# mcveanlab/mccortex

Hardware: AMD Instinct MI355X
Metric: k-mers/s inserted (build), k=31, 50M x 150bp synthetic reads (higher is better)
Workload: dtype u64

## Files before the change

### include/mcx_gpu.h

```cpp
#ifndef MCX_GPU_H_
#define MCX_GPU_H_

#include <stddef.h>
#include <stdint.h>

#ifdef __cplusplus
extern "C" {
#endif

typedef enum {
  MCX_OK = 0,
  MCX_ERR_ARG = -1,
  MCX_ERR_NODEVICE = -2,
  MCX_ERR_NOMEM = -3,
  MCX_ERR_FULL = -4,
  MCX_ERR_HIP = -5,
  MCX_ERR_SINK = -6
} mcx_status;

typedef struct {
  uint64_t num_se_reads;
  uint64_t num_good_reads;
  uint64_t num_bad_reads;
  uint64_t total_bases_read;
  uint64_t total_bases_loaded;
  uint64_t contigs_parsed;
  uint64_t num_kmers_loaded;
  uint64_t num_kmers_novel;
  uint64_t num_pe_reads;
  uint64_t num_dup_se_reads;
  uint64_t num_dup_pe_pairs;
} mcx_load_stats;

typedef struct mcx_graph mcx_graph;

const char *mcx_last_error(void);
const char *mcx_version(void);
int mcx_device_count(void);
int mcx_device_memory(int device, uint64_t *free_bytes, uint64_t *total_bytes);

int mcx_graph_create(mcx_graph **g, int kmer_size, int ncols,
                     uint64_t capacity_kmers, int device);
int mcx_graph_create_shard(mcx_graph **g, int kmer_size, int ncols, uint64_t capacity_kmers,
                           int device, int nparts, int part);
void mcx_graph_destroy(mcx_graph *g);

int mcx_graph_reset(mcx_graph *g);

int mcx_graph_configure(mcx_graph *g, const char *key, uint64_t value);
int mcx_graph_profile(mcx_graph *g, char *buf, size_t buflen);

int mcx_graph_create_multi(mcx_graph **out, int kmer_size, int ncols, uint64_t capacity_kmers,
                           const int *devices, int ndevices);
int mcx_multi_exchange_bytes(int kmer_size, int ndevices, uint64_t capacity_kmers, uint64_t *bytes_per_device);
int mcx_graph_ndevices(const mcx_graph *g);

int mcx_graph_capacity(const mcx_graph *g, uint64_t *slots, uint64_t *bytes);

int mcx_graph_add_reads(mcx_graph *g, int colour,
                        const uint8_t *bases, const uint8_t *quals,
                        const uint64_t *read_offsets, uint64_t nreads,
                        uint8_t fq_cutoff_abs, uint8_t hp_cutoff,
                        mcx_load_stats *stats_accum);

int mcx_graph_add_reads_pcr(mcx_graph *g, int colour,
                            const uint8_t *bases, const uint8_t *quals,
                            const uint64_t *read_offsets, uint64_t nreads,
                            uint8_t fq_cutoff_abs1, uint8_t fq_cutoff_abs2, uint8_t hp_cutoff,
                            int paired, int matedir, mcx_load_stats *stats_accum);
int mcx_graph_pcr_reset(mcx_graph *g);

int mcx_graph_add_stream_dev(mcx_graph *g, int colour,
                             const void *d_stream, uint64_t nbytes);

int mcx_pack_stream_dev(const void *d_stream, uint64_t nbytes, void *d_code, void *d_inv, void *hip_stream);
int mcx_graph_add_packed_dev(mcx_graph *g, int colour, const void *d_code, const void *d_inv, uint64_t npos);

int mcx_graph_partition_stream_dev(mcx_graph *g, const void *d_stream, uint64_t nbytes,
                                   int nparts, uint64_t bin_capacity,
                                   void *d_keys, void *d_edges, void *d_counts);
int mcx_graph_insert_tuples_dev(mcx_graph *g, int colour, const void *d_keys,
                                const void *d_edges, uint64_t n);
uint32_t mcx_key_owner(const uint64_t *key_words, int kmer_size, int nparts);

int mcx_graph_hashtest(mcx_graph *g, uint64_t first, uint64_t n);
int mcx_hashtest_func(int device, int kmer_size, uint64_t n, uint32_t nparts, uint64_t *hash_out);

int mcx_debug_probe(void *d_buf, uint64_t cap_words, uint32_t nregions, uint32_t spb, uint32_t iters, uint32_t jit_mask, float *ms_out);

int mcx_graph_insert_tuple_segments_dev(mcx_graph *g, int colour, const void *d_keys, const void *d_edges,
                                        const void *d_counts, uint32_t nseg, uint64_t seg_cap);

int mcx_graph_shard_layout(mcx_graph *g, uint64_t tuples_per_call, uint32_t *segs_per_owner,
                           uint64_t *seg_cap, uint64_t *ov_cap);
int mcx_graph_shard_bins_dev(mcx_graph *g, const void *d_stream, uint64_t nbytes, void *d_keys,
                             void *d_counts, uint64_t seg_cap, void *d_ov_keys, void *d_ov_edges,
                             void *d_ov_counts, uint64_t ov_cap);
int mcx_graph_add_segments_dev(mcx_graph *g, int colour, const void *d_keys, const void *d_counts,
                               uint32_t nseg, uint64_t seg_cap, uint64_t ntuples);
uint32_t mcx_graph_key_owner(const mcx_graph *g, const uint64_t *key_words);

enum { MCX_RECORDS_MUST_EXIST = 1, MCX_RECORDS_MASK_EDGES = 2 };
typedef struct {
  uint64_t nkmers_read, nkmers_loaded, nkmers_novel;
  int64_t first_oversized, first_zero_covg, first_edges_no_covg;
} mcx_records_stats;
int mcx_graph_add_records(mcx_graph *g, const void *recs, uint64_t nrecs, int file_ncols,
                          const int32_t *from_col, const int32_t *into_col, int nmap, uint32_t flags,
                          mcx_records_stats *stats_accum);

int mcx_graph_intersect_finish(mcx_graph *g, uint64_t *removed);

#define MCX_CLEAN_NBINS 1000
#define MCX_CLEAN_BYTES_PER_KMER 64
#define MCX_CLEAN_BYTES_PER_SLOT 4
typedef struct {
  uint64_t num_tips, num_tip_kmers;
  uint64_t num_low_covg_unitigs, num_low_covg_unitig_kmers;
  uint64_t num_tip_and_low_unitigs, num_tip_and_low_unitig_kmers;
  uint64_t nkmers_before, nkmers_removed;
} mcx_clean_stats;
int mcx_graph_unitig_stats(mcx_graph *g, uint64_t *before);
int mcx_graph_clean(mcx_graph *g, uint32_t covg_threshold, uint32_t min_keep_tip, mcx_clean_stats *stats, uint64_t *after);

enum { MCX_INFER_POP = 1, MCX_INFER_PRESENCE_COVG = 2 };
int mcx_graph_infer_edges(mcx_graph *g, void *recs, uint64_t nrecs, int ncols, uint32_t flags, uint64_t *nmodified);
int mcx_graph_infer_edges_dev(mcx_graph *g, void *d_recs, uint64_t nrecs, int ncols, uint32_t flags, uint64_t *nmodified);

int mcx_graph_kmer_covg(mcx_graph *g, uint64_t *nkmers, uint64_t *sumcov);
int mcx_graph_covg_histogram(mcx_graph *g, uint64_t *hist, uint32_t nbins);

int mcx_graph_checksum(mcx_graph *g, uint64_t *checksum, uint64_t *nkmers);
// ... 52 lines not shown
```

### mccortex_amd/csrc/mcx_api.hip

```cpp
#include <hip/hip_runtime.h>

#include <stdarg.h>
#include <stdio.h>
#include <stdlib.h>
#include <string.h>
#include <cstring>

#include <rocprim/device/device_radix_sort.hpp>
#include <rocprim/device/device_scan.hpp>

#include <algorithm>
#include <array>
#include <cmath>
#include <memory>
#include <vector>
#include <thread>
#include <atomic>
#include <chrono>
#include <mutex>
#include <condition_variable>
#include <functional>

#include "../../include/mcx_gpu.h"
#include "mcx_kernels.h"
// ... 81 lines not shown
  {
    if (owner_.load() == std::this_thread::get_id()) {
      fprintf(stderr, "mcx: internal error: the staging pool was re-entered between begin() and finish()\n");
      abort();
    }
  }
  std::atomic<std::thread::id> owner_{std::thread::id()};
  void worker()
  {
    std::unique_lock<std::mutex> lk(mu_);
    for (;;) {
      cv_work_.wait(lk, [&] { return next_ < T_; });
      const int ti = next_++;
      const std::function<void(int)> *f = fn_;
      lk.unlock();
      (*f)(ti);
      lk.lock();
      if (--pending_ == 0) cv_done_.notify_one();
    }
  }
  std::mutex mu_, call_mu_;
  std::condition_variable cv_work_, cv_done_;
  std::vector<std::thread> th_;
  const std::function<void(int)> *fn_ = nullptr;
  int T_ = 0, next_ = 0, pending_ = 0;
};

constexpr uint64_t kCarry = 128;
constexpr uint32_t kL1Sets = 32;
static uint64_t stage_bytes()
{
  static uint64_t v = 0;
  if (!v) {
    const char *e = getenv("MCX_STAGE_BYTES");
    v = e ? strtoull(e, nullptr, 10) : (128ull << 20);
    if (v < 1024) v = 1024;
    v = (v + 63) / 64 * 64;
  }
  return v;
}
#define kStageBytes stage_bytes()

struct mcx_group;
struct mcx_graph {
  int k = 0, W = 0, ncols = 0, device = 0;
  hipStream_t stream = nullptr;
  TableView t{};
  uint64_t table_bytes = 0;
  uint64_t touch_bytes = 0;
  Counters *d_ctr = nullptr;
  Counters *h_ctr = nullptr;
  uint32_t *h_full = nullptr;
  static constexpr int kStageBufs = 3;
  uint8_t *h_stage[kStageBufs] = {nullptr, nullptr, nullptr};
  uint8_t *d_stage[kStageBufs] = {nullptr, nullptr, nullptr};
  hipEvent_t ev[kStageBufs] = {nullptr, nullptr, nullptr};
  hipStream_t cstream = nullptr;
  hipEvent_t ev_copy[kStageBufs] = {nullptr, nullptr, nullptr}, ev_wait0[kStageBufs] = {nullptr, nullptr, nullptr}, ev_wait1[kStageBufs] = {nullptr, nullptr, nullptr};
  bool ev_wait_used[kStageBufs] = {false, false, false};
  uint64_t stage_alloc = 0;
  int cur = 0;
  int grid = 0;
  int grid_stream = 0, grid_split = 0, grid_insert = 0;
  bool defer = true;
  uint64_t defer_tuples = 0;
  uint32_t nsub = 0;
  uint32_t b1 = 0, subs_per_bin = 0;
  uint64_t cap1 = 0, cap2 = 0;
  uint32_t rep1 = 8;
  bool rep1_forced = false;
  uint64_t *l1_keys = nullptr, *l2_keys = nullptr;
  uint64_t *l2_hi = nullptr;
  uint64_t l2_hi_off = 0;
  uint64_t *l2_base = nullptr;
  int place_tries = 1;
  uint64_t l2_off = 0;
  hipStream_t stream2 = nullptr;
  hipEvent_t ev_split[2] = {nullptr, nullptr}, ev_ins[2] = {nullptr, nullptr};
  unsigned long long *l1_cnt = nullptr, *l2_cnt = nullptr;
  uint32_t nsets = 1;
  uint64_t set_cap = 0;
  std::vector<int> set_colour;
  std::vector<uint64_t> set_pending;
  uint64_t pending = 0;
  uint64_t pending_l2 = 0;
  uint32_t l2_regions = 0;
  uint32_t flush_regions = 0;
  uint32_t idle_next = 0;
  uint64_t idle_base = 0;
  std::vector<uint64_t> idle_mark;
  static constexpr uint32_t kSnap = 32;
  struct Snap { uint64_t ub; int set; int which; bool is_base; hipEvent_t ev; };
  Counters *h_snap = nullptr;
  Snap snap[kSnap] = {};
  uint32_t snap_head = 0, snap_tail = 0;
  uint64_t snap_last[2] = {0, 0};
  bool snap_base_known = true;
  uint64_t n_flushes = 0;
  int hidden = -1;
  int ncols_vis = 0;
  uint32_t *d_readstrt = nullptr;
  bool must_exist = false;
  int pending_colour = 0;
  bool profile = false;
  int overlap = -1;
  struct Span { const char *name; hipEvent_t a, b; };
  std::vector<Span> spans;
  mcx_group *group = nullptr;
  int gidx = 0;
  mcx_group *as_group = nullptr;
  uint32_t own_lbo = 0;
  unsigned long long *d_infer = nullptr;
  struct CleanCache *clean = nullptr;
};

static uint8_t *touch_base(const mcx_graph *g) { return reinterpret_cast<uint8_t *>(g->t.touch) - kTouchHdr; }

static OwnerSpec owner_spec(const mcx_graph *g)
{
  if (g->own_lbo) return OwnerSpec{2u, g->own_lbo, (uint32_t)g->gidx, g->k};
  return OwnerSpec{g->t.lbo ? 1u : 0u, 0u, 0u, g->k};
}

static int flush_deferred(mcx_graph *g);
static void free_defer(mcx_graph *g);
static void snap_push(mcx_graph *g, bool is_base);
static void snap_push(mcx_graph *g, bool is_base, uint64_t ub, int set, int which);
static void sets_release(mcx_graph *g)
{
  std::fill(g->set_colour.begin(), g->set_colour.end(), -1);
  std::fill(g->set_pending.begin(), g->set_pending.end(), 0);
}
struct StreamLaunch;
static int group_submit_stream(mcx_group *G, int idx, const StreamLaunch &L, int colour);
static void group_destroy(mcx_group *G);
static int grp_drain(mcx_group *G);
static int grp_sync(mcx_group *G);
static int grp_device_stats(mcx_group *G, mcx_load_stats *out);
static int grp_add_reads(mcx_group *G, int colour, const uint8_t *bases, const uint8_t *quals, const uint64_t *off,
                         uint64_t nreads, uint8_t fq, uint8_t hp, mcx_load_stats *stats_accum);
static int grp_add_reads_pcr(mcx_group *G, int colour, const uint8_t *bases, const uint8_t *quals, const uint64_t *off,
                             uint64_t nreads, uint8_t fq1, uint8_t fq2, uint8_t hp, int paired, int matedir,
                             mcx_load_stats *stats_accum);
static int grp_add_reads_must_exist(mcx_group *G, int colour, const uint8_t *bases, const uint8_t *quals, const uint64_t *off,
                                    uint64_t nreads, uint8_t fq, uint8_t hp, mcx_load_stats *stats_accum);
static int grp_intersect_finish(mcx_group *G, uint64_t *removed);
static int grp_add_records(mcx_group *G, const void *recs, uint64_t nrecs, int file_ncols, const int32_t *from_col,
                           const int32_t *into_col, int nmap, uint32_t flags, mcx_records_stats *stats_accum);
static int grp_export(mcx_group *G, mcx_graph *f, int sorted, mcx_sink_fn sink, void *ctx);
static int grp_part_of_pointer(mcx_group *G, const void *d_ptr, mcx_graph **part);
static mcx_graph *grp_part(mcx_group *G, int i);
static int grp_n(mcx_group *G);
static uint64_t grp_spilled(mcx_group *G);
#define NO_GROUP(g, what) do { if ((g) && (g)->as_group) return fail(MCX_ERR_ARG, what " takes a shard, not the multi-GPU handle"); } while (0)

extern "C" const char *mcx_last_error(void) { return g_err; }
extern "C" const char *mcx_version(void) { return "mccortex_amd 0.1 (gfx950)"; }

extern "C" int mcx_device_count(void)
{
  int n = 0;
  if (hipGetDeviceCount(&n) != hipSuccess) return 0;
  return n;
}

extern "C" int mcx_device_memory(int device, uint64_t *free_bytes, uint64_t *total_bytes)
{
  int ndev = 0;
  if (hipGetDeviceCount(&ndev) != hipSuccess || device < 0 || device >= ndev)
    return fail(MCX_ERR_NODEVICE, "no HIP device %d", device);
  HIP_TRY(hipSetDevice(device));
  size_t f = 0, t = 0;
  HIP_TRY(hipMemGetInfo(&f, &t));
  if (free_bytes) *free_bytes = f;
  if (total_bytes) *total_bytes = t;
  return MCX_OK;
}

static int check_k(int k)
{
  if (k < 3 || k > 127 || !(k & 1)) return fail(MCX_ERR_ARG, "kmer size must be odd and 3..127 (got %d)", k);
  return MCX_OK;
}

extern "C" int mcx_graph_create(mcx_graph **out, int kmer_size, int ncols, uint64_t capacity_kmers, int device)
{
  return mcx_graph_create_shard(out, kmer_size, ncols, capacity_kmers, device, 1, 0);
}

static uint32_t region_bits(uint64_t nsub, uint32_t lbo)
{
  uint32_t lb1 = 0;
  const uint32_t lb1_max = lbo ? std::min<uint32_t>(9, 11 - lbo) : 9;
  while (lb1 < lb1_max && (2ull << lb1) <= nsub) lb1++;
  while (lb1 < 11 && ((nsub + (1ull << lb1) - 1) >> lb1) > (uint64_t)kMaxBins) lb1++;
  return lb1;
}

extern "C" int mcx_graph_create_shard(mcx_graph **out, int kmer_size, int ncols, uint64_t capacity_kmers, int device,
                                      int nparts, int part)
{
  if (!out) return fail(MCX_ERR_ARG, "null handle pointer");
  *out = nullptr;
  if (check_k(kmer_size) != MCX_OK) return MCX_ERR_ARG;
  if (nparts < 1 || nparts > 32 || (nparts & (nparts - 1)) || part < 0 || part >= nparts)
    return fail(MCX_ERR_ARG, "shards must be a power of two <= 32 and 0 <= part < shards (got %d of %d)", part, nparts);
  if (ncols < 1 || ncols > 4096) return fail(MCX_ERR_ARG, "ncols out of range: %d", ncols);
  if (kmer_size > 63 && nparts != 1)
    return fail(MCX_ERR_ARG, "k > 63 (three- and four-word keys) builds on one device: the exchange formats carry at most two key words");
  int ndev = 0;
  if (hipGetDeviceCount(&ndev) != hipSuccess || ndev <= 0)
    return fail(MCX_ERR_NODEVICE, "no HIP device available (this library has no CPU path)");
  if (device < 0 || device >= ndev) return fail(MCX_ERR_NODEVICE, "device %d out of range (%d devices)", device, ndev);
  HIP_TRY(hipSetDevice(device));

  mcx_graph *g = new mcx_graph();
  g->k = kmer_size;
  g->W = words_for_k(kmer_size);
  g->ncols = ncols;
  g->ncols_vis = ncols;
  g->device = device;
  const uint64_t sub_slots = 1ull << sub_shift_for_words(g->W);
  uint64_t nsub = (std::max<uint64_t>(capacity_kmers, 1024) + sub_slots - 1) / sub_slots;
  uint32_t lbo = 0;
  while ((1 << lbo) < nparts) lbo++;
  uint32_t lb1 = region_bits(nsub, lbo);
  if (const char *e = getenv("MCX_LB1")) { const uint32_t v = (uint32_t)atoi(e); if (!lbo && v >= 6 && v <= 11 && ((nsub + (1ull << v) - 1) >> v) <= (uint64_t)kMaxBins && ((nsub + (1ull << v) - 1) >> v) >= 1) lb1 = v; }
  if (lbo && lb1 + lbo > 11) {
    const uint64_t max_slots = ((uint64_t)kMaxBins << (11 - lbo)) * sub_slots;
    delete g;
    return fail(MCX_ERR_ARG, "capacity per device too large for a table split over %d devices: %llu slots requested, at most %llu "
                "(use more devices or a smaller -n / -m)", nparts, (unsigned long long)(nsub * sub_slots), (unsigned long long)max_slots);
  }
  const uint64_t spb = (nsub + (1ull << lb1) - 1) >> lb1;
  nsub = spb << lb1;
  if (nsub >= (1ull << 31)) { delete g; return fail(MCX_ERR_ARG, "capacity too large"); }
  uint64_t novf = std::max<uint64_t>(sub_slots, (nsub * sub_slots / 32 + sub_slots - 1) / sub_slots * sub_slots);
  if (const char *e = getenv("MCX_OVERFLOW_SLOTS")) novf = strtoull(e, nullptr, 10) / kBucket * kBucket;
  if (novf / kBucket >= (1ull << 32)) novf = ((1ull << 32) - 1) * kBucket;
  const uint64_t slots = nsub * sub_slots + novf;
  g->t.nmain = nsub * sub_slots;
  g->t.nslots = slots;
  g->t.lb1 = lb1;
  g->t.lbo = lbo;
  g->t.part = (uint32_t)part;
  g->t.spb = (uint32_t)spb;
  g->t.S = (uint32_t)(g->W + ncols);
  g->t.max_probe = (uint32_t)sub_slots;
  { const char *e = getenv("MCX_DEFER"); if (e) g->defer = atoi(e) != 0; }
  if (g->W > 2) g->defer = false;
  { const char *e = getenv("MCX_GRID_STREAM"); if (e) g->grid_stream = atoi(e); }
  { const char *e = getenv("MCX_REP1"); if (e && atoi(e) >= 1 && atoi(e) <= 4096) { g->rep1 = (uint32_t)atoi(e); g->rep1_forced = true; } }
  { const char *e = getenv("MCX_GRID_SPLIT"); if (e) g->grid_split = atoi(e); }
  { const char *e = getenv("MCX_GRID_INSERT"); if (e) g->grid_insert = atoi(e); }
  g->table_bytes = slots * g->t.S * 8;

  hipDeviceProp_t prop;
  HIP_TRY(hipGetDeviceProperties(&prop, device));
  g->grid = prop.multiProcessorCount * 8;

#define CREATE_TRY(expr)                                                            \
  do {                                                                              \
    hipError_t _e = (expr);                                                         \
    if (_e != hipSuccess) {                                                         \
      int rc = fail(_e == hipErrorOutOfMemory ? MCX_ERR_NOMEM : MCX_ERR_HIP, "%s: %s", #expr, hipGetErrorString(_e)); \
      mcx_graph_destroy(g);                                                         \
      return rc;                                                                    \
    }                                                                               \
  } while (0)
  CREATE_TRY(hipStreamCreateWithFlags(&g->stream, hipStreamNonBlocking));
  CREATE_TRY(hipMalloc((void **)&g->t.rec, g->table_bytes));
  if (ncols == 1) {
    g->t.KS = g->t.VS = (uint32_t)(g->W + 1);
    g->t.val = g->t.rec + g->W;
    g->t.VC = 0;
  } else {
    g->t.KS = (uint32_t)g->W;
    g->t.VS = 1;
    g->t.val = g->t.rec + g->t.nslots * (uint64_t)g->W;
    g->t.VC = g->t.nslots;
  }
  CREATE_TRY(hipMalloc((void **)&g->d_ctr, sizeof(Counters)));
  CREATE_TRY(hipHostMalloc((void **)&g->h_ctr, sizeof(Counters), hipHostMallocDefault));
  CREATE_TRY(hipHostMalloc((void **)&g->h_full, sizeof(uint32_t), hipHostMallocDefault));
  *g->h_full = 0;
  g->touch_bytes = (1 + ((g->t.nmain >> sub_shift_for_words(g->W)) + 31) / 32) * 4;
  {
    uint8_t *tb = nullptr;
    CREATE_TRY(hipMalloc((void **)&tb, kTouchHdr + g->touch_bytes));
    g->t.touch = reinterpret_cast<uint32_t *>(tb + kTouchHdr);
  }
  CREATE_TRY(hipMemsetAsync(g->t.rec, 0, g->table_bytes, g->stream));
  CREATE_TRY(hipMemsetAsync(touch_base(g), 0, kTouchHdr + g->touch_bytes, g->stream));
  CREATE_TRY(hipMemsetAsync(g->d_ctr, 0, sizeof(Counters), g->stream));
  CREATE_TRY(hipStreamSynchronize(g->stream));
#undef CREATE_TRY
  *out = g;
  return MCX_OK;
}

static void clean_drop(mcx_graph *g);

extern "C" void mcx_graph_destroy(mcx_graph *g)
{
  if (g && g->as_group) { group_destroy(g->as_group); delete g; return; }
  if (!g) return;
  (void)hipSetDevice(g->device);
  if (g->stream) (void)hipStreamSynchronize(g->stream);
  if (g->cstream) { (void)hipStreamSynchronize(g->cstream); (void)hipStreamDestroy(g->cstream); }
  for (int i = 0; i < mcx_graph::kStageBufs; i++) {
    if (g->h_stage[i]) (void)hipHostFree(g->h_stage[i]);
    if (g->d_stage[i]) (void)hipFree(g->d_stage[i]);
    if (g->ev[i]) (void)hipEventDestroy(g->ev[i]);
    if (g->ev_copy[i]) (void)hipEventDestroy(g->ev_copy[i]);
    if (g->ev_wait0[i]) (void)hipEventDestroy(g->ev_wait0[i]);
    if (g->ev_wait1[i]) (void)hipEventDestroy(g->ev_wait1[i]);
  }
  free_defer(g);
  for (auto &sp : g->spans) { (void)hipEventDestroy(sp.a); (void)hipEventDestroy(sp.b); }
  if (g->t.rec) (void)hipFree(g->t.rec);
  if (g->t.touch) (void)hipFree(touch_base(g));
  if (g->stream2) {
    (void)hipStreamDestroy(g->stream2);
    for (int i = 0; i < 2; i++) { (void)hipEventDestroy(g->ev_split[i]); (void)hipEventDestroy(g->ev_ins[i]); }
  }
  if (g->d_ctr) (void)hipFree(g->d_ctr);
  if (g->d_readstrt) (void)hipFree(g->d_readstrt);
  if (g->d_infer) (void)hipFree(g->d_infer);
  clean_drop(g);
  if (g->h_ctr) (void)hipHostFree(g->h_ctr);
  if (g->h_full) (void)hipHostFree(g->h_full);
  if (g->h_snap) {
    (void)hipHostFree(g->h_snap);
    for (uint32_t i = 0; i < mcx_graph::kSnap; i++) (void)hipEventDestroy(g->snap[i].ev);
  }
  if (g->stream) (void)hipStreamDestroy(g->stream);
  delete g;
}

extern "C" int mcx_graph_reset(mcx_graph *g)
{
  if (g && g->as_group) {
    int rc = grp_drain(g->as_group);
    for (int i = 0; rc == MCX_OK && i < grp_n(g->as_group); i++) rc = mcx_graph_reset(grp_part(g->as_group, i));
    return rc;
  }
  if (!g) return fail(MCX_ERR_ARG, "null graph");
  HIP_TRY(hipSetDevice(g->device));
  clean_drop(g);
  HIP_TRY(hipMemsetAsync(g->t.rec, 0, g->table_bytes, g->stream));
  HIP_TRY(hipMemsetAsync(touch_base(g), 0, kTouchHdr + g->touch_bytes, g->stream));
  HIP_TRY(hipMemsetAsync(g->d_ctr, 0, sizeof(Counters), g->stream));
  g->n_flushes = 0;
  if (g->h_full) { HIP_TRY(hipStreamSynchronize(g->stream)); *g->h_full = 0; }
  if (g->l1_cnt) HIP_TRY(hipMemsetAsync(g->l1_cnt, 0, (size_t)g->nsets * g->b1 * g->rep1 * 8, g->stream));
  if (g->l2_cnt) HIP_TRY(hipMemsetAsync(g->l2_cnt, 0, (size_t)g->l2_regions * g->subs_per_bin * 8, g->stream));
  if (g->d_readstrt) HIP_TRY(hipMemsetAsync(g->d_readstrt, 0xff, g->t.nslots * 8, g->stream));
  g->pending = g->pending_l2 = 0;
  g->idle_next = 0; g->idle_base = 0; g->idle_mark.clear();
  sets_release(g);
  snap_push(g, true);
  return MCX_OK;
}

extern "C" int mcx_graph_capacity(const mcx_graph *g, uint64_t *slots, uint64_t *bytes)
{
  if (g && g->as_group) {
    uint64_t s_ = 0, b_ = 0;
    for (int i = 0; i < grp_n(g->as_group); i++) { uint64_t s1 = 0, b1 = 0; mcx_graph_capacity(grp_part(g->as_group, i), &s1, &b1); s_ += s1; b_ += b1; }
    if (slots) *slots = s_;
    if (bytes) *bytes = b_;
    return MCX_OK;
  }
  if (!g) return fail(MCX_ERR_ARG, "null graph");
  if (slots) *slots = g->t.nslots;
  if (bytes) *bytes = g->table_bytes;
  return MCX_OK;
}

extern "C" void *mcx_graph_stream(mcx_graph *g) { return !g ? nullptr : g->as_group ? (void *)grp_part(g->as_group, 0)->stream : (void *)g->stream; }

struct StreamLaunch {
  const uint8_t *stream;
  uint64_t nbytes, pos_lo, pos_hi;
  unsigned char *flag;
  const uint32_t *code = nullptr;
  const uint16_t *inv = nullptr;
};

#define DISPATCH_WC(g, F, ...)                                                        \
  do {                                                                                \
    if ((g)->W == 1) { if ((g)->ncols == 1) F<1, true>(__VA_ARGS__); else F<1, false>(__VA_ARGS__); } \
    else { if ((g)->ncols == 1) F<2, true>(__VA_ARGS__); else F<2, false>(__VA_ARGS__); }            \
  } while (0)

#define DISPATCH_WC4(g, F, ...)                                                       \
  do {                                                                                \
    const bool one_ = (g)->ncols == 1;                                                \
    switch ((g)->W) {                                                                 \
      case 1: if (one_) F<1, true>(__VA_ARGS__); else F<1, false>(__VA_ARGS__); break; \
      case 2: if (one_) F<2, true>(__VA_ARGS__); else F<2, false>(__VA_ARGS__); break; \
      case 3: if (one_) F<3, true>(__VA_ARGS__); else F<3, false>(__VA_ARGS__); break; \
      default: if (one_) F<4, true>(__VA_ARGS__); else F<4, false>(__VA_ARGS__); break; \
    }                                                                                 \
  } while (0)
#define LAUNCH_W4(W_, KERNEL, ...)                                       \
  do {                                                                   \
    switch (W_) {                                                        \
      case 1: hipLaunchKernelGGL((KERNEL<1>), __VA_ARGS__); break;       \
      case 2: hipLaunchKernelGGL((KERNEL<2>), __VA_ARGS__); break;       \
      case 3: hipLaunchKernelGGL((KERNEL<3>), __VA_ARGS__); break;       \
      default: hipLaunchKernelGGL((KERNEL<4>), __VA_ARGS__); break;      \
    }                                                                    \
  } while (0)
#define NO_WIDE(g, what) do { if ((g) && (g)->W > 2) return fail(MCX_ERR_ARG, what " is not available for k > 63"); } while (0)

struct SpanGuard {
  mcx_graph *g; size_t idx; bool on;
  SpanGuard(mcx_graph *g_, const char *name) : g(g_), idx(0), on(g_->profile) {
    if (!on) return;
    mcx_graph::Span sp{name, nullptr, nullptr};
    (void)hipEventCreate(&sp.a); (void)hipEventCreate(&sp.b);
    (void)hipEventRecord(sp.a, g->stream);
    idx = g->spans.size();
    g->spans.push_back(sp);
  }
  ~SpanGuard() { if (on) (void)hipEventRecord(g->spans[idx].b, g->stream); }
};

template <class K> static void allow_lds(K kernel, size_t bytes)
{
  (void)hipFuncSetAttribute(reinterpret_cast<const void *>(kernel), hipFuncAttributeMaxDynamicSharedMemorySize, (int)bytes);
}

static StreamArgs make_args(mcx_graph *g, const StreamLaunch &L)
{
  StreamArgs a;
  a.stream = L.stream; a.code = L.code; a.inv = L.inv; a.nbytes = L.nbytes; a.pos_lo = L.pos_lo; a.pos_hi = L.pos_hi;
  a.tile0 = L.pos_lo / kTile;
  a.ntiles = (L.pos_hi + kTile - 1) / kTile;
  a.k = g->k; a.ctr = g->d_ctr; a.flag = L.flag;
  return a;
}

template <int W, bool ONECOL> static void launch_direct_t(mcx_graph *g, const StreamLaunch &L, int colour)
{
  const StreamArgs a = make_args(g, L);
  const uint64_t nt = a.ntiles > a.tile0 ? a.ntiles - a.tile0 : 0;
  if (!nt) return;
  InsertSink<W, ONECOL> is{g->t, (uint32_t)colour};
  SpanGuard sp(g, "k_stream");
  const dim3 grid((unsigned)std::min<uint64_t>(nt, (uint64_t)g->grid));
  if (a.code) hipLaunchKernelGGL((k_stream<W, ONECOL, true>), grid, dim3(kThreads), 0, g->stream, a, is);
  else hipLaunchKernelGGL((k_stream<W, ONECOL, false>), grid, dim3(kThreads), 0, g->stream, a, is);
}

template <int W, bool ONECOL, bool FULL, int SH, bool PK>
static void launch_bin_stream_pk(mcx_graph *g, const StreamArgs &a, uint64_t nt, int colour, BinSpec bs, BinOut out)
{
  InsertSink<W, ONECOL> is{g->t, (uint32_t)colour};
  static bool once_dev[64] = {false};
  bool &once = once_dev[g->device & 63];
  if (!once) {
    allow_lds(k_stream_bin<W, ONECOL, 512, FULL, SH, PK>, sizeof(BinLds<W, 512, FULL>));
    allow_lds(k_stream_bin<W, ONECOL, 1024, FULL, SH, PK>, sizeof(BinLds<W, 1024, FULL>));
    allow_lds(k_stream_bin<W, ONECOL, kMaxBins, FULL, SH, PK>, sizeof(BinLds<W, kMaxBins, FULL>));
    once = true;
  }
  SpanGuard sp(g, "k_stream_bin");
  if constexpr (W == 1 && !FULL && SH == 0) {
    static const int fc_cap = [] { const char *e = getenv("MCX_STREAM_FC"); return e ? atoi(e) : 0; }();
    if (fc_cap && bs.nlocal <= 512) {
      const dim3 gridf((unsigned)std::min<uint64_t>(nt, (uint64_t)(g->grid_stream ? g->grid_stream : g->grid)));
#define MCX_FC_LAUNCH(CAPV, PRIVV) { \
        static bool once_f[64] = {false}; \
        if (!once_f[g->device & 63]) { allow_lds(k_stream_fc<ONECOL, PK, CAPV, PRIVV>, sizeof(FcLds<CAPV>)); once_f[g->device & 63] = true; } \
        hipLaunchKernelGGL((k_stream_fc<ONECOL, PK, CAPV, PRIVV>), gridf, dim3(kThreads), sizeof(FcLds<CAPV>), g->stream, a, bs, out, is); }
      if (bs.rep >= gridf.x && bs.rep > 8) MCX_FC_LAUNCH(10, true)
      else MCX_FC_LAUNCH(10, false)
#undef MCX_FC_LAUNCH
      return;
    }
    static const bool wide = [] { const char *e = getenv("MCX_STREAM_T"); return !e || atoi(e) == 512; }();
    if (wide && bs.nlocal <= 512) {
      using GeoW = Geo<512, 512 * kPosPerLane>;
      static bool once_w[64] = {false};
      if (!once_w[g->device & 63]) { allow_lds(k_stream_bin<W, ONECOL, 512, FULL, SH, PK, 512>, sizeof(BinLds<W, 512, FULL, GeoW>)); once_w[g->device & 63] = true; }
      const dim3 gridw((unsigned)std::min<uint64_t>((nt + 1) / 2, (uint64_t)(g->grid_stream ? g->grid_stream : g->grid)));
      hipLaunchKernelGGL((k_stream_bin<W, ONECOL, 512, FULL, SH, PK, 512>), gridw, dim3(512), sizeof(BinLds<W, 512, FULL, GeoW>), g->stream, a, bs, out, is);
      return;
    }
  }
  const dim3 grid((unsigned)std::min<uint64_t>(nt, (uint64_t)(g->grid_stream ? g->grid_stream : g->grid)));
  if (bs.nlocal <= 512)
    hipLaunchKernelGGL((k_stream_bin<W, ONECOL, 512, FULL, SH, PK>), grid, dim3(kThreads), sizeof(BinLds<W, 512, FULL>), g->stream, a, bs, out, is);
  else if (bs.nlocal <= 1024)
    hipLaunchKernelGGL((k_stream_bin<W, ONECOL, 1024, FULL, SH, PK>), grid, dim3(kThreads), sizeof(BinLds<W, 1024, FULL>), g->stream, a, bs, out, is);
  else
    hipLaunchKernelGGL((k_stream_bin<W, ONECOL, kMaxBins, FULL, SH, PK>), grid, dim3(kThreads), sizeof(BinLds<W, kMaxBins, FULL>), g->stream, a, bs, out, is);
}

template <int W, bool ONECOL, bool FULL, int SH>
static void launch_bin_stream_t(mcx_graph *g, const StreamLaunch &L, int colour, BinSpec bs, BinOut out)
{
  const StreamArgs a = make_args(g, L);
  const uint64_t nt = a.ntiles > a.tile0 ? a.ntiles - a.tile0 : 0;
  if (!nt) return;
  if (!FULL && a.code) launch_bin_stream_pk<W, ONECOL, FULL, SH, !FULL>(g, a, nt, colour, bs, out);
  else launch_bin_stream_pk<W, ONECOL, FULL, SH, false>(g, a, nt, colour, bs, out);
}

template <int W, bool ONECOL, bool IN_FULL, bool SHARD>
static void launch_bin_tuples_t(mcx_graph *g, TupleIn in, int colour, BinSpec bs, BinOut out)
{
  constexpr bool kWide = W == 1 && !IN_FULL;
  static const bool wide = kWide && [] { const char *e = getenv("MCX_SPLIT_T"); return !e || atoi(e) == 512; }();
  const bool use_wide = wide && bs.nlocal <= 1024;
  const bool use_huge = wide && !use_wide && bs.nlocal <= (uint32_t)kMaxBins;
  const uint64_t tile = use_huge ? 1024 * 16 : use_wide ? 512 * 16 : kTile;
  const uint64_t nchunks = (in.seg_cap + tile - 1) / tile * in.nseg;
  if (!nchunks) return;
  InsertSink<W, ONECOL> is{g->t, (uint32_t)colour};
  using GeoW = Geo<512, 512 * 16>;
  static bool once_dev[64] = {false};
  bool &once = once_dev[g->device & 63];
  if (!once) {
    allow_lds(k_tuples_bin<W, ONECOL, 512, IN_FULL, SHARD>, sizeof(BinLds<W, 512, false>));
    allow_lds(k_tuples_bin<W, ONECOL, 1024, IN_FULL, SHARD>, sizeof(BinLds<W, 1024, false>));
    allow_lds(k_tuples_bin<W, ONECOL, kMaxBins, IN_FULL, SHARD>, sizeof(BinLds<W, kMaxBins, false>));
    if constexpr (kWide) allow_lds(k_tuples_bin<W, ONECOL, 512, IN_FULL, SHARD, 512>, sizeof(BinLds<W, 512, false, GeoW>));
    if constexpr (kWide) allow_lds(k_tuples_bin<W, ONECOL, 1024, IN_FULL, SHARD, 512>, sizeof(BinLds<W, 1024, false, GeoW>));
    if constexpr (kWide) allow_lds(k_tuples_bin<W, ONECOL, kMaxBins, IN_FULL, SHARD, 1024>, sizeof(BinLds<W, kMaxBins, false, Geo<1024, 1024 * 16>>));
    once = true;
  }
  SpanGuard sp(g, "k_tuples_bin");
  const uint64_t gmax = (uint64_t)(g->grid_split ? g->grid_split : g->grid * 4);
  if constexpr (kWide) {
    if (use_huge) {
      using GeoH = Geo<1024, 1024 * 16>;
      const dim3 gridh((unsigned)std::min<uint64_t>(nchunks, g->grid_split ? gmax : gmax / 4));
      hipLaunchKernelGGL((k_tuples_bin<W, ONECOL, kMaxBins, IN_FULL, SHARD, 1024>), gridh, dim3(1024), sizeof(BinLds<W, kMaxBins, false, GeoH>), g->stream, in, bs, out, is, g->d_ctr);
      return;
    }
    if (use_wide) {
      const dim3 gridw((unsigned)std::min<uint64_t>(nchunks, g->grid_split ? gmax : gmax / 2));
      if (bs.nlocal <= 512)
        hipLaunchKernelGGL((k_tuples_bin<W, ONECOL, 512, IN_FULL, SHARD, 512>), gridw, dim3(512), sizeof(BinLds<W, 512, false, GeoW>), g->stream, in, bs, out, is, g->d_ctr);
      else
        hipLaunchKernelGGL((k_tuples_bin<W, ONECOL, 1024, IN_FULL, SHARD, 512>), gridw, dim3(512), sizeof(BinLds<W, 1024, false, GeoW>), g->stream, in, bs, out, is, g->d_ctr);
      return;
    }
  }
  const dim3 grid((unsigned)std::min<uint64_t>(nchunks, gmax));
  if (bs.nlocal <= 512)
    hipLaunchKernelGGL((k_tuples_bin<W, ONECOL, 512, IN_FULL, SHARD>), grid, dim3(kThreads), sizeof(BinLds<W, 512, false>), g->stream, in, bs, out, is, g->d_ctr);
  else if (bs.nlocal <= 1024)
    hipLaunchKernelGGL((k_tuples_bin<W, ONECOL, 1024, IN_FULL, SHARD>), grid, dim3(kThreads), sizeof(BinLds<W, 1024, false>), g->stream, in, bs, out, is, g->d_ctr);
  else
    hipLaunchKernelGGL((k_tuples_bin<W, ONECOL, kMaxBins, IN_FULL, SHARD>), grid, dim3(kThreads), sizeof(BinLds<W, kMaxBins, false>), g->stream, in, bs, out, is, g->d_ctr);
}
template <int W, bool ONECOL> static void launch_bin_region_stream(mcx_graph *g, const StreamLaunch &L, int colour, BinSpec bs, BinOut out)
{
  if (g->t.lbo) launch_bin_stream_t<W, ONECOL, false, 1>(g, L, colour, bs, out);
  else launch_bin_stream_t<W, ONECOL, false, 0>(g, L, colour, bs, out);
}
template <int W, bool ONECOL> static void launch_split_regions(mcx_graph *g, TupleIn in, int colour, BinSpec bs, BinOut out)
{ launch_bin_tuples_t<W, ONECOL, false, false>(g, in, colour, bs, out); }
template <int W, bool ONECOL> static void launch_bin_received(mcx_graph *g, TupleIn in, int colour, BinSpec bs, BinOut out)
{
  if (g->t.lbo) launch_bin_tuples_t<W, ONECOL, true, true>(g, in, colour, bs, out);
  else launch_bin_tuples_t<W, ONECOL, true, false>(g, in, colour, bs, out);
}

static uint64_t *l2_ptr(const mcx_graph *g, uint64_t off)
{
  if (g->l2_hi && off >= g->l2_hi_off) return g->l2_hi + (off - g->l2_hi_off) * g->cap2 * g->W;
  return g->l2_keys + off * g->cap2 * g->W;
}

template <int W, bool ONECOL> static void launch_lds_insert_t(mcx_graph *g, int colour, uint32_t sub0, uint32_t nsub)
{
  const size_t lds = Sub<W>::kSlots * (W + 1) * 8 + LdsQueue<W>::kTuples * 8 * W;
  static bool once_dev[64] = {false};
  bool &once = once_dev[g->device & 63];
  if (!once) { allow_lds(k_lds_insert<W, ONECOL>, lds); once = true; }
  BinOut bins{l2_ptr(g, g->l2_off), nullptr, g->l2_cnt + g->l2_off, g->cap2, nullptr, nullptr, nullptr, 0};
  SpanGuard sp(g, "k_lds_insert");
  hipLaunchKernelGGL((k_lds_insert<W, ONECOL>), dim3((unsigned)std::min<uint64_t>(nsub, (uint64_t)(g->grid_insert ? g->grid_insert : g->grid * 4))),
                     dim3(LdsCfg<W>::kThreads), lds, g->stream, g->t, (uint32_t)colour, bins, sub0, nsub, g->d_ctr);
}

template <int W, bool ONECOL>
static void launch_insert_tuples_t(mcx_graph *g, int colour, const uint64_t *keys, const uint8_t *edges, uint64_t n, uint32_t only_own = 0)
{
  const int grid = (int)std::min<uint64_t>((n + kThreads * kBatch - 1) / (kThreads * kBatch), (uint64_t)g->grid);
  InsertSink<W, ONECOL> s{g->t, (uint32_t)colour};
  SpanGuard sp(g, "k_insert_tuples");
  hipLaunchKernelGGL((k_insert_tuples<W, ONECOL>), dim3(grid), dim3(kThreads), 0, g->stream, s, keys, edges, n, g->d_ctr, only_own);
}

static void free_defer(mcx_graph *g)
{
  (void)hipFree(g->l1_keys); (void)hipFree(g->l1_cnt);
  (void)hipFree(g->l2_base); (void)hipFree(g->l2_hi); (void)hipFree(g->l2_cnt);
  g->l1_keys = g->l2_keys = g->l2_base = g->l2_hi = nullptr; g->l1_cnt = g->l2_cnt = nullptr;
  g->cap1 = g->cap2 = 0;
  g->l2_regions = 0;
  g->set_colour.clear(); g->set_pending.clear();
}

__global__ __launch_bounds__(512) void k_l2_probe(uint64_t *keys, uint64_t cap, uint32_t nregions, uint32_t spb, uint32_t iters,
                                                  uint32_t jit_mask = 0 )
{
  const uint32_t region = blockIdx.x % nregions, blk = blockIdx.x / nregions, nblk = gridDim.x / nregions;
  const uint32_t w = threadIdx.x >> 6, l = threadIdx.x & 63u;
  for (uint32_t it = 0; it < iters; it++)
    for (uint32_t k = 0; k < spb / 32u; k++) {
      const uint32_t front = w * 4u + (l >> 4) + 32u * k;
      const uint32_t seg = region * spb + front;
      const uint64_t jit = ((seg * 0x9E3779B1u) >> 8) & jit_mask & ~15u;
      const uint64_t at = (uint64_t)seg * cap + jit + ((uint64_t)it * nblk + blk) * 16u + (l & 15u);
      if (jit + ((uint64_t)it * nblk + blk) * 16u + 16u <= cap) keys[at] = at;
    }
}

static uint64_t *l2_place(mcx_graph *g, size_t bytes, uint32_t nreg, int tries, float *ms_out)
{
  std::vector<uint64_t *> cand;
  std::vector<float> ms;
  hipEvent_t e0 = nullptr, e1 = nullptr;
  if (tries > 1 && (hipEventCreate(&e0) != hipSuccess || hipEventCreate(&e1) != hipSuccess)) { (void)hipGetLastError(); tries = 1; }
  const uint32_t iters = (uint32_t)std::max<uint64_t>(8, g->cap2 * g->W / 1024);
  for (int i = 0; i < std::max(tries, 1); i++) {
    if (i > 0) {
      size_t fr = 0, tot = 0;
      if (hipMemGetInfo(&fr, &tot) != hipSuccess || fr < bytes + (size_t)(tot / 16)) { (void)hipGetLastError(); break; }
    }
    uint64_t *p = nullptr;
    if (hipMalloc((void **)&p, bytes) != hipSuccess) { (void)hipGetLastError(); break; }
    cand.push_back(p);
    float t = 0.f;
    if (tries > 1)
      for (int rep = 0; rep < 2; rep++) {
        (void)hipEventRecord(e0, g->stream);
        hipLaunchKernelGGL(k_l2_probe, dim3(nreg * 64), dim3(512), 0, g->stream, p, g->cap2 * g->W, nreg, g->subs_per_bin, iters);
        (void)hipEventRecord(e1, g->stream);
        if (hipEventSynchronize(e1) != hipSuccess || hipEventElapsedTime(&t, e0, e1) != hipSuccess) { (void)hipGetLastError(); t = 0.f; }
      }
    ms.push_back(t);
    float worst = 0.f, best_t = 0.f;
    for (float x : ms) { worst = std::max(worst, x); if (x > 0.f && (best_t == 0.f || x < best_t)) best_t = x; }
    if (tries > 1 && best_t > 0.f && best_t < 0.70f * worst) break;
  }
  if (e0) (void)hipEventDestroy(e0);
  if (e1) (void)hipEventDestroy(e1);
  if (cand.empty()) return nullptr;
  size_t best = 0;
  for (size_t i = 1; i < cand.size(); i++) if (ms[i] > 0.f && (ms[best] <= 0.f || ms[i] < ms[best])) best = i;
  for (size_t i = 0; i < cand.size(); i++) if (i != best) (void)hipFree(cand[i]);
  if (getenv("MCX_TIMING") && cand.size() > 1) {
    fprintf(stderr, "[timing] sub-table bins (%u regions): %zu placements probed:", nreg, cand.size());
    for (size_t i = 0; i < cand.size(); i++) fprintf(stderr, " %.3f%s", ms[i], i == best ? "*" : "");
    fprintf(stderr, " ms\n");
  }
  if (ms_out) *ms_out = ms[best];
  return cand[best];
}

static uint32_t flush_group(const mcx_graph *g);
static int ensure_l2(mcx_graph *g, uint32_t regions, bool whole = false)
{
  if (g->l2_keys && g->l2_regions >= regions && !(g->l2_hi && (whole || (regions > g->l2_regions / 2 && regions != g->l2_regions)))) return MCX_OK;
  if (g->pending_l2) return fail(MCX_ERR_ARG, "internal: sub-table bins resized while in use");
  HIP_TRY(hipStreamSynchronize(g->stream));
  (void)hipFree(g->l2_base); (void)hipFree(g->l2_hi); (void)hipFree(g->l2_cnt);
  g->l2_keys = g->l2_base = g->l2_hi = nullptr; g->l2_cnt = nullptr; g->l2_regions = 0; g->l2_hi_off = 0;
  const uint64_t nb = (uint64_t)regions * g->subs_per_bin;
  int tries = g->place_tries;
  { const char *e = getenv("MCX_PLACE_BINS"); if (e) tries = atoi(e); }
  if (g->subs_per_bin % 32 || regions < 8) tries = 1;
  const uint32_t G = flush_group(g);
  const bool halves = !whole && tries > 1 && regions == 2 * G && !g->t.lbo && !g->group;
  if (halves) {
    const size_t hbytes = (nb / 2) * g->cap2 * 8 * g->W;
    g->l2_base = l2_place(g, hbytes, G, tries, nullptr);
    if (g->l2_base) g->l2_hi = l2_place(g, hbytes, G, tries, nullptr);
    if (g->l2_base && !g->l2_hi) { (void)hipFree(g->l2_base); g->l2_base = nullptr; }
    g->l2_hi_off = nb / 2;
  } else {
    g->l2_base = l2_place(g, nb * g->cap2 * 8 * g->W, std::min<uint32_t>(regions, 32), tries, nullptr);
  }
  if (!g->l2_base || hipMalloc((void **)&g->l2_cnt, nb * 8) != hipSuccess) {
    (void)hipGetLastError();
    (void)hipFree(g->l2_base); (void)hipFree(g->l2_hi); g->l2_base = g->l2_hi = nullptr;
    return fail(MCX_ERR_NOMEM, "out of device memory for the sub-table bins (%llu regions)", (unsigned long long)regions);
  }
  HIP_TRY(hipMemsetAsync(g->l2_cnt, 0, nb * 8, g->stream));
  g->l2_keys = g->l2_base;
  g->l2_regions = regions;
  return MCX_OK;
}

static bool flush_overlap(const mcx_graph *g)
{
  static const bool on = [] { const char *e = getenv("MCX_FLUSH_OVERLAP"); return !e || atoi(e) != 0; }();
  return g->overlap < 0 ? on : g->overlap != 0;
}

static uint32_t flush_group(const mcx_graph *g)
{
  uint32_t G = g->flush_regions;
  if (!G) {
    const char *e = getenv("MCX_FLUSH_REGIONS");
    G = e ? (uint32_t)strtoul(e, nullptr, 10) : 0;
  }
  if (!G) G = std::max<uint32_t>(32u, 16384u / std::max<uint32_t>(1u, g->subs_per_bin));
  return std::min<uint32_t>(G, g->b1);
}

static int ensure_defer(mcx_graph *g)
{
  if (g->l1_keys) return MCX_OK;
  g->nsub = (uint32_t)(g->t.nmain >> sub_shift_for_words(g->W));
  g->b1 = 1u << g->t.lb1;
  g->subs_per_bin = g->t.spb;
  if (g->t.lb1 < 6 || g->b1 > (uint32_t)kMaxBins || g->subs_per_bin > (uint32_t)kMaxBins) { g->defer = false; return MCX_OK; }
  uint64_t tcap = g->defer_tuples;
  if (!tcap) {
    const char *e = getenv("MCX_DEFER_TUPLES");
    if (e) {
      tcap = strtoull(e, nullptr, 10);
    } else {
      size_t fr = 0, tot = 0;
      (void)hipMemGetInfo(&fr, &tot);
      const uint64_t per_tuple = 8ull * g->W * (g->t.lbo ? 240 : 118) / 100 + 1;
      const uint64_t by_mem = (uint64_t)((double)fr * 0.40) / per_tuple;
      tcap = std::max<uint64_t>(std::min<uint64_t>(std::min<uint64_t>(64 * g->t.nslots, by_mem), 1ull << 33), 1ull << 20);
    }
  }
  for (;; tcap /= 2) {
    if (tcap < (1ull << 20)) { g->defer = false; g->defer_tuples = 0; (void)hipGetLastError(); return MCX_OK; }
    g->defer_tuples = tcap;
    g->nsets = g->ncols > 1 ? kL1Sets : 1;
    if (const char *e = getenv("MCX_L1_SETS")) { const int v = atoi(e); if (v >= 1 && v <= 32) g->nsets = (uint32_t)v; }
    g->set_cap = tcap / g->nsets;
    if (!g->rep1_forced) g->rep1 = g->nsets != 1 ? 8 : g->set_cap / g->b1 / 64 >= (1u << 16) ? 64 : g->set_cap / g->b1 / 32 >= (1u << 16) ? 32 : 8;
    g->cap1 = (uint64_t)((double)g->set_cap / g->b1 / g->rep1 * (g->b1 == 1 ? 1.02 : 1.06)) + (g->nsets > 1 ? 2048 : 8192);
    static const double cap2_slack = [] { const char *e = getenv("MCX_CAP2_SLACK"); const double v = e ? atof(e) : 0; return v >= 1.0 && v <= 4.0 ? v : 1.25; }();
    g->cap2 = g->nsub == 1 ? tcap + 8192 : (uint64_t)((double)tcap / g->nsub * cap2_slack) + 1024;
    g->cap1 = (g->cap1 + 1) & ~1ull;
    g->cap2 = (g->cap2 + 1) & ~1ull;
    if (g->cap1 >= 0xFFFFFFFFull || g->cap2 >= 0xFFFFFFFFull) continue;
    const uint64_t n1 = (uint64_t)g->nsets * g->b1 * g->rep1 * g->cap1;
    const bool ok = hipMalloc((void **)&g->l1_keys, n1 * 8 * g->W) == hipSuccess &&
                    hipMalloc((void **)&g->l1_cnt, (size_t)g->nsets * g->b1 * g->rep1 * 8) == hipSuccess &&
                    ensure_l2(g, flush_overlap(g) ? std::min<uint32_t>(2 * flush_group(g), g->b1) : flush_group(g)) == MCX_OK;
    if (ok) break;
    free_defer(g);
    (void)hipGetLastError();
  }
  HIP_TRY(hipMemsetAsync(g->l1_cnt, 0, (size_t)g->nsets * g->b1 * g->rep1 * 8, g->stream));
  g->set_colour.assign(g->nsets, -1);
  g->set_pending.assign(g->nsets, 0);
  return MCX_OK;
}

static BinOut l1_out(const mcx_graph *g, int set)
{
  const uint64_t segs = (uint64_t)g->b1 * g->rep1;
  return BinOut{g->l1_keys + (uint64_t)set * segs * g->cap1 * g->W, nullptr, g->l1_cnt + (uint64_t)set * segs, g->cap1, nullptr, nullptr, nullptr, 0};
}

static int ensure_flush_stream(mcx_graph *g)
{
  if (g->stream2) return MCX_OK;
  HIP_TRY(hipStreamCreateWithFlags(&g->stream2, hipStreamNonBlocking));
  for (int i = 0; i < 2; i++) {
    if (!g->ev_split[i]) HIP_TRY(hipEventCreateWithFlags(&g->ev_split[i], hipEventDisableTiming));
    if (!g->ev_ins[i]) HIP_TRY(hipEventCreateWithFlags(&g->ev_ins[i], hipEventDisableTiming));
  }
  return MCX_OK;
}

static int flush_deferred(mcx_graph *g)
{
  if (!g->pending && !g->pending_l2) {
    sets_release(g);
    if (!g->idle_mark.empty()) {
      g->idle_next = 0; g->idle_base = 0; g->idle_mark.clear();
      snap_push(g, true);
    }
    return MCX_OK;
  }
  HIP_TRY(hipSetDevice(g->device));
  const uint32_t G = g->pending_l2 ? g->b1 : std::min(flush_group(g), g->l2_regions);
  if (g->pending_l2 && g->l2_regions < g->b1) return fail(MCX_ERR_ARG, "internal: split tuples without bins");
  const bool overlap = flush_overlap(g) && g->pending && !g->pending_l2 && g->l2_regions >= 2 * G && G < g->b1;
  hipStream_t s1 = g->stream;
  if (overlap) {
    int rc2 = ensure_flush_stream(g);
    if (rc2 != MCX_OK) return rc2;
    HIP_TRY(hipEventRecord(g->ev_split[0], s1));
    HIP_TRY(hipStreamWaitEvent(g->stream2, g->ev_split[0], 0));
  }
  std::vector<int> colours;
  if (g->pending_l2) colours.push_back(g->pending_colour);
  for (uint32_t s = 0; s < g->nsets && g->pending; s++) {
    const int c = g->set_colour[s];
    if (c >= 0 && g->set_pending[s] && std::find(colours.begin(), colours.end(), c) == colours.end()) colours.push_back(c);
  }
  uint32_t gi = 0;
  for (size_t ci = 0; ci < colours.size(); ci++) {
    const int colour = colours[ci];
    TupleIn in{};
    uint32_t nmine = 0;
    for (uint32_t s = 0; s < g->nsets && g->pending; s++)
      if (g->set_colour[s] == colour && g->set_pending[s]) in.set_map[nmine++] = (uint8_t)s;
    for (uint32_t r0 = 0; r0 < g->b1; r0 += G, gi++) {
      const uint32_t ng = std::min(G, g->b1 - r0);
      const int hb = overlap ? (int)(gi & 1u) : 0;
      g->l2_off = (uint64_t)hb * G * g->subs_per_bin;
      if (overlap && gi >= 2) HIP_TRY(hipStreamWaitEvent(s1, g->ev_ins[hb], 0));
      if (nmine) {
        in.keys = g->l1_keys + (uint64_t)r0 * g->cap1 * g->W;
        in.edges = nullptr;
        in.counts = g->l1_cnt + r0;
        in.seg_cap = g->cap1;
        in.nseg = ng * g->rep1 * nmine;
        in.seg_group = ng;
        in.seg_stride = g->b1;
        in.set_rep = g->nsets > 1 ? g->rep1 : 0;
        BinSpec bs{BIN_SUBLOCAL, 0, g->subs_per_bin, 1, ng * g->subs_per_bin, ng, 0, r0};
        BinOut out{l2_ptr(g, g->l2_off), nullptr, g->l2_cnt + g->l2_off, g->cap2, nullptr, nullptr, nullptr, 0};
        DISPATCH_WC(g, launch_split_regions, g, in, colour, bs, out);
        HIP_TRY(hipGetLastError());
      }
      if (overlap) {
        HIP_TRY(hipEventRecord(g->ev_split[hb], s1));
        HIP_TRY(hipStreamWaitEvent(g->stream2, g->ev_split[hb], 0));
        g->stream = g->stream2;
      }
      DISPATCH_WC(g, launch_lds_insert_t, g, colour, r0 * g->subs_per_bin, ng * g->subs_per_bin);
      g->stream = s1;
      HIP_TRY(hipGetLastError());
      if (overlap) HIP_TRY(hipEventRecord(g->ev_ins[hb], g->stream2));
    }
  }
  g->l2_off = 0;
  if (overlap)
    for (int i = 0; i < 2; i++) HIP_TRY(hipStreamWaitEvent(s1, g->ev_ins[i], 0));
  if (g->pending) HIP_TRY(hipMemsetAsync(g->l1_cnt, 0, (size_t)g->nsets * g->b1 * g->rep1 * 8, g->stream));
  g->pending = 0;
  g->pending_l2 = 0;
  g->n_flushes++;
  g->idle_next = 0; g->idle_base = 0; g->idle_mark.clear();
  sets_release(g);
  snap_push(g, true);
  return MCX_OK;
}

static void snap_push(mcx_graph *g, bool is_base, uint64_t ub, int set, int which)
{
  if (!g->h_snap) {
    if (hipHostMalloc((void **)&g->h_snap, sizeof(Counters) * mcx_graph::kSnap, hipHostMallocDefault) != hipSuccess) { (void)hipGetLastError(); g->h_snap = nullptr; return; }
    for (uint32_t i = 0; i < mcx_graph::kSnap; i++)
      if (hipEventCreateWithFlags(&g->snap[i].ev, hipEventDisableTiming) != hipSuccess) {
        (void)hipGetLastError();
        for (uint32_t j = 0; j < i; j++) { (void)hipEventDestroy(g->snap[j].ev); g->snap[j].ev = nullptr; }
        (void)hipHostFree(g->h_snap);
        g->h_snap = nullptr;
        return;
      }
  }
  if (is_base) {
    g->snap_tail = g->snap_head;
    g->snap_base_known = false;
  }
  if (g->snap_head - g->snap_tail >= mcx_graph::kSnap) return;
  const uint32_t i = g->snap_head % mcx_graph::kSnap;
  if (hipMemcpyAsync(&g->h_snap[i], g->d_ctr, sizeof(Counters), hipMemcpyDeviceToHost, g->stream) != hipSuccess ||
      hipEventRecord(g->snap[i].ev, g->stream) != hipSuccess) { (void)hipGetLastError(); return; }
  g->snap[i].ub = ub;
  g->snap[i].set = set;
  g->snap[i].which = which;
  g->snap[i].is_base = is_base;
  g->snap_head++;
}
static void snap_push(mcx_graph *g, bool is_base) { snap_push(g, is_base, 0, 0, 0); }

static void snap_poll(mcx_graph *g)
{
  if (!g->h_snap) return;
  while (g->snap_tail != g->snap_head) {
    const uint32_t i = g->snap_tail % mcx_graph::kSnap;
    if (hipEventQuery(g->snap[i].ev) != hipSuccess) { (void)hipGetLastError(); break; }
    const uint64_t v[2] = {g->h_snap[i].kmers, g->h_snap[i].binned};
    const mcx_graph::Snap &e = g->snap[i];
    if (e.is_base) {
      g->snap_base_known = true;
    } else if (g->snap_base_known && g->idle_mark.empty() && (size_t)e.set < g->set_pending.size()) {
      const uint64_t yielded = std::min<uint64_t>(e.ub, v[e.which] - g->snap_last[e.which]);
      const uint64_t d = e.ub - yielded;
      g->pending -= std::min(g->pending, d);
      g->set_pending[e.set] -= std::min(g->set_pending[e.set], d);
    }
    g->snap_last[0] = v[0];
    g->snap_last[1] = v[1];
    g->snap_tail++;
  }
}

static bool defer_has_room(const mcx_graph *g, int colour, uint64_t need)
{
  for (uint32_t s = 0; s < g->nsets; s++)
    if (g->set_colour[s] < 0 || (g->set_colour[s] == colour && g->set_pending[s] + need <= g->set_cap)) return true;
  return false;
}
static void settle_for_room(mcx_graph *g, int colour, uint64_t need)
{
  if (!g->h_snap) return;
  while (!defer_has_room(g, colour, need) && g->snap_tail != g->snap_head) {
    if (hipEventSynchronize(g->snap[g->snap_tail % mcx_graph::kSnap].ev) != hipSuccess) { (void)hipGetLastError(); return; }
    const uint32_t before = g->snap_tail;
    snap_poll(g);
    if (g->snap_tail == before) return;
// ... 7 lines not shown
  if (rc != MCX_OK || !g->defer) return rc;
  snap_poll(g);
  settle_for_room(g, colour, ub);
  for (int pass = 0; pass < 2; pass++) {
    int free_set = -1;
    for (uint32_t s = 0; s < g->nsets; s++) {
      if (g->set_colour[s] == colour && g->set_pending[s] + ub <= g->set_cap) {
        g->set_pending[s] += ub; g->pending += ub;
        if (set_out) *set_out = (int)s;
        return MCX_OK;
      }
      if (g->set_colour[s] < 0 && free_set < 0) free_set = (int)s;
    }
    if (free_set >= 0) {
      g->set_colour[free_set] = colour;
      g->set_pending[free_set] = ub; g->pending += ub;
      if (set_out) *set_out = free_set;
      return MCX_OK;
    }
    rc = flush_deferred(g);
    if (rc != MCX_OK) return rc;
  }
  return fail(MCX_ERR_ARG, "internal: no L1 bin set after a flush");
}

static int l2_reserve(mcx_graph *g, int colour, uint64_t ub)
{
  int rc = ensure_defer(g);
  if (rc != MCX_OK || !g->defer) return rc;
  if ((g->pending_l2 && colour != g->pending_colour) ||
      ((g->pending_l2 || g->pending) && g->pending_l2 + g->pending + ub > g->defer_tuples)) {
    rc = flush_deferred(g);
    if (rc != MCX_OK) return rc;
  }
  g->pending_colour = colour;
  return MCX_OK;
}

static int full_poll(mcx_graph *g)
{
  if (!g->h_full || !g->t.touch) return MCX_OK;
  if (*g->h_full) return fail(MCX_ERR_FULL, "Hash table is full");
  HIP_TRY(hipMemcpyAsync(g->h_full, g->t.touch - 2, sizeof(uint32_t), hipMemcpyDeviceToHost, g->stream));
  return MCX_OK;
}

static int submit_stream(mcx_graph *g, const StreamLaunch &L, int colour)
{
  if (g->group) return group_submit_stream(g->group, g->gidx, L, colour);
  { int rc = full_poll(g); if (rc != MCX_OK) return rc; }
  if (g->defer) { int rc = ensure_defer(g); if (rc != MCX_OK) return rc; }
  if (!g->defer) {
    DISPATCH_WC4(g, launch_direct_t, g, L, colour);
    HIP_TRY(hipGetLastError());
    return MCX_OK;
  }
  snap_poll(g);
  for (uint64_t lo = L.pos_lo; lo < L.pos_hi;) {
    settle_for_room(g, colour, std::min<uint64_t>(L.pos_hi - lo, g->set_cap));
    uint64_t room = g->set_cap;
    for (uint32_t s = 0; s < g->nsets; s++)
      if (g->set_colour[s] == colour && g->set_pending[s] < g->set_cap) { room = g->set_cap - g->set_pending[s]; break; }
    if (room < (uint64_t)kTile * 16 && room < L.pos_hi - lo) room = g->set_cap;
    const uint64_t hi = std::min(L.pos_hi, lo + room);
    int set = 0;
    int rc = defer_reserve(g, colour, hi - lo, &set);
    if (rc != MCX_OK) return rc;
    StreamLaunch P = L;
    P.pos_lo = lo; P.pos_hi = hi;
    BinSpec bs{BIN_GROUP, 0, g->b1, g->rep1, g->b1, 1, 0, 0};
    BinOut out = l1_out(g, set);
    DISPATCH_WC(g, launch_bin_region_stream, g, P, colour, bs, out);
    HIP_TRY(hipGetLastError());
    snap_push(g, false, hi - lo, set, 0);
    lo = hi;
  }
  return MCX_OK;
}

static int ensure_stage(mcx_graph *g);



extern "C" int mcx_graph_configure(mcx_graph *g, const char *key, uint64_t value)
{
  if (g && key && g->as_group) {
    const bool isec = !strcmp(key, "intersect");
    if (isec && g->ncols < 2) return fail(MCX_ERR_ARG, "intersect mode needs one colour more than the output has");
    if (!strcmp(key, "defer") && !value) return fail(MCX_ERR_ARG, "a multi-GPU table always uses the partitioned insert");
    int rc = grp_drain(g->as_group);
    for (int i = 0; rc == MCX_OK && i < grp_n(g->as_group); i++) rc = mcx_graph_configure(grp_part(g->as_group, i), key, value);
    if (isec && rc == MCX_OK) {
      g->hidden = g->ncols - 1;
      g->ncols_vis = g->ncols - 1;
    }
    return rc;
  }
  if (!g || !key) return fail(MCX_ERR_ARG, "null argument");
  HIP_TRY(hipSetDevice(g->device));
  if (!strcmp(key, "defer")) {
    int rc = flush_deferred(g);
    if (rc != MCX_OK) return rc;
    g->defer = value != 0 && g->W <= 2;
    return MCX_OK;
  }
  if (!strcmp(key, "debug_realloc_l2")) {
    int rc = flush_deferred(g);
    if (rc != MCX_OK) return rc;
    if (!g->l2_keys || g->l2_hi) return MCX_OK;
    HIP_TRY(hipStreamSynchronize(g->stream));
    if (g->stream2) HIP_TRY(hipStreamSynchronize(g->stream2));
    static std::vector<void *> holes;
    void *hole = nullptr;
    if (value && hipMalloc(&hole, value) == hipSuccess) holes.push_back(hole);
    uint64_t *nk = nullptr;
    HIP_TRY(hipMalloc((void **)&nk, (uint64_t)g->l2_regions * g->subs_per_bin * g->cap2 * 8 * g->W));
    (void)hipFree(g->l2_base);
    g->l2_base = g->l2_keys = nk;
    return MCX_OK;
  }
  if (!strcmp(key, "place_bins")) {
    if (value < 1 || value > 32) return fail(MCX_ERR_ARG, "place_bins: 1..32");
    g->place_tries = (int)value;
    return MCX_OK;
  }
  if (!strcmp(key, "defer_tuples")) {
    int rc = flush_deferred(g);
    if (rc != MCX_OK) return rc;
    HIP_TRY(hipStreamSynchronize(g->stream));
    free_defer(g);
    g->defer_tuples = value;
    return MCX_OK;
  }
  if (!strcmp(key, "flush_overlap")) {
    int rc = flush_deferred(g);
    if (rc != MCX_OK) return rc;
    HIP_TRY(hipStreamSynchronize(g->stream));
    g->overlap = value != 0;
    if (g->l1_keys && g->overlap) return ensure_l2(g, std::min<uint32_t>(2 * flush_group(g), g->b1));
    return MCX_OK;
  }
  if (!strcmp(key, "flush_regions")) {
    int rc = flush_deferred(g);
    if (rc != MCX_OK) return rc;
    g->flush_regions = (uint32_t)value;
    if (g->l1_keys) return ensure_l2(g, flush_group(g));
    return MCX_OK;
  }
  if (!strcmp(key, "intersect")) {
    if (!value) return fail(MCX_ERR_ARG, "intersect mode cannot be switched off");
    if (g->ncols < 2) return fail(MCX_ERR_ARG, "intersect mode needs one colour more than the output has");
    HIP_TRY(hipStreamSynchronize(g->stream));
    g->hidden = g->ncols - 1;
    g->ncols_vis = g->ncols - 1;
    g->defer = false;
    return MCX_OK;
  }
  if (!strcmp(key, "must_exist")) {
    int rc = flush_deferred(g);
    if (rc != MCX_OK) return rc;
    g->must_exist = value != 0;
    if (g->must_exist) g->defer = false;
    return MCX_OK;
  }
  if (!strcmp(key, "prepare")) {
    const double t0 = now_s();
    int rc = ensure_stage(g);
    const double t1 = now_s();
    if (rc == MCX_OK && g->defer && !g->must_exist) rc = ensure_defer(g);
    const double t2 = now_s();
    if (rc == MCX_OK && g->defer && !g->must_exist && flush_overlap(g)) rc = ensure_flush_stream(g);
    if (getenv("MCX_TIMING"))
      fprintf(stderr, "[timing] prepare: pinned staging + copy stream %.1f ms, partition workspace (%.1f GB) %.1f ms, flush stream %.1f ms\n", (t1 - t0) * 1e3,
              g->l1_keys ? (double)g->nsets * g->b1 * g->rep1 * g->cap1 * 8 * g->W / 1e9 : 0.0, (t2 - t1) * 1e3, (now_s() - t2) * 1e3);
    return rc;
  }
  if (!strcmp(key, "grid")) {
    if (value > (1u << 20)) return fail(MCX_ERR_ARG, "grid: 0 .. 2^20 blocks");
    int cus = 0;
    HIP_TRY(hipDeviceGetAttribute(&cus, hipDeviceAttributeMultiprocessorCount, g->device));
    g->grid = value ? (int)value : cus * 8;
    return MCX_OK;
  }
  if (!strcmp(key, "grid_stream")) { g->grid_stream = (int)value; return MCX_OK; }
  if (!strcmp(key, "grid_split")) { g->grid_split = (int)value; return MCX_OK; }
  if (!strcmp(key, "grid_insert")) { g->grid_insert = (int)value; return MCX_OK; }
  if (!strcmp(key, "profile")) {
    HIP_TRY(hipStreamSynchronize(g->stream));
    for (auto &sp : g->spans) { (void)hipEventDestroy(sp.a); (void)hipEventDestroy(sp.b); }
    g->spans.clear();
    g->profile = value != 0;
    return MCX_OK;
  }
  return fail(MCX_ERR_ARG, "unknown configuration key '%s'", key);
}

extern "C" int mcx_graph_profile(mcx_graph *g, char *buf, size_t buflen)
{
  if (g && buf && buflen && g->as_group) {
    size_t o = 0;
    buf[0] = '\0';
    std::vector<char> tmp(buflen);
    for (int i = 0; i < grp_n(g->as_group); i++) {
// ... 34 lines not shown
  if (g && g->as_group) {
    mcx_graph *part = nullptr;
    int rc = grp_part_of_pointer(g->as_group, d_stream, &part);
    if (rc != MCX_OK) return rc;
    return mcx_graph_add_stream_dev(part, colour, d_stream, nbytes);
  }
  if (!g) return fail(MCX_ERR_ARG, "null graph");
  if (colour < 0 || colour >= g->ncols) return fail(MCX_ERR_ARG, "colour %d out of range", colour);
  if (((uintptr_t)d_stream & 15) != 0) return fail(MCX_ERR_ARG, "stream must be 16-byte aligned");
  if (!nbytes) return MCX_OK;
  HIP_TRY(hipSetDevice(g->device));
  StreamLaunch L{(const uint8_t *)d_stream, nbytes, 0, nbytes, nullptr};
  return submit_stream(g, L, colour);
}

extern "C" int mcx_pack_stream_dev(const void *d_stream, uint64_t nbytes, void *d_code, void *d_inv, void *hip_stream)
{
  if (!d_stream || !d_code || !d_inv) return fail(MCX_ERR_ARG, "null argument");
  if (((uintptr_t)d_stream & 15) != 0) return fail(MCX_ERR_ARG, "stream must be 16-byte aligned");
  if (!nbytes) return MCX_OK;
  const uint64_t nch = (nbytes + 15) / 16;
  hipLaunchKernelGGL(k_pack_stream, dim3((unsigned)((nch + 255) / 256)), dim3(256), 0, (hipStream_t)hip_stream,
                     (const uint8_t *)d_stream, nbytes, (uint32_t *)d_code, (uint16_t *)d_inv);
  HIP_TRY(hipGetLastError());
  return MCX_OK;
}

extern "C" int mcx_graph_add_packed_dev(mcx_graph *g, int colour, const void *d_code, const void *d_inv, uint64_t npos)
{
  if (!g) return fail(MCX_ERR_ARG, "null graph");
  if (g->as_group) {
    mcx_graph *part = nullptr;
    int rc = grp_part_of_pointer(g->as_group, d_code, &part);
    if (rc != MCX_OK) return rc;
    return mcx_graph_add_packed_dev(part, colour, d_code, d_inv, npos);
  }
  if (colour < 0 || colour >= g->ncols) return fail(MCX_ERR_ARG, "colour %d out of range", colour);
  if (!d_code || !d_inv) return fail(MCX_ERR_ARG, "null argument");
  if (!npos) return MCX_OK;
  if (g->must_exist) return fail(MCX_ERR_ARG, "device streams cannot be loaded in must-exist mode");
  HIP_TRY(hipSetDevice(g->device));
  StreamLaunch L{nullptr, npos, 0, npos, nullptr, (const uint32_t *)d_code, (const uint16_t *)d_inv};
  return submit_stream(g, L, colour);
}

extern "C" int mcx_graph_partition_stream_dev(mcx_graph *g, const void *d_stream, uint64_t nbytes, int nparts,
                                              uint64_t bin_capacity, void *d_keys, void *d_edges, void *d_counts)
{
  NO_GROUP(g, "mcx_graph_partition_stream_dev");
  if (!g) return fail(MCX_ERR_ARG, "null graph");
  NO_WIDE(g, "mcx_graph_partition_stream_dev");
  if (nparts < 1 || nparts > kMaxBins) return fail(MCX_ERR_ARG, "nparts must be 1..%d", kMaxBins);
  if (bin_capacity >= 0xFFFFFFFFull) return fail(MCX_ERR_ARG, "bin capacity must be below 2^32 tuples");
  if (((uintptr_t)d_stream & 15) != 0) return fail(MCX_ERR_ARG, "stream must be 16-byte aligned");
  if (!nbytes) return MCX_OK;
  HIP_TRY(hipSetDevice(g->device));
  StreamLaunch L{(const uint8_t *)d_stream, nbytes, 0, nbytes, nullptr};
  BinSpec bs{BIN_OWNER, (uint32_t)nparts, (uint32_t)nparts, 1, (uint32_t)nparts, 1, 0, 0};
  BinOut out{(uint64_t *)d_keys, (uint8_t *)d_edges, (unsigned long long *)d_counts, bin_capacity, nullptr, nullptr, nullptr, 0};
  if (g->W == 1) launch_bin_stream_t<1, true, true, 0>(g, L, 0, bs, out);
  else launch_bin_stream_t<2, true, true, 0>(g, L, 0, bs, out);
  HIP_TRY(hipGetLastError());
  return MCX_OK;
}

extern "C" int mcx_graph_insert_tuples_dev(mcx_graph *g, int colour, const void *d_keys, const void *d_edges, uint64_t n)
{
  NO_GROUP(g, "mcx_graph_insert_tuples_dev");
  if (!g) return fail(MCX_ERR_ARG, "null graph");
  if (colour < 0 || colour >= g->ncols) return fail(MCX_ERR_ARG, "colour %d out of range", colour);
  if (!n) return MCX_OK;
  HIP_TRY(hipSetDevice(g->device));
  if (g->defer) { int rc = ensure_defer(g); if (rc != MCX_OK) return rc; }
  if (!g->defer) {
    DISPATCH_WC4(g, launch_insert_tuples_t, g, colour, (const uint64_t *)d_keys, (const uint8_t *)d_edges, n);
    HIP_TRY(hipGetLastError());
    return MCX_OK;
  }
  for (uint64_t lo = 0; lo < n;) {
    const uint64_t cnt = std::min(n - lo, g->set_cap);
    int set = 0;
    int rc = defer_reserve(g, colour, cnt, &set);
    if (rc != MCX_OK) return rc;
    TupleIn in{(const uint64_t *)d_keys + lo * g->W, (const uint8_t *)d_edges + lo, nullptr, cnt, 1, 1, 1};
    BinSpec bs{BIN_GROUP, 0, g->b1, g->rep1, g->b1, 1, 0, 0};
    BinOut out = l1_out(g, set);
    DISPATCH_WC(g, launch_bin_received, g, in, colour, bs, out);
    HIP_TRY(hipGetLastError());
    lo += cnt;
  }
  return MCX_OK;
}

extern "C" int mcx_debug_probe(void *d_buf, uint64_t cap_words, uint32_t nregions, uint32_t spb, uint32_t iters, uint32_t jit_mask, float *ms_out)
{
  hipEvent_t e0, e1;
  HIP_TRY(hipEventCreate(&e0)); HIP_TRY(hipEventCreate(&e1));
  float t = 0.f;
  for (int rep = 0; rep < 2; rep++) {
    (void)hipEventRecord(e0, 0);
    hipLaunchKernelGGL(k_l2_probe, dim3(nregions * 64), dim3(512), 0, 0, (uint64_t *)d_buf, cap_words, nregions, spb, iters, jit_mask);
    (void)hipEventRecord(e1, 0);
    HIP_TRY(hipEventSynchronize(e1));
    HIP_TRY(hipEventElapsedTime(&t, e0, e1));
  }
  (void)hipEventDestroy(e0); (void)hipEventDestroy(e1);
  if (ms_out) *ms_out = t;
  return MCX_OK;
}

template <int W> __global__ void k_hashtest_keys(uint64_t *keys, uint64_t first, uint64_t n)
{
  for (uint64_t i = (uint64_t)blockIdx.x * blockDim.x + threadIdx.x; i < n; i += (uint64_t)gridDim.x * blockDim.x) {
    keys[i * W] = first + i;
    for (int w = 1; w < W; w++) keys[i * W + w] = 0;
  }
}
template <int W> __global__ void k_hashtest_func(uint64_t lo, uint64_t hi, unsigned int *out)
{
  uint32_t h = 0;
  for (uint64_t i = lo + (uint64_t)blockIdx.x * blockDim.x + threadIdx.x; i < hi; i += (uint64_t)gridDim.x * blockDim.x) {
    Kmer<W> key;
    key.w[0] = i;
    for (int w = 1; w < W; w++) key.w[w] = 0;
    h ^= kmer_hash<W>(key, 0, nullptr);
  }
  for (int d = 32; d; d >>= 1) h ^= __shfl_xor(h, d, 64);
  if ((threadIdx.x & 63) == 0 && h) atomicXor(out, h);
}

extern "C" int mcx_graph_hashtest(mcx_graph *g, uint64_t first, uint64_t n)
{
  NO_GROUP(g, "mcx_graph_hashtest");
  if (!g) return fail(MCX_ERR_ARG, "null graph");
  if (first + n < first) return fail(MCX_ERR_ARG, "key range wraps");
  HIP_TRY(hipSetDevice(g->device));
  const uint64_t chunk = std::min<uint64_t>(n, 1ull << 26);
  if (!chunk) return mcx_graph_sync(g);
  uint64_t *d_keys = nullptr;
  uint8_t *d_edges = nullptr;
  if (hipMalloc((void **)&d_keys, chunk * 8 * g->W) != hipSuccess || hipMalloc((void **)&d_edges, chunk) != hipSuccess) {
    (void)hipGetLastError(); (void)hipFree(d_keys); (void)hipFree(d_edges);
    return fail(MCX_ERR_NOMEM, "out of device memory for the hashtest key buffer");
  }
  int rc = MCX_OK;
  if (hipMemsetAsync(d_edges, 0, chunk, g->stream) != hipSuccess) rc = fail(MCX_ERR_HIP, "hipMemsetAsync failed");
  for (uint64_t lo = 0; lo < n && rc == MCX_OK; lo += chunk) {
    const uint64_t cnt = std::min(chunk, n - lo);
    LAUNCH_W4(g->W, k_hashtest_keys, dim3(4096), dim3(256), 0, g->stream, d_keys, first + lo, cnt);
    rc = mcx_graph_insert_tuples_dev(g, 0, d_keys, d_edges, cnt);
  }
  const int rc2 = mcx_graph_sync(g);
  (void)hipFree(d_keys); (void)hipFree(d_edges);
  return rc != MCX_OK ? rc : rc2;
}

extern "C" int mcx_hashtest_func(int device, int kmer_size, uint64_t n, uint32_t nparts, uint64_t *hash_out)
{
  int ndev = 0;
  if (hipGetDeviceCount(&ndev) != hipSuccess || device < 0 || device >= ndev) return fail(MCX_ERR_NODEVICE, "no HIP device %d", device);
  if (kmer_size < 3 || kmer_size > 127 || !(kmer_size & 1)) return fail(MCX_ERR_ARG, "kmer size %d", kmer_size);
  if (!nparts || !hash_out) return fail(MCX_ERR_ARG, "nparts / hash_out");
  HIP_TRY(hipSetDevice(device));
  unsigned int *d = nullptr;
  HIP_TRY(hipMalloc((void **)&d, (size_t)nparts * 4));
  std::vector<unsigned int> h(nparts, 0);
  bool ok = hipMemset(d, 0, (size_t)nparts * 4) == hipSuccess;
  const int W = words_for_k(kmer_size);
  for (uint32_t p = 0; p < nparts && ok; p++) {
    const uint64_t lo = (uint64_t)p * (n / nparts), hi = p + 1 == nparts ? n : lo + n / nparts;
    if (hi <= lo) continue;
    const unsigned grid = (unsigned)std::min<uint64_t>((hi - lo + 255) / 256, 8192);
    LAUNCH_W4(W, k_hashtest_func, dim3(grid), dim3(256), 0, 0, lo, hi, d + p);
  }
  ok = ok && hipMemcpy(h.data(), d, (size_t)nparts * 4, hipMemcpyDeviceToHost) == hipSuccess;
  (void)hipFree(d);
  if (!ok) { (void)hipGetLastError(); return fail(MCX_ERR_HIP, "hashtest kernels failed"); }
  uint64_t sum = 0;
  for (uint32_t p = 0; p < nparts; p++) sum += h[p];
  *hash_out = sum;
  return MCX_OK;
}

extern "C" int mcx_graph_insert_tuple_segments_dev(mcx_graph *g, int colour, const void *d_keys, const void *d_edges,
                                                   const void *d_counts, uint32_t nseg, uint64_t seg_cap)
{
  NO_GROUP(g, "mcx_graph_insert_tuple_segments_dev");
  if (!g) return fail(MCX_ERR_ARG, "null graph");
  if (colour < 0 || colour >= g->ncols) return fail(MCX_ERR_ARG, "colour %d out of range", colour);
  if (!nseg || !seg_cap) return MCX_OK;
  if (!d_keys || !d_edges || !d_counts) return fail(MCX_ERR_ARG, "null tuple buffers");
  HIP_TRY(hipSetDevice(g->device));
  int rc = ensure_defer(g);
  if (rc != MCX_OK) return rc;
  if (!g->defer) return fail(MCX_ERR_ARG, "tuple segments need the deferred insert path (table too small or defer=0)");
  const uint64_t ub = std::min<uint64_t>((uint64_t)nseg * seg_cap, g->set_cap);
  int set = 0;
  rc = defer_reserve(g, colour, ub, &set);
  if (rc != MCX_OK) return rc;
  TupleIn in{(const uint64_t *)d_keys, (const uint8_t *)d_edges, (const unsigned long long *)d_counts, seg_cap, nseg, nseg, nseg};
  BinSpec bs{BIN_GROUP, 0, g->b1, g->rep1, g->b1, 1, 0, 0};
  BinOut out = l1_out(g, set);
  DISPATCH_WC(g, launch_bin_received, g, in, colour, bs, out);
  HIP_TRY(hipGetLastError());
  return MCX_OK;
}

static const uint32_t kShardRep = 8;

extern "C" int mcx_graph_shard_layout(mcx_graph *g, uint64_t tuples_per_call, uint32_t *segs_per_owner,
                                      uint64_t *seg_cap, uint64_t *ov_cap)
{
  NO_GROUP(g, "mcx_graph_shard_layout");
  if (!g) return fail(MCX_ERR_ARG, "null graph");
  NO_WIDE(g, "mcx_graph_shard_layout");
  const uint32_t nparts = 1u << g->t.lbo, b1 = 1u << g->t.lb1;
  const uint64_t nseg = (uint64_t)nparts * kShardRep * b1;
  if (segs_per_owner) *segs_per_owner = kShardRep * b1;
  if (seg_cap) *seg_cap = (uint64_t)((double)tuples_per_call / (double)nseg * 1.06) + 2048;
  if (ov_cap) *ov_cap = std::max<uint64_t>(1u << 16, tuples_per_call / nparts / 64);
  return MCX_OK;
}

static int shard_bins_launch(mcx_graph *g, const StreamLaunch &L, void *d_keys, void *d_counts, uint64_t seg_cap,
                             void *d_ov_keys, void *d_ov_edges, void *d_ov_counts, uint64_t ov_cap, bool spill = false);

extern "C" int mcx_graph_shard_bins_dev(mcx_graph *g, const void *d_stream, uint64_t nbytes, void *d_keys,
                                        void *d_counts, uint64_t seg_cap, void *d_ov_keys, void *d_ov_edges,
                                        void *d_ov_counts, uint64_t ov_cap)
{
  if (!g) return fail(MCX_ERR_ARG, "null graph");
  NO_WIDE(g, "mcx_graph_shard_bins_dev");
  if (g->as_group) return fail(MCX_ERR_ARG, "device-pointer exchange calls take a shard, not the multi-GPU handle");
  if (!nbytes) return MCX_OK;
  StreamLaunch L{(const uint8_t *)d_stream, nbytes, 0, nbytes, nullptr};
  return shard_bins_launch(g, L, d_keys, d_counts, seg_cap, d_ov_keys, d_ov_edges, d_ov_counts, ov_cap);
}

static int shard_bins_launch(mcx_graph *g, const StreamLaunch &L, void *d_keys, void *d_counts, uint64_t seg_cap,
                             void *d_ov_keys, void *d_ov_edges, void *d_ov_counts, uint64_t ov_cap, bool spill)
{
  if (!L.code && ((uintptr_t)L.stream & 15) != 0) return fail(MCX_ERR_ARG, "stream must be 16-byte aligned");
  if (g->t.lb1 + g->t.lbo > 11) return fail(MCX_ERR_ARG, "too many (owner, region) bins");
  if (seg_cap >= 0xFFFFFFFFull) return fail(MCX_ERR_ARG, "segment capacity must be below 2^32 tuples");
  HIP_TRY(hipSetDevice(g->device));
  const uint32_t nparts = 1u << g->t.lbo, b1 = 1u << g->t.lb1;
  BinSpec bs{BIN_GLOBAL, nparts, nparts * b1, kShardRep, b1, 1, g->t.lb1, spill ? 1u : 0u};
  BinOut out{(uint64_t *)d_keys, nullptr, (unsigned long long *)d_counts, seg_cap,
             (uint64_t *)d_ov_keys, (uint8_t *)d_ov_edges, (unsigned long long *)d_ov_counts, ov_cap};
  if (g->W == 1) launch_bin_stream_t<1, true, false, 2>(g, L, 0, bs, out);
  else launch_bin_stream_t<2, true, false, 2>(g, L, 0, bs, out);
  HIP_TRY(hipGetLastError());
  return MCX_OK;
}

extern "C" int mcx_graph_add_segments_dev(mcx_graph *g, int colour, const void *d_keys, const void *d_counts,
                                          uint32_t nseg, uint64_t seg_cap, uint64_t ntuples)
{
  NO_GROUP(g, "mcx_graph_add_segments_dev");
  if (!g) return fail(MCX_ERR_ARG, "null graph");
  NO_WIDE(g, "mcx_graph_add_segments_dev");
  if (colour < 0 || colour >= g->ncols) return fail(MCX_ERR_ARG, "colour %d out of range", colour);
  if (!nseg) return MCX_OK;
  HIP_TRY(hipSetDevice(g->device));
  int rc = ensure_defer(g);
  if (rc != MCX_OK) return rc;
  if (!g->defer) return fail(MCX_ERR_ARG, "packed segments need the deferred insert path (table too small or defer=0)");
  if (nseg % g->b1) return fail(MCX_ERR_ARG, "segments must cover whole sets of %u regions", g->b1);
  rc = l2_reserve(g, colour, ntuples);
  if (rc != MCX_OK) return rc;
  rc = ensure_l2(g, g->b1, true);
  if (rc != MCX_OK) return rc;
  TupleIn in{(const uint64_t *)d_keys, nullptr, (const unsigned long long *)d_counts, seg_cap, nseg, nseg, nseg};
  BinSpec bs{BIN_SUBLOCAL, 0, g->subs_per_bin, 1, g->nsub, g->b1, 0, 0};
  BinOut out{g->l2_keys, nullptr, g->l2_cnt, g->cap2, nullptr, nullptr, nullptr, 0};
  DISPATCH_WC(g, launch_split_regions, g, in, colour, bs, out);
  HIP_TRY(hipGetLastError());
  g->pending_l2 += ntuples;
  return MCX_OK;
}

static const uint32_t kSuperkRep = 8;

extern "C" int mcx_superk_supported(int kmer_size) { return kmer_size >= kSuperkMinK && kmer_size <= 63 && (kmer_size & 1); }
extern "C" int mcx_superk_record_bytes(int kmer_size) { return mcx_superk_supported(kmer_size) ? 16 * words_for_k(kmer_size) : 0; }

extern "C" uint32_t mcx_superk_owner(const uint64_t *key_words, int kmer_size, int nparts)
{
  uint32_t lbo = 0;
  while ((1 << lbo) < nparts) lbo++;
  return words_for_k(kmer_size) == 1 ? superk_owner(0, key_words[0], kmer_size, lbo) : superk_owner(key_words[0], key_words[1], kmer_size, lbo);
}

extern "C" int mcx_graph_superk_layout(mcx_graph *g, int nparts, uint64_t positions_per_call, uint32_t *segs_per_owner,
                                       uint64_t *seg_cap)
{
  NO_GROUP(g, "mcx_graph_superk_layout");
  if (!g) return fail(MCX_ERR_ARG, "null graph");
  NO_WIDE(g, "mcx_graph_superk_layout");
  if (nparts < 1 || nparts > 32 || (nparts & (nparts - 1))) return fail(MCX_ERR_ARG, "shards must be a power of two <= 32");
  if (segs_per_owner) *segs_per_owner = kSuperkRep;
  if (seg_cap) *seg_cap = positions_per_call / 4 / ((uint64_t)nparts * kSuperkRep) + 4096;
  return MCX_OK;
}

extern "C" int mcx_graph_superk_bins_dev(mcx_graph *g, const void *d_stream, uint64_t nbytes, int nparts, void *d_recs,
                                         void *d_counts, uint64_t seg_cap)
{
  NO_GROUP(g, "mcx_graph_superk_bins_dev");
  if (!g) return fail(MCX_ERR_ARG, "null graph");
  NO_WIDE(g, "mcx_graph_superk_bins_dev");
  if (!mcx_superk_supported(g->k)) return fail(MCX_ERR_ARG, "super-k-mer records need an odd k in %d..63 (got %d)", kSuperkMinK, g->k);
  if (nparts < 1 || nparts > 32 || (nparts & (nparts - 1))) return fail(MCX_ERR_ARG, "shards must be a power of two <= 32");
  if (((uintptr_t)d_stream & 15) != 0) return fail(MCX_ERR_ARG, "stream must be 16-byte aligned");
  if (!nbytes) return MCX_OK;
  HIP_TRY(hipSetDevice(g->device));
  uint32_t lbo = 0;
  while ((1 << lbo) < nparts) lbo++;
  StreamLaunch L{(const uint8_t *)d_stream, nbytes, 0, nbytes, nullptr};
  const StreamArgs a = make_args(g, L);
  const uint64_t nt = a.ntiles > a.tile0 ? a.ntiles - a.tile0 : 0;
  if (!nt) return MCX_OK;
  SuperkOut out{d_recs, (unsigned long long *)d_counts, seg_cap, lbo, kSuperkRep, nullptr, nullptr, nullptr, 0};
  SpanGuard sp(g, "k_stream_superk");
  const dim3 grid((unsigned)std::min<uint64_t>(nt, (uint64_t)g->grid));
  if (g->W == 1) hipLaunchKernelGGL((k_stream_superk<1, false>), grid, dim3(kThreads), 0, g->stream, a, out);
  else hipLaunchKernelGGL((k_stream_superk<2, false>), grid, dim3(kThreads), 0, g->stream, a, out);
  HIP_TRY(hipGetLastError());
  return MCX_OK;
}

static int superk_bins_launch(mcx_graph *g, const StreamLaunch &L, const SuperkOut &out)
{
  if (!L.code && ((uintptr_t)L.stream & 15) != 0) return fail(MCX_ERR_ARG, "stream must be 16-byte aligned");
  HIP_TRY(hipSetDevice(g->device));
  const StreamArgs a = make_args(g, L);
  const uint64_t nt = a.ntiles > a.tile0 ? a.ntiles - a.tile0 : 0;
  if (!nt) return MCX_OK;
  SpanGuard sp(g, "k_stream_superk");
  const dim3 grid((unsigned)std::min<uint64_t>(nt, (uint64_t)g->grid));
  if (g->W == 1) {
    if (a.code) hipLaunchKernelGGL((k_stream_superk<1, true>), grid, dim3(kThreads), 0, g->stream, a, out);
    else hipLaunchKernelGGL((k_stream_superk<1, false>), grid, dim3(kThreads), 0, g->stream, a, out);
  } else {
    if (a.code) hipLaunchKernelGGL((k_stream_superk<2, true>), grid, dim3(kThreads), 0, g->stream, a, out);
    else hipLaunchKernelGGL((k_stream_superk<2, false>), grid, dim3(kThreads), 0, g->stream, a, out);
  }
  HIP_TRY(hipGetLastError());
  return MCX_OK;
}

template <int W, bool ONECOL> static void launch_superk_bin(mcx_graph *g, SuperkIn in, int colour, BinSpec bs, BinOut out)
{
  const uint64_t nunits = (in.seg_cap + kSkChunk - 1) / kSkChunk * in.nseg;
  InsertSink<W, ONECOL> is{g->t, (uint32_t)colour};
  const size_t lds512 = ((sizeof(BinLds<W, 512, false>) + 15) & ~(size_t)15) + kSkMapBytes;
  const size_t ldsmax = ((sizeof(BinLds<W, kMaxBins, false>) + 15) & ~(size_t)15) + kSkMapBytes;
  static bool once_dev[64] = {false};
  bool &once = once_dev[g->device & 63];
// ... 220 lines not shown
{
#if defined(__x86_64__)
  static const int level = getenv("MCX_NO_AVX2") ? 0 : (__builtin_cpu_supports("avx512bw") && __builtin_cpu_supports("avx512vl") && !getenv("MCX_NO_AVX512")) ? 2
                           : __builtin_cpu_supports("avx2") ? 1 : 0;
  if (level == 2) { pack_block_avx512(src, n, code, inv); return; }
  if (level == 1) { pack_block_avx2(src, n, code, inv); return; }
#endif
  for (size_t i = 0; i < n; i += 16) pack16_swar(src + i, code + i / 16, inv + i / 16);
}

extern "C" uint64_t mcx_pack_reads_host(const uint8_t *bases, const uint64_t *off, uint64_t nreads, uint32_t *code, uint16_t *inv, uint64_t cap_pos, int fused)
{
  const uint64_t L = nreads ? off[nreads] - off[0] + nreads : 0, total = kCarry + ((L + 63) & ~63ull);
  if (total > cap_pos) return 0;
  if (fused) {
    if (!pack_reads_available()) return 0;
#if defined(__x86_64__)
    uint8_t sep[kCarry];
    memset(sep, '\n', sizeof(sep));
    pack_block(sep, (size_t)kCarry, code, inv);
    const PackReads PR{bases, off, 0, nreads, kCarry, false, 0, 0};
    uint64_t p = kCarry;
    for (uint64_t step = 64; p < total; step = total > (1u << 24) ? (1u << 18) : step * 3 % 8191 / 64 * 64 + 64) {
      const uint64_t q = std::min(total, p + step);
      pack_reads_avx512(PR, p, q, code, inv);
      p = q;
    }
#endif
    return total;
  }
  std::vector<uint8_t> txt(total, (uint8_t)'\n');
  for (uint64_t i = 0, p = kCarry; i < nreads; i++) {
    const uint64_t len = off[i + 1] - off[i];
    memcpy(txt.data() + p, bases + off[i], len);
    p += len + 1;
  }
  pack_block(txt.data(), (size_t)total, code, inv);
  return total;
}

extern "C" void mcx_pack_bases(const uint8_t *src, uint64_t n, uint32_t *code, uint16_t *inv)
{
  pack_block(src, (size_t)n, code, inv);
}

static int stage_threads()
{
  static const int n = [] {
    const char *e = getenv("MCX_STAGE_THREADS");
    const int hw = (int)std::thread::hardware_concurrency();
    const int v = e ? atoi(e) : std::max(1, std::min(24, hw / 2));
    return v < 1 ? 1 : v > 64 ? 64 : v;
  }();
  return n;
}

struct StageTiming {
  double wait = 0, prep = 0, pack = 0, submit = 0; uint64_t chunks = 0, flushes = 0;
  ~StageTiming() { if (chunks && getenv("MCX_STAGE_TIMING")) fprintf(stderr, "[stage] %llu chunks: wait for buffer %.1f ms, prepare %.1f ms, pack %.1f ms, copy + launches %.1f ms (%llu background flushes)\n",
                                          (unsigned long long)chunks, wait * 1e3, prep * 1e3, pack * 1e3, submit * 1e3, (unsigned long long)flushes); }
};
static StageTiming g_stage_timing;

static int flush_if_device_idle(mcx_graph *g, int starved = -1 )
{
  static const int mode_env = [] { const char *e = getenv("MCX_IDLE_FLUSH"); return e ? atoi(e) : 1; }();
  if (mode_env == 3 && !(g->idle_base || g->pending >= g->defer_tuples / 4 * 3)) return MCX_OK;
  const int mode = mode_env == 3 ? 2 : mode_env;
  const bool on = mode != 0;
  if (!on || !g->defer || g->group || g->nsets != 1 || !g->pending || g->pending_l2 || g->set_colour.empty() || g->set_colour[0] < 0) return MCX_OK;
  const uint32_t G = std::min(flush_group(g), g->l2_regions);
  if (G >= g->b1) return MCX_OK;
  const uint32_t ngroups = (g->b1 + G - 1) / G;
  if (mode != 2 && g->pending / ngroups < std::max<uint64_t>(g->defer_tuples / 8 / ngroups, 1ull << 24)) return MCX_OK;
  if (mode != 2 && starved == 0) return MCX_OK;
  if (mode != 2 && starved < 0 && hipStreamQuery(g->stream) != hipSuccess) { (void)hipGetLastError(); return MCX_OK; }
  const uint32_t r0 = g->idle_next * G < g->b1 ? g->idle_next * G : 0;
  g->idle_next = (r0 / G + 1) % ngroups;
  g_stage_timing.flushes++;
  const uint32_t ng = std::min(G, g->b1 - r0);
  const int colour = g->set_colour[0];
  g->l2_off = 0;
  TupleIn in{g->l1_keys + (uint64_t)r0 * g->cap1 * g->W, nullptr, g->l1_cnt + r0, g->cap1, ng * g->rep1, ng, g->b1};
  BinSpec bs{BIN_SUBLOCAL, 0, g->subs_per_bin, 1, ng * g->subs_per_bin, ng, 0, r0};
  BinOut out{g->l2_keys, nullptr, g->l2_cnt, g->cap2, nullptr, nullptr, nullptr, 0};
  DISPATCH_WC(g, launch_split_regions, g, in, colour, bs, out);
  HIP_TRY(hipGetLastError());
  DISPATCH_WC(g, launch_lds_insert_t, g, colour, r0 * g->subs_per_bin, ng * g->subs_per_bin);
  HIP_TRY(hipGetLastError());
  HIP_TRY(hipMemset2DAsync(g->l1_cnt + r0, (size_t)g->b1 * 8, 0, (size_t)ng * 8, g->rep1, g->stream));
  if (g->idle_mark.size() != ngroups) g->idle_mark.assign(ngroups, g->idle_base);
  g->idle_mark[r0 / G] = g->idle_base + g->pending;
  const uint64_t base = *std::min_element(g->idle_mark.begin(), g->idle_mark.end());
  const uint64_t freed = base - g->idle_base;
  g->idle_base = base;
  g->pending -= std::min(g->pending, freed);
  g->set_pending[0] -= std::min(g->set_pending[0], freed);
  return MCX_OK;
}

static bool stage_packed()
{
  static const bool packed = [] { const char *e = getenv("MCX_PACKED"); return !e || atoi(e) != 0; }();
  return packed;
}
static uint64_t stage_inv_at() { return (((kCarry + kStageBytes + 64) / 16 * 4) + 63) & ~63ull; }
static uint64_t stage_off_region()
{
  if (!stage_packed()) return kCarry + kStageBytes + 256;
  return (stage_inv_at() + (kCarry + kStageBytes + 64) / 16 * 2 + 255) & ~255ull;
}

static int ensure_stage(mcx_graph *g)
{
  if (g->stage_alloc) return MCX_OK;
  const uint64_t bytes = stage_off_region() + (kStageBytes / 16 + 2) * sizeof(uint64_t);
  for (int i = 0; i < mcx_graph::kStageBufs; i++) {
    if (!g->h_stage[i]) HIP_TRY(hipHostMalloc((void **)&g->h_stage[i], bytes, hipHostMallocDefault));
    if (!g->d_stage[i]) HIP_TRY(hipMalloc((void **)&g->d_stage[i], bytes));
    if (!g->ev[i]) HIP_TRY(hipEventCreateWithFlags(&g->ev[i], hipEventDisableTiming));
    if (!g->ev_copy[i]) HIP_TRY(hipEventCreateWithFlags(&g->ev_copy[i], hipEventDisableTiming));
    if (!g->ev_wait0[i]) HIP_TRY(hipEventCreate(&g->ev_wait0[i]));
    if (!g->ev_wait1[i]) HIP_TRY(hipEventCreate(&g->ev_wait1[i]));
  }
  if (!g->cstream) HIP_TRY(hipStreamCreateWithFlags(&g->cstream, hipStreamNonBlocking));
  g->stage_alloc = bytes;
  return MCX_OK;
}

static int add_reads_qh(mcx_graph *g, int colour, const uint8_t *bases, const uint8_t *quals,
                        const uint64_t *off, uint64_t nreads, uint8_t fq, uint8_t hp);
static int add_reads_must_exist(mcx_graph *g, int colour, const uint8_t *bases, const uint8_t *quals,
                                const uint64_t *off, uint64_t nreads, uint8_t fq, uint8_t hp);

static int add_reads_packed(mcx_graph *g, int colour, const uint8_t *bases, const uint64_t *off, uint64_t nreads,
                            unsigned char *d_flags)
{
  const uint64_t off_region = stage_off_region();
  const uint64_t max_offs = kStageBytes / 16;
  const uint64_t cap_pos = kCarry + kStageBytes + 64;
  const uint64_t inv_at = stage_inv_at();
  uint32_t carry_code[kCarry / 16];
  uint16_t carry_inv[kCarry / 16];
  for (uint64_t i = 0; i < kCarry / 16; i++) { carry_code[i] = 0; carry_inv[i] = 0xFFFF; }
  uint64_t r = 0, r_pos = 0;
  const int T = stage_threads();
  const bool fused = pack_reads_available();

  struct Job {
    int b = 0;
    uint8_t *hs = nullptr;
    uint32_t *hcode = nullptr;
    uint16_t *hinv = nullptr;
    uint64_t *hoff = nullptr;
    uint64_t r0 = 0, nwhole = 0, L = 0, Lp = 0, total = 0;
    long long piece_of = -1;
    uint64_t piece_from = 0, piece_data = 0;
    std::atomic<uint64_t> next_run{0};
    std::function<void(int)> fn;
    bool async = false;
  } jobs[2];

  auto plan = [&](Job &J) -> int {
    J.b = g->cur;
    g->cur = (g->cur + 1) % mcx_graph::kStageBufs;
    const double tq0 = now_s();
    HIP_TRY(hipEventSynchronize(g->ev[J.b]));
    g_stage_timing.wait += now_s() - tq0;
    J.hs = g->h_stage[J.b];
    J.hcode = reinterpret_cast<uint32_t *>(J.hs);
    J.hinv = reinterpret_cast<uint16_t *>(J.hs + inv_at);
// ... 1559 lines not shown
```

### mccortex_amd/csrc/mcx_defer.h

```cpp
#pragma once
#include "mcx_kernels.h"

namespace mcx {

enum : int { BIN_OWNER = 0, BIN_GROUP = 1, BIN_SUBLOCAL = 2, BIN_GLOBAL = 3 };

struct BinSpec {
  int mode;
  uint32_t nparts;
  uint32_t nlocal;
  uint32_t rep;
  uint32_t nout;
  uint32_t seg_mod;
  uint32_t lb1;
  uint32_t region0;
};

__device__ __forceinline__ uint32_t out_seg(const BinSpec &bs, uint32_t ob0, uint32_t b)
{
  if (bs.mode == BIN_GLOBAL)
    return ((((b >> bs.lb1) * bs.rep + blockIdx.x % bs.rep) << bs.lb1) | (b & ((1u << bs.lb1) - 1u)));
  return ob0 + b;
}

struct BinOut {
  uint64_t *keys;
  uint8_t *edges;
  unsigned long long *counts;
  uint64_t cap;
  uint64_t *ov_keys;
  uint8_t *ov_edges;
  unsigned long long *ov_counts;
  uint64_t ov_cap;
};

#define MCX_LDS_AS __attribute__((address_space(3)))

#ifdef MCX_PHASES
__device__ unsigned long long g_phase[3][8];
#define MCX_PH_DECL unsigned long long ph_t = wall_clock64(), ph_acc[8] = {0, 0, 0, 0, 0, 0, 0, 0};
#define MCX_PH(i) { const unsigned long long n_ = wall_clock64(); ph_acc[i] += n_ - ph_t; ph_t = n_; }
#define MCX_PH_COUNT ph_acc[7]++;
#define MCX_PH_DUMP(kid) { if (threadIdx.x == 0) for (int i_ = 0; i_ < 8; i_++) atomicAdd(&g_phase[kid][i_], ph_acc[i_]); }
#else
#define MCX_PH_DECL
#define MCX_PH(i)
#define MCX_PH_COUNT
#define MCX_PH_DUMP(kid)
#endif
constexpr int kMaxBins = 2048;
constexpr uint64_t kQMask = (1ull << 56) - 1;

template <int W> __device__ __forceinline__ Kmer<W> tuple_pack(const Kmer<W> &q, uint32_t e)
{
  Kmer<W> t = q;
  t.w[0] |= (uint64_t)e << 56;
  return t;
}
template <int W> __device__ __forceinline__ Kmer<W> tuple_q(const Kmer<W> &t)
{
  Kmer<W> q = t;
  q.w[0] &= kQMask;
  return q;
}

constexpr int kRounds = 2;
constexpr int kStage = kTile / kRounds;

template <int T_, int TILE_, int R_ = kRounds> struct Geo {
  static constexpr int kT = T_, kTileG = TILE_, kRoundsG = R_, kStageG = TILE_ / R_;
};
using Geo256 = Geo<kThreads, kTile>;

template <int W, int NB, bool FULL, class G = Geo256> struct BinLds {
  using geo = G;
  uint64_t skey[G::kStageG * W];
  unsigned long long gbase[NB];
  uint32_t cnt[NB + 64];
  uint32_t rnk[NB + 64];
  uint32_t off[NB + 64];
  uint32_t wsum[G::kT / 64];
  uint16_t sbin[G::kStageG];
  uint8_t se[FULL ? G::kStageG : 16];
};

__device__ __forceinline__ uint32_t tid_now()
{
  uint32_t t = threadIdx.x;
  asm volatile("" : "+v"(t));
  return t;
}

template <int NB, int T = kThreads> struct BinRes { unsigned long long g0[(NB + T - 1) / T]; };

template <class LDS, int NB>
__device__ __forceinline__ void bin_reserve(LDS &L, const BinSpec &bs, const BinOut &out, uint32_t ob0, BinRes<NB, LDS::geo::kT> &res,
                                            bool trash_beyond = false)
{
  constexpr int kT = LDS::geo::kT;
  const int tid = threadIdx.x;
  __syncthreads();
  {
    constexpr int PERB = NB / kT;
    static_assert(NB % kT == 0, "bins per thread");
    uint32_t c[PERB], x = 0;
#pragma unroll
    for (int i = 0; i < PERB; i++) {
      const uint32_t b = (uint32_t)tid * PERB + i;
      c[i] = b < bs.nlocal ? L.cnt[b] : 0;
      x += c[i];
    }
    const uint32_t mine = x;
#pragma unroll
    for (int d = 1; d < 64; d <<= 1) {
      const uint32_t y = __shfl_up(x, d, 64);
      if ((tid & 63) >= d) x += y;
    }
    if ((tid & 63) == 63) L.wsum[tid >> 6] = x;
    __syncthreads();
    uint32_t before = 0, total = 0;
#pragma unroll
    for (int w = 0; w < kT / 64; w++) {
      const uint32_t ws = L.wsum[w];
      if (w < (tid >> 6)) before += ws;
      total += ws;
    }
    uint32_t o = before + x - mine;
#pragma unroll
    for (int i = 0; i < PERB; i++) {
      const uint32_t b = (uint32_t)tid * PERB + i;
      if (b < bs.nlocal) L.off[b] = o;
      o += c[i];
    }
    if (tid < 64) L.off[bs.nlocal + tid] = tid && trash_beyond ? (uint32_t)LDS::geo::kTileG : total;
  }
  __syncthreads();
#pragma unroll
  for (int q = 0; q < (NB + kT - 1) / kT; q++) {
    const uint32_t b = (uint32_t)q * kT + tid;
    res.g0[q] = 0;
    if (b < bs.nlocal) {
      const uint32_t c = L.cnt[b];
      if (c) res.g0[q] = atomicAdd(&out.counts[out_seg(bs, ob0, b)], (unsigned long long)c);
    }
  }
}

constexpr unsigned long long kDstMask = (1ULL << 48) - 1;

template <class LDS, int NB>
__device__ __forceinline__ void bin_commit(LDS &L, const BinSpec &bs, const BinOut &out, uint32_t ob0, const BinRes<NB, LDS::geo::kT> &res)
{
  constexpr int kT = LDS::geo::kT;
#pragma unroll
  for (int q = 0; q < (NB + kT - 1) / kT; q++) {
    const uint32_t b = (uint32_t)q * kT + threadIdx.x;
    if (b < bs.nlocal) {
      const uint32_t o0 = L.off[b], o1 = L.off[b + 1];
      const unsigned long long g0 = res.g0[q];
      const unsigned long long room = out.cap > g0 ? out.cap - g0 : 0;
      const uint32_t lim = o0 + (uint32_t)min((unsigned long long)(o1 - o0), room);
      const unsigned long long dst = ((unsigned long long)out_seg(bs, ob0, b) * out.cap + g0 - o0) & kDstMask;
      L.gbase[b] = dst | ((unsigned long long)lim << 48);
    }
  }
}

template <class LDS> __device__ __forceinline__ uint32_t bin_rank(LDS &L, uint32_t local)
{
  return L.off[local] + atomicAdd(&L.rnk[local], 1u);
}

template <int W, bool FULL, class LDS>
__device__ __forceinline__ void bin_place(LDS &L, int round, uint32_t p, uint32_t local, const Kmer<W> &t, uint32_t e)
{
  constexpr uint32_t kSt = LDS::geo::kStageG;
  if ((int)(p / kSt) != round) return;
  const uint32_t q = p % kSt;
  L.skey[q * W] = t.w[0];
  if (W == 2) L.skey[q * W + 1] = t.w[W - 1];
  L.sbin[q] = (uint16_t)local;
  if (FULL) L.se[q] = (uint8_t)e;
}

template <int W, bool ONECOL, bool FULL, int SH, class LDS>
__device__ __forceinline__ void bin_writeout(LDS &L, int round, const BinSpec &bs, const BinOut &out, uint32_t ob0,
                                             uint32_t region_of_seg, const InsertSink<W, ONECOL> &isink,
                                             uint32_t &novel, uint32_t &full)
{
  __syncthreads();
  const uint32_t n = L.off[bs.nlocal];
  constexpr uint32_t kSt = LDS::geo::kStageG;
  const uint32_t lo = (uint32_t)round * kSt;
  const uint32_t hi = min(n, lo + kSt);
  auto emit = [&](uint32_t p, uint32_t b, unsigned long long gb, uint64_t t0, uint64_t t1) {
    if (p < (uint32_t)(gb >> 48)) {
      const uint64_t at = (gb + p) & kDstMask;
      uint64_t *kd = out.keys + at * W;
      kd[0] = t0;
      if (W == 2) kd[1] = t1;
      if (FULL) out.edges[at] = L.se[p - lo];
    } else if (FULL || bs.mode == BIN_OWNER) {
      full = 2;
    } else {
      Kmer<W> tq;
      tq.w[0] = t0;
      if (W == 2) tq.w[W - 1] = t1;
      const uint32_t e = (uint32_t)(tq.w[0] >> 56);
      const Kmer<W> qq = tuple_q<W>(tq);
      const uint32_t lbq = lbq_of(isink.t);
      if (SH == 2) {
        const Kmer<W> key = key_unquot<W>(qq, lbq, b ^ mix_g(region_mix<W>(qq), lbq));
        const uint32_t owner = b >> bs.lb1;
        const unsigned long long pos = atomicAdd(&out.ov_counts[owner], 1ULL);
        if (pos < out.ov_cap) {
          uint64_t *kd = out.ov_keys + ((uint64_t)owner * out.ov_cap + pos) * W;
          kd[0] = key.w[0];
          if (W == 2) kd[1] = key.w[W - 1];
          out.ov_edges[(uint64_t)owner * out.ov_cap + pos] = (uint8_t)e;
        } else {
          const unsigned long long sp_cap = bs.region0 ? out.ov_counts[bs.nparts + 1] : 0;
          const unsigned long long sp = sp_cap ? atomicAdd(&out.ov_counts[bs.nparts], 1ULL) : 0;
          if (sp < sp_cap) {
            const uint64_t at = (uint64_t)bs.nparts * out.ov_cap + sp;
            uint64_t *kd = out.ov_keys + at * W;
            kd[0] = key.w[0];
            if (W == 2) kd[1] = key.w[W - 1];
            out.ov_edges[at] = (uint8_t)e;
          } else {
            full = 2;
          }
        }
      } else {
        table_mark_written(isink.t);
        table_count_fallback(isink.t);
        const uint32_t region = bs.mode == BIN_GROUP ? b : region_of_seg;
        const Kmer<W> key = key_unquot<W>(qq, lbq, r_of<W>(isink.t, region, qq));
        const uint64_t slot = key_slot<W>(isink.t, key);
        const uint64_t cur = *key_ptr_t<W, ONECOL>(isink.t, slot);
        probe_insert<W, ONECOL>(isink.t, key, slot, cur, 0, e, isink.col, novel, full);
      }
    }
  };
  for (uint32_t p = lo + threadIdx.x; p < hi; p += LDS::geo::kT) {
    const uint32_t q = p - lo;
    const uint32_t b = L.sbin[q];
    emit(p, b, L.gbase[b], L.skey[q * W], W == 2 ? L.skey[q * W + W - 1] : 0);
  }
  if (round + 1 < LDS::geo::kRoundsG) __syncthreads();
}

struct LaneWin { uint32_t a2, a1, a0, r2, r1, r0; };
__device__ __forceinline__ uint32_t pairrev32(uint32_t x)
{
  const uint32_t r = __builtin_bitreverse32(x);
  return ((r >> 1) & 0x55555555u) | ((r & 0x55555555u) << 1);
}
__device__ __forceinline__ LaneWin lane_win(const uint32_t *s_code, uint32_t pl, int k)
{
  LaneWin w;
  w.a2 = s_code[pl >> 4];
  w.a1 = s_code[(pl >> 4) + 1];
  w.a0 = s_code[(pl >> 4) + 2];
  const uint32_t c2 = pairrev32(~w.a0), c1 = pairrev32(~w.a1), c0 = pairrev32(~w.a2);
  const int t = 66 - 2 * k;
  if (t < 32) {
    w.r2 = (c2 << t) | (c1 >> (32 - t));
    w.r1 = (c1 << t) | (c0 >> (32 - t));
    w.r0 = c0 << t;
  } else {
    const uint64_t x = (((uint64_t)c1 << 32) | c0) << (t - 32);
    w.r2 = (uint32_t)(x >> 32);
    w.r1 = (uint32_t)x;
    w.r0 = 0;
  }
  return w;
}

template <int W, bool ONECOL>
__device__ __noinline__ void foreign_insert(const InsertSink<W, ONECOL> &isink, Kmer<W> key, uint32_t e,
                                            uint32_t &novel, uint32_t &full)
{
  table_mark_written(isink.t);
  table_count_foreign(isink.t);
  const uint64_t slot = key_slot<W>(isink.t, key);
// ... 145 lines not shown
          local = (local & valid) | (trash & ~valid);
          tle[j] = local | (e << 24);
        } else {
          uint32_t G;
          Kmer<W> q;
          if (W == 1) {
            const uint64_t kk = sel >> key_sh;
            q.w[0] = kk >> lbq;
            G = ((uint32_t)kk ^ (region_mix<W>(q) >> mix_sh)) & qmask;
          } else {
            uint32_t r;
            q = key_quot<W>(key, lbq, r);
            G = r ^ mix_g(region_mix<W>(q), lbq);
          }
          local = SH == 1 ? (G & lmask) : G;
          tk[j] = tuple_pack<W>(q, e);
          if (SH == 1 && valid && (G >> t_lb1) != t_part) {
            foreign_insert<W, ONECOL>(isink, key, e, n_novel, full);
            local = trash;
          }
          local = (local & valid) | (trash & ~valid);
          tle[j] = local;
        }
        const uint32_t arr_now = atomicAdd(&L.cnt[local], 1u);
        if (j > 0) { tle[j - 1] |= arr_prev << 12; asm volatile("" : "+v"(tle[j - 1])); }
        arr_prev = arr_now;
        if (j == kPosPerLane - 1) tle[j] |= arr_now << 12;
        if (W == 1) asm volatile("" : "+v"(tle[j]), "+v"(tk[j].w[0]));
        else asm volatile("" : "+v"(tle[j]), "+v"(tk[j].w[0]), "+v"(tk[j].w[W - 1]));
        if (W == 2) {
          fw.w[0] = ((fw.w[0] << 2) | (fw.w[W - 1] >> 62)) & top_mask;
          fw.w[W - 1] = (fw.w[W - 1] << 2) | nuc_next;
          rc.w[W - 1] = (rc.w[W - 1] >> 2) | (rc.w[0] << 62);
          rc.w[0] = (rc.w[0] >> 2) | ((uint64_t)(3u - nuc_next) << first_shift);
        }
      }
    }
    MCX_PH(1)
    BinRes<NB, T> res;
    bin_reserve<LDS, NB>(L, bs, out, ob0, res, !FULL);
    MCX_PH(2)
#pragma unroll
    for (int j = 0; j < kPosPerLane; j++) {
      tle[j] += L.off[tle[j] & 0xfffu] << 12;
      if ((j & 3) == 3) asm volatile("" : "+v"(tle[j - 3]), "+v"(tle[j - 2]), "+v"(tle[j - 1]), "+v"(tle[j]));
    }
    bin_commit<LDS, NB>(L, bs, out, ob0, res);
    MCX_PH(3)
    for (int round = 0; round < kRounds; round++) {
#pragma unroll
      for (int j = 0; j < kPosPerLane; j++)
        bin_place<W, FULL, LDS>(L, round, FULL ? (tle[j] >> 12) & 0xfffu : tle[j] >> 12, tle[j] & 0xfffu, tk[j], tle[j] >> 24);
      bin_writeout<W, ONECOL, FULL, SH, LDS>(L, round, bs, out, ob0, 0, isink, n_novel, full);
      if (round == 0) { MCX_PH(4) } else { MCX_PH(5) }
    }
  }
  MCX_PH_DUMP(0)

  block_add(&a.ctr->kmers, n_kmers);
  block_add(&a.ctr->contigs, n_contigs);
  block_add(&a.ctr->novel, n_novel);
  if (full == 1) a.ctr->full = 1;
  if (full == 2) a.ctr->bin_over = 1;
  if (a.flag && n_contigs) *a.flag = 1;
}

struct TupleIn {
  const uint64_t *keys;
  const uint8_t *edges;
  const unsigned long long *counts;
  uint64_t seg_cap;
  uint32_t nseg;
  uint32_t seg_group, seg_stride;
  uint32_t set_rep;
  uint8_t set_map[32];
};
__device__ __forceinline__ uint64_t tuple_seg_phys(const TupleIn &in, uint32_t seg)
{
  uint32_t q = seg / in.seg_group;
  if (in.set_rep) q = (uint32_t)in.set_map[q / in.set_rep] * in.set_rep + q % in.set_rep;
  return (uint64_t)q * in.seg_stride + seg % in.seg_group;
}

template <int W, bool ONECOL, int NB, bool IN_FULL, bool SHARD, int T = kThreads, int R = kRounds, int P = 16>
__global__ __launch_bounds__(T, (W == 1 || T > kThreads ? 4 : 3)) void k_tuples_bin(TupleIn in, BinSpec bs, BinOut out,
                                                                         InsertSink<W, ONECOL> isink_arg, Counters *ctr)
{
  extern __shared__ __attribute__((aligned(16))) unsigned char dyn_lds[];
  using LDS = BinLds<W, NB, false, Geo<T, T * P, R>>;
  constexpr int kThreads = T, kTile = T * P;
  LDS &L = *reinterpret_cast<LDS *>(dyn_lds);
  __shared__ InsertSink<W, ONECOL> isink;
  if (threadIdx.x == 0) isink = isink_arg;
  __syncthreads();
  const uint32_t t_spb = isink_arg.t.spb, t_lb1 = isink_arg.t.lb1, t_lbq = isink_arg.t.lb1 + isink_arg.t.lbo, t_part = isink_arg.t.part;
  const int tid = threadIdx.x;
  uint32_t n_novel = 0, full = 0;
  const uint64_t chunks_per_seg = (in.seg_cap + kTile - 1) / kTile;
  const bool xcd = bs.mode == BIN_SUBLOCAL && gridDim.x % 8 == 0 && bs.seg_mod % 8 == 0 && in.nseg % bs.seg_mod == 0;
  const uint32_t group = xcd ? blockIdx.x % 8 : 0;
  const uint32_t nseg_g = xcd ? in.nseg / 8 : in.nseg;
  constexpr uint32_t kWin = 2;
  const uint32_t bins_g = xcd ? bs.seg_mod / 8 : 1;
  const uint32_t reps = xcd ? in.nseg / bs.seg_mod : 1;
  const uint32_t win_segs = kWin * reps;
  const uint32_t nwin = (bins_g + kWin - 1) / kWin;
  const uint64_t nchunks = xcd ? (uint64_t)nwin * chunks_per_seg * win_segs : chunks_per_seg * nseg_g;
  const uint64_t v0 = xcd ? blockIdx.x / 8 : blockIdx.x, vstep = xcd ? gridDim.x / 8 : gridDim.x;
  const uint32_t lmask = (1u << t_lb1) - 1u;
  MCX_PH_DECL
  for (uint64_t v = v0; v < nchunks; v += vstep) {
    uint32_t seg;
    uint64_t start;
    if (xcd) {
      const uint64_t per_win = chunks_per_seg * win_segs;
      const uint32_t win = (uint32_t)(v / per_win);
      const uint64_t rem = v % per_win;
      const uint32_t s = (uint32_t)(rem % win_segs);
      const uint32_t rgi = win * kWin + s % kWin;
      if (rgi >= bins_g) continue;
      seg = (s / kWin) * bs.seg_mod + group + 8 * rgi;
      start = (rem / win_segs) * kTile;
    } else {
      seg = (uint32_t)(v % nseg_g);
      start = (v / nseg_g) * kTile;
    }
    const uint64_t pseg = tuple_seg_phys(in, seg);
    uint64_t cnt = in.counts ? (uint64_t)in.counts[pseg] : in.seg_cap;
    if (cnt > in.seg_cap) cnt = in.seg_cap;
    if (start >= cnt) continue;
    const uint32_t n = (uint32_t)min((uint64_t)kTile, cnt - start);
    const uint32_t lregion = bs.mode == BIN_SUBLOCAL ? seg % bs.seg_mod : 0;
    const uint32_t region = bs.region0 + lregion;
    const uint32_t ob0 = (bs.mode == BIN_SUBLOCAL ? lregion * t_spb : 0) + (blockIdx.x % bs.rep) * bs.nout;
    MCX_PH(6) MCX_PH_COUNT
    __syncthreads();
    for (uint32_t b = tid; b < bs.nlocal + 64; b += kThreads) { L.cnt[b] = 0; L.rnk[b] = 0; }
    __syncthreads();
    MCX_PH(0)
    const uint32_t trash = bs.nlocal + 1u + ((uint32_t)tid & 31u);
    const uint64_t *kin = in.keys + (pseg * in.seg_cap + start) * W;
    const uint8_t *ein = IN_FULL ? in.edges + pseg * in.seg_cap + start : nullptr;
    constexpr int PER = kTile / kThreads;
    Kmer<W> tk[PER];
    uint32_t ev[IN_FULL ? PER : 1], loc[PER];
    uint32_t okm = 0;
    const bool vec16 = !IN_FULL && (((uintptr_t)in.keys & 15u) == 0) && (W == 2 || (in.seg_cap & 1u) == 0);
    if (vec16) {
      const ulonglong2 *kin2 = reinterpret_cast<const ulonglong2 *>(kin);
#pragma unroll
      for (int q = 0; q < PER; q += (W == 1 ? 2 : 1)) {
        const uint32_t p = (uint32_t)(q / (W == 1 ? 2 : 1)) * kThreads + tid;
        const uint32_t i = W == 1 ? 2 * p : p;
        tk[q].w[0] = 0; tk[q + (W == 1 ? 1 : 0)].w[W - 1] = 0;
        if (i < n) {
          const ulonglong2 x = kin2[p];
          okm |= 1u << q;
          if (W == 1) {
            tk[q].w[0] = x.x;
            tk[q + (W == 1 ? 1 : 0)].w[0] = x.y;
            if (i + 1 < n) okm |= 2u << q;
          } else {
            tk[q].w[0] = x.x;
            tk[q].w[W - 1] = x.y;
          }
        }
      }
    } else {
#pragma unroll
    for (int q = 0; q < PER; q++) {
      const uint32_t i = (uint32_t)q * kThreads + tid;
      if (i < n) okm |= 1u << q;
      tk[q].w[0] = 0; if (W == 2) tk[q].w[W - 1] = 0;
      if (IN_FULL) ev[q] = 0;
      if (i < n) {
        tk[q].w[0] = kin[(uint64_t)i * W];
        if (W == 2) tk[q].w[W - 1] = kin[(uint64_t)i * W + 1];
        if (IN_FULL) ev[q] = ein[i];
      }
    }
    }
#pragma unroll
    for (int q = 0; q < PER; q++) {
      const uint32_t i = (uint32_t)q * kThreads + tid;
      uint32_t hb;
      if (IN_FULL) {
        uint32_t r;
        const uint32_t lbq = t_lbq;
        const Kmer<W> key = tk[q];
        const Kmer<W> qq = key_quot<W>(key, lbq, r);
        const uint32_t G = r ^ mix_g(region_mix<W>(qq), lbq);
        hb = 0;
        loc[q] = G & lmask;
        tk[q] = tuple_pack<W>(qq, ev[q]);
        if (SHARD && (okm >> q & 1u) && (G >> t_lb1) != t_part) {
          foreign_insert<W, ONECOL>(isink, key, ev[q], n_novel, full);
          okm &= ~(1u << q);
        }
      } else {
        hb = sub_hash<W>(tuple_q<W>(tk[q]));
        loc[q] = __umulhi(hb, t_spb);
      }
      if (loc[q] >= bs.nlocal) loc[q] = bs.nlocal - 1;
      loc[q] = (okm >> q & 1u) ? loc[q] : trash;
      atomicAdd(&L.cnt[loc[q]], 1u);
      (void)i;
    }
    MCX_PH(1)
    BinRes<NB, T> res;
    bin_reserve<LDS, NB>(L, bs, out, ob0, res, true);
    MCX_PH(2)
#pragma unroll
    for (int q = 0; q < PER; q++)
      loc[q] |= bin_rank<LDS>(L, loc[q]) << 16;
    bin_commit<LDS, NB>(L, bs, out, ob0, res);
    MCX_PH(3)
    for (int round = 0; round < R; round++) {
#pragma unroll
      for (int q = 0; q < PER; q++)
        bin_place<W, false, LDS>(L, round, loc[q] >> 16, loc[q] & 0xffffu, tk[q], 0);
      bin_writeout<W, ONECOL, false, 0, LDS>(L, round, bs, out, ob0, region, isink, n_novel, full);
      if (round == 0) { MCX_PH(4) } else { MCX_PH(5) }
    }
  }
  MCX_PH_DUMP(1)
  block_add(&ctr->novel, n_novel);
  if (full == 1) ctr->full = 1;
  if (full == 2) ctr->bin_over = 1;
}

template <int W> struct LdsCfg {
  static constexpr int kThreads = 512;
  static constexpr int kMinWaves = 4;
  static constexpr bool kPrefetch = true;
  static constexpr int kBatch = 4;
};
template <int W> struct LdsQueue { static constexpr uint32_t kTuples = W == 1 ? 1856 : 288; };

__device__ __forceinline__ uint32_t lds_phys1(uint32_t slot)
{
  return slot ^ ((slot >> 4) & 2u);
}
constexpr uint32_t kLdsVal1 = 4096;

template <int W>
__device__ __forceinline__ bool lds_apply(unsigned long long *lds, const Kmer<W> &key, uint32_t bucket, uint32_t e,
                                          uint32_t &n_novel, uint32_t &full)
{
  const unsigned long long want = key.w[0] | kFlag;
  uint32_t steps = 0;
  if constexpr (W == 1) {
    typedef unsigned long long u64x2 __attribute__((ext_vector_type(2)));
    typedef MCX_LDS_AS const volatile u64x2 lds_cv;
    uint32_t b = bucket;
    for (;;) {
      const uint32_t sw = (b >> 3) & 1u;
      unsigned long long *b0 = lds + b * kBucket;
      unsigned long long *h0 = b0 + 2 * sw, *h1 = b0 + 2 * (sw ^ 1u);
      const u64x2 lo = *(lds_cv *)h0;
      const u64x2 hi = *(lds_cv *)h1;
      unsigned long long *hit = nullptr, *emp = nullptr;
      if (hi.y == 0) emp = h1 + 1;
      if (hi.x == 0) emp = h1;
      if (lo.y == 0) emp = h0 + 1;
      if (lo.x == 0) emp = h0;
      if (hi.y == want) hit = h1 + 1;
      if (hi.x == want) hit = h1;
      if (lo.y == want) hit = h0 + 1;
      if (lo.x == want) hit = h0;
      if (hit) {
        unsigned long long *val = hit + kLdsVal1;
        const unsigned long long old = atomicAdd(val, 256ULL);
        if (e & ~(uint32_t)old) atomicOr(val, (unsigned long long)e);
        return true;
      }
      if (emp) {
        if (atomicCAS(emp, 0ULL, want) == 0) {
          unsigned long long *val = emp + kLdsVal1;
          n_novel++;
          atomicAdd(val, 256ULL);
          if (e) atomicOr(val, (unsigned long long)e);
          return true;
        }
        if (++steps > (1u << 22)) { full = 1; return true; }
        continue;
      }
      b = (b + 1) & (uint32_t)(Sub<W>::kBuckets - 1);
      if (b == bucket) return false;
    }
  } else {
    constexpr uint32_t kK1 = 1, kV = W;
#define MCX_SP(b_, j_) (lds + (size_t)(b_) * (kBucket * (W + 1)) + (j_) * (W + 1))
    uint32_t b = bucket;
    for (;;) {
      unsigned long long k[kBucket];
#pragma unroll
      for (int j = 0; j < kBucket; j++)
        k[j] = __hip_atomic_load((MCX_LDS_AS unsigned long long *)MCX_SP(b, j), __ATOMIC_RELAXED, __HIP_MEMORY_SCOPE_WORKGROUP);
      int hit = -1, empty = -1;
      bool retry = false;
#pragma unroll
      for (int j = kBucket - 1; j >= 0; j--) {
        if (k[j] == 0) empty = j;
        if ((k[j] & ~kPending) == want) {
// ... 118 lines not shown
    MCX_LD(a, K[2 * (0 * T + tid)]) MCX_LD(b, K[2 * (0 * T + tid) + 1]) MCX_LD(c, V[0 * T + tid])
    MCX_LD(d, K[2 * (1 * T + tid)]) MCX_LD(e, K[2 * (1 * T + tid) + 1]) MCX_LD(f, V[1 * T + tid])
#undef MCX_LD
  }
}

template <int W, bool ONECOL, int T>
__device__ __forceinline__ void slice_fetch(const TableView &t, uint32_t sub, uint32_t col, int tid, SliceRegs &v, bool zeros_known)
{
  if (zeros_known && !((t.touch[1 + (sub >> 5)] >> (sub & 31u)) & 1u)) {
#define MCX_Z(m) { v.m.x = 0; v.m.y = 0; }
    MCX_Z(a) MCX_Z(b) MCX_Z(c) MCX_Z(d) MCX_Z(e) MCX_Z(f) MCX_Z(g) MCX_Z(h)
#undef MCX_Z
    return;
  }
  slice_load<W, ONECOL, T>(t, sub, col, tid, v);
}

template <int W, bool ONECOL, int T>
__device__ __forceinline__ void slice_to_lds(unsigned long long *lds, int tid, const SliceRegs &v)
{
  ulonglong2 *dst = reinterpret_cast<ulonglong2 *>(lds);
  if (ONECOL && W == 1) {
#define MCX_ST(m, q) { const uint32_t ph = lds_phys1((uint32_t)(q * T + tid)); lds[ph] = v.m.x; lds[kLdsVal1 + ph] = v.m.y; }
    MCX_ST(a, 0) MCX_ST(b, 1) MCX_ST(c, 2) MCX_ST(d, 3) MCX_ST(e, 4) MCX_ST(f, 5) MCX_ST(g, 6) MCX_ST(h, 7)
#undef MCX_ST
  } else if (ONECOL) {
#define MCX_ST(m, q) dst[q * T + tid] = make_ulonglong2(v.m.x, v.m.y);
    MCX_ST(a, 0) MCX_ST(b, 1) MCX_ST(c, 2) MCX_ST(d, 3) MCX_ST(e, 4) MCX_ST(f, 5)
#undef MCX_ST
  } else if (W == 1) {
#define MCX_PUT1(q, kv, vv) { const uint32_t ph = lds_phys1(2u * (uint32_t)(q * T + tid)) >> 1; dst[ph] = make_ulonglong2(kv.x, kv.y); dst[kLdsVal1 / 2 + ph] = make_ulonglong2(vv.x, vv.y); }
    MCX_PUT1(0, v.a, v.e) MCX_PUT1(1, v.b, v.f) MCX_PUT1(2, v.c, v.g) MCX_PUT1(3, v.d, v.h)
#undef MCX_PUT1
  } else {
#define MCX_PUT2(j, k0, k1, vv) { const int p = j * T + tid; dst[3 * p] = make_ulonglong2(k0.x, k0.y); dst[3 * p + 1] = make_ulonglong2(vv.x, k1.x); dst[3 * p + 2] = make_ulonglong2(k1.y, vv.y); }
    MCX_PUT2(0, v.a, v.b, v.c) MCX_PUT2(1, v.d, v.e, v.f)
#undef MCX_PUT2
  }
}

template <int W, bool ONECOL, int T>
__device__ __forceinline__ void slice_store(const TableView &t, uint32_t sub, uint32_t col, int tid, const unsigned long long *lds)
{
  const ulonglong2 *src = reinterpret_cast<const ulonglong2 *>(lds);
  const uint64_t s0 = (uint64_t)sub * Sub<W>::kSlots;
  if (ONECOL && W == 1) {
    ulonglong2 *dst = reinterpret_cast<ulonglong2 *>(t.rec + s0 * 2);
#pragma unroll
    for (int q = 0; q < 8; q++) {
      const uint32_t sl = (uint32_t)(q * T + tid), ph = lds_phys1(sl);
      dst[sl] = make_ulonglong2(lds[ph], lds[kLdsVal1 + ph]);
    }
  } else if (ONECOL) {
    ulonglong2 *dst = reinterpret_cast<ulonglong2 *>(t.rec + s0 * (W + 1));
    constexpr int PER = (int)(Sub<W>::kSlots * (W + 1) * 8 / 16 / T);
#pragma unroll
    for (int q = 0; q < PER; q++) {
      dst[q * T + tid] = src[q * T + tid];
    }
  } else if (W == 1) {
    ulonglong2 *K = reinterpret_cast<ulonglong2 *>(t.rec + s0);
    ulonglong2 *V = reinterpret_cast<ulonglong2 *>(t.val + (uint64_t)col * t.VC + s0);
#pragma unroll
    for (int q = 0; q < 4; q++) {
      const uint32_t p = (uint32_t)(q * T + tid), ph = lds_phys1(2u * p) >> 1;
      K[p] = src[ph];
      V[p] = src[kLdsVal1 / 2 + ph];
    }
  } else {
    ulonglong2 *K = reinterpret_cast<ulonglong2 *>(t.rec + s0 * 2);
    ulonglong2 *V = reinterpret_cast<ulonglong2 *>(t.val + (uint64_t)col * t.VC + s0);
#pragma unroll
    for (int j = 0; j < 2; j++) {
      const int p = j * T + tid;
      const ulonglong2 x = src[3 * p], y = src[3 * p + 1], z = src[3 * p + 2];
      K[2 * p] = x;
      K[2 * p + 1] = make_ulonglong2(y.y, z.x);
      V[p] = make_ulonglong2(y.x, z.y);
    }
  }
}

template <int W, bool ONECOL>
__global__ __launch_bounds__(LdsCfg<W>::kThreads, LdsCfg<W>::kMinWaves) void k_lds_insert(TableView t, uint32_t col, BinOut bins,
                                                                       uint32_t sub0, uint32_t nsub, Counters *ctr)
{
  constexpr int kLdsThreads = LdsCfg<W>::kThreads;
  constexpr int kLdsBatch = LdsCfg<W>::kBatch;
  extern __shared__ __attribute__((aligned(16))) unsigned char dyn_lds[];
  unsigned long long *lds = reinterpret_cast<unsigned long long *>(dyn_lds);
  const int tid = threadIdx.x;
  uint32_t n_novel = 0, full = 0;
  unsigned long long *queue = lds + Sub<W>::kSlots * (W + 1);
  constexpr uint32_t kQueueCap = LdsQueue<W>::kTuples;
  __shared__ uint32_t s_nq;
  if (tid == 0) s_nq = 0;

  auto next_bin = [&](uint32_t from) {
    while (from < nsub && bins.counts[from] == 0) from += gridDim.x;
    return from;
  };
  uint32_t bi = next_bin(blockIdx.x);
  SliceRegs v{};
  const bool zeros_known = t.touch && t.touch[0] == 0;
  constexpr bool kPrefetch = LdsCfg<W>::kPrefetch;
  if (kPrefetch && bi < nsub) slice_fetch<W, ONECOL, kLdsThreads>(t, sub0 + bi, col, tid, v, zeros_known);
  auto idx = [&](int q) -> uint32_t { return (uint32_t)q * kLdsThreads + tid; };
  auto load_batch_of = [&](uint32_t bin, uint64_t nfill, uint64_t j0, Kmer<W> (&tk)[kLdsBatch]) {
    const uint64_t *kin = bins.keys + (uint64_t)bin * bins.cap * W;
#pragma unroll
    for (int q = 0; q < kLdsBatch; q++) {
      uint64_t i = j0 + idx(q);
      i = i < nfill ? i : 0;
      tk[q].w[0] = kin[i * W];
      if (W == 2) tk[q].w[W - 1] = kin[i * W + 1];
    }
  };
  constexpr uint64_t kStep = (uint64_t)kLdsThreads * kLdsBatch;
  MCX_PH_DECL
  while (bi < nsub) {
    const uint32_t sub = sub0 + bi;
    const uint32_t region = sub / t.spb;
    MCX_PH(6) MCX_PH_COUNT
    uint64_t n = bins.counts[bi];
    if (n > bins.cap) n = bins.cap;
    const uint32_t nb = next_bin(bi + gridDim.x);
    __syncthreads();
    MCX_PH(0)
    if (tid == 0) bins.counts[bi] = 0;
    if (!kPrefetch) slice_fetch<W, ONECOL, kLdsThreads>(t, sub, col, tid, v, zeros_known);
    slice_to_lds<W, ONECOL, kLdsThreads>(lds, tid, v);
    __syncthreads();
    MCX_PH(1)

    auto load_batch = [&](uint64_t j0, Kmer<W> (&tk)[kLdsBatch]) { load_batch_of(bi, n, j0, tk); };
    auto unpack = [&](const Kmer<W> &tp, Kmer<W> &key, uint32_t &bucket, uint32_t &e) {
      e = (uint32_t)(tp.w[0] >> 56);
      const Kmer<W> qq = tuple_q<W>(tp);
      const uint32_t m = region_mix<W>(qq);
      key = key_unquot<W>(qq, lbq_of(t), ((t.part << t.lb1) | region) ^ mix_g(m, lbq_of(t)));
      bucket = mix_bucket(m, lbq_of(t), Sub<W>::kBuckets);
    };
    auto apply_slow = [&](const Kmer<W> &key, uint32_t bucket, uint32_t e) {
      if (!lds_apply<W>(lds, key, bucket, e, n_novel, full))
        probe_insert<W, ONECOL>(t, key, ovf_start<W>(t, key), 0, 0, e, col, n_novel, full, true);
    };
    auto apply_batch = [&](uint64_t j0, const Kmer<W> (&tk)[kLdsBatch]) {
#pragma unroll
      for (int q = 0; q < kLdsBatch; q++)
        if (j0 + idx(q) < n) {
          Kmer<W> key;
          uint32_t bucket, e;
          unpack(tk[q], key, bucket, e);
          if (!lds_try<W>(lds, key, bucket, e, n_novel)) {
            const uint32_t qi = atomicAdd(&s_nq, 1u);
            if (qi < kQueueCap) {
              queue[qi * W] = tk[q].w[0];
              if (W == 2) queue[qi * W + 1] = tk[q].w[W - 1];
            } else {
              apply_slow(key, bucket, e);
            }
          }
        }
    };
    auto run = [&](auto has_next) {
      Kmer<W> ta[kLdsBatch], tb[kLdsBatch];
      load_batch(0, ta);
      load_batch(kStep, tb);
      if (decltype(has_next)::value) slice_fetch<W, ONECOL, kLdsThreads>(t, sub0 + nb, col, tid, v, zeros_known);
      for (uint64_t j0 = 0; j0 < n; j0 += 2 * kStep) {
        apply_batch(j0, ta);
        load_batch(j0 + 2 * kStep, ta);
        apply_batch(j0 + kStep, tb);
        load_batch(j0 + 3 * kStep, tb);
      }
    };
    if (kPrefetch && nb < nsub) run(std::true_type{}); else run(std::false_type{});
    MCX_PH(2)
    __syncthreads();
    MCX_PH(3)
    {
      const uint32_t nq = min(s_nq, kQueueCap);
      for (uint32_t i = tid; i < nq; i += kLdsThreads) {
        Kmer<W> tp, key;
        uint32_t bucket, e;
        tp.w[0] = queue[i * W];
        if (W == 2) tp.w[W - 1] = queue[i * W + 1];
        unpack(tp, key, bucket, e);
        apply_slow(key, bucket, e);
      }
      __syncthreads();
      if (tid == 0) s_nq = 0;
    }
    MCX_PH(4)
    slice_store<W, ONECOL, kLdsThreads>(t, sub, col, tid, lds);
    if (tid == 0 && t.touch) atomicOr(&t.touch[1 + (sub >> 5)], 1u << (sub & 31u));
    bi = nb;
    MCX_PH(5)
  }
  MCX_PH_DUMP(2)
  block_add(&ctr->novel, n_novel);
  if (full) ctr->full = 1;
}

}
```

### mccortex_amd/csrc/mcx_kernels.h

```cpp
#pragma once
#include <hip/hip_runtime.h>
#include <stdint.h>
#include "mcx_kmer.h"

namespace mcx {

constexpr int kBucket = 4;
template <int W> struct Sub {
  static constexpr int kShift = W == 1 ? 12 : 11;
  static constexpr uint64_t kSlots = 1ull << kShift;
  static constexpr uint32_t kBuckets = (uint32_t)(kSlots / kBucket);
};
__host__ __device__ constexpr int sub_shift_for_words(int W) { return W == 1 ? 12 : 11; }

struct TableView {
  uint64_t *rec;
  uint64_t nslots;
  uint64_t nmain;
  uint32_t lb1;
  uint32_t lbo;
  uint32_t part;
  uint32_t spb;
  uint32_t S;
  uint32_t max_probe;
  uint32_t KS;
  uint32_t VS;
  uint64_t *val;
  uint64_t VC;
  uint32_t *touch;
};
constexpr int kTouchHdr = 32;
__device__ __forceinline__ void table_mark_written(const TableView &t)
{
  if (t.touch) t.touch[0] = 1u;
}
__device__ __forceinline__ void table_count_slow(unsigned long long *ctr)
{
  const unsigned long long act = __builtin_amdgcn_ballot_w64(true);
  const uint32_t lane = __builtin_amdgcn_mbcnt_hi((uint32_t)(act >> 32), __builtin_amdgcn_mbcnt_lo((uint32_t)act, 0u));
  if (lane == 0) atomicAdd(ctr, (unsigned long long)__popcll(act));
}
__device__ __forceinline__ void table_count_fallback(const TableView &t)
{
  if (t.touch) table_count_slow(reinterpret_cast<unsigned long long *>(t.touch) - 4);
}
__device__ __forceinline__ void table_count_foreign(const TableView &t)
{
  if (t.touch) table_count_slow(reinterpret_cast<unsigned long long *>(t.touch) - 3);
}
__device__ __forceinline__ bool table_full_flagged(const TableView &t)
{
  return t.touch && __hip_atomic_load(t.touch - 2, __ATOMIC_RELAXED, __HIP_MEMORY_SCOPE_AGENT) != 0u;
}
__device__ __forceinline__ void table_flag_full(const TableView &t)
{
  if (t.touch) __hip_atomic_store(t.touch - 2, 1u, __ATOMIC_RELAXED, __HIP_MEMORY_SCOPE_AGENT);
}
__device__ __forceinline__ uint64_t *key_ptr(const TableView &t, uint64_t slot) { return t.rec + slot * t.KS; }
__device__ __forceinline__ uint64_t *val_ptr(const TableView &t, uint64_t slot, uint32_t col)
{
  return t.val + slot * t.VS + (uint64_t)col * t.VC;
}
template <int W, bool ONECOL> __device__ __forceinline__ uint64_t *key_ptr_t(const TableView &t, uint64_t slot)
{
  return t.rec + slot * (ONECOL ? (uint64_t)(W + 1) : (uint64_t)W);
}
template <int W, bool ONECOL> __device__ __forceinline__ uint64_t *val_ptr_t(const TableView &t, uint64_t slot, uint32_t col)
{
  return ONECOL ? t.rec + slot * (uint64_t)(W + 1) + W : t.val + (uint64_t)col * t.VC + slot;
}

template <int W> __device__ __host__ __forceinline__ uint32_t region_mix(const Kmer<W> &q)
{
  uint32_t x = (uint32_t)q.w[0] ^ (uint32_t)(q.w[0] >> 32);
  if (W == 2) x ^= ((uint32_t)q.w[W - 1] ^ (uint32_t)(q.w[W - 1] >> 32)) * 0x85EBCA6Bu;
  if (W > 2)
    for (int i = 1; i < W; i++) x ^= ((uint32_t)q.w[i] ^ (uint32_t)(q.w[i] >> 32)) * (0x85EBCA6Bu + 0x9E3779B2u * (uint32_t)(i - 1));
  return x * 0x9E3779B1u;
}
template <int W> __device__ __host__ __forceinline__ uint32_t sub_hash(const Kmer<W> &q)
{
  uint32_t x = (uint32_t)q.w[0] + (uint32_t)(q.w[0] >> 32) * 0xC2B2AE35u;
  if (W == 2) x += (uint32_t)q.w[W - 1] * 0x27D4EB2Fu + (uint32_t)(q.w[W - 1] >> 32) * 0x165667B1u;
  if (W > 2)
    for (int i = 1; i < W; i++) x += (uint32_t)q.w[i] * (0x27D4EB2Fu + 0x3C6EF372u * (uint32_t)(i - 1)) + (uint32_t)(q.w[i] >> 32) * (0x165667B1u + 0x7F4A7C16u * (uint32_t)(i - 1));
  x *= 0x85EBCA6Bu;
  x ^= x >> 15;
  return x * 0x2C1B3C6Du;
}
__device__ __host__ __forceinline__ uint32_t mix_g(uint32_t m, uint32_t lbq) { return (uint32_t)(((uint64_t)m << lbq) >> 32); }
__device__ __host__ __forceinline__ uint32_t mix_bucket(uint32_t m, uint32_t lbq, uint32_t nbuckets)
{
  return (m >> (22u - lbq)) & (nbuckets - 1u);
}
template <int W> __device__ __host__ __forceinline__ Kmer<W> key_quot(const Kmer<W> &key, uint32_t lb1 , uint32_t &r)
{
  Kmer<W> q = key;
  if (W == 1) {
    r = (uint32_t)key.w[0] & ((1u << lb1) - 1u);
    q.w[0] = key.w[0] >> lb1;
    return q;
  }
  r = 0;
  if (lb1) {
    r = (uint32_t)key.w[W - 1] & ((1u << lb1) - 1u);
    if (W == 2) q.w[W - 1] = (key.w[W - 1] >> lb1) | (key.w[0] << (64 - lb1));
    if (W > 2)
      for (int i = W - 1; i >= 1; i--) q.w[i] = (key.w[i] >> lb1) | (key.w[i - 1] << (64 - lb1));
    q.w[0] = key.w[0] >> lb1;
  }
  return q;
}
template <int W> __device__ __host__ __forceinline__ Kmer<W> key_unquot(const Kmer<W> &q, uint32_t lb1, uint32_t r)
{
  Kmer<W> key = q;
  if (W == 1) {
    key.w[0] = (q.w[0] << lb1) | r;
    return key;
  }
  if (lb1) {
    key.w[0] = q.w[0] << lb1;
    if (W == 2) { key.w[0] |= q.w[W - 1] >> (64 - lb1); key.w[W - 1] = q.w[W - 1] << lb1; }
    if (W > 2)
      for (int i = 0; i < W; i++) key.w[i] = (q.w[i] << lb1) | (i + 1 < W ? q.w[i + 1] >> (64 - lb1) : 0ull);
    key.w[W - 1] |= r;
  }
  return key;
}
__device__ __host__ __forceinline__ uint32_t lbq_of(const TableView &t) { return t.lb1 + t.lbo; }

struct TableAddr { uint32_t G, region, sub, bucket; };
template <int W> __device__ __forceinline__ TableAddr addr_of(const TableView &t, const Kmer<W> &q, uint32_t r)
{
  const uint32_t b = sub_hash<W>(q);
  const uint32_t lbq = lbq_of(t), m = region_mix<W>(q);
  TableAddr a;
  a.G = r ^ mix_g(m, lbq);
  a.region = a.G & ((1u << t.lb1) - 1u);
  a.sub = a.region * t.spb + __umulhi(b, t.spb);
  a.bucket = mix_bucket(m, lbq, Sub<W>::kBuckets);
  return a;
}
template <int W> __device__ __forceinline__ uint32_t key_owner(const TableView &t, const Kmer<W> &key)
{
  uint32_t r;
  const Kmer<W> q = key_quot<W>(key, lbq_of(t), r);
  return (r ^ mix_g(region_mix<W>(q), lbq_of(t))) >> t.lb1;
}
template <int W> __device__ __forceinline__ uint32_t r_of(const TableView &t, uint32_t region, const Kmer<W> &q)
{
  return ((t.part << t.lb1) | region) ^ mix_g(region_mix<W>(q), lbq_of(t));
}
template <int W> __device__ __forceinline__ uint64_t key_slot(const TableView &t, const Kmer<W> &key)
{
  uint32_t r;
  const Kmer<W> q = key_quot<W>(key, lbq_of(t), r);
  const TableAddr a = addr_of<W>(t, q, r);
  return ((uint64_t)a.sub << Sub<W>::kShift) + (uint64_t)a.bucket * kBucket;
}

constexpr int kMmer = 13;
constexpr uint32_t kMmerMask = (1u << (2 * kMmer)) - 1u;
constexpr int kSuperkMinK = kMmer + 16;

MCX_HD uint32_t mmer_hash(uint32_t c)
{
  const uint32_t x = c * 0x9E3779B1u;
  return x ^ (x >> 15);
}
MCX_HD uint32_t owner_of_minimizer(uint32_t min_hash, uint32_t lbo)
{
  return lbo ? ((min_hash * 0x85EBCA6Bu) ^ (min_hash >> 13)) * 0xC2B2AE35u >> (32u - lbo) : 0u;
}

MCX_HD uint32_t superk_owner(uint64_t w0, uint64_t w1, int k, uint32_t lbo)
{
  uint32_t best = 0xFFFFFFFFu;
  for (int p = 0; p + kMmer <= k; p++) {
    const int sh = 2 * (k - kMmer - p);
    const uint64_t low = sh >= 64 ? (w0 >> (sh - 64)) : (sh ? (w1 >> sh) | (w0 << (64 - sh)) : w1);
    const uint32_t f = (uint32_t)low & kMmerMask;
    uint32_t r = 0;
    for (int i = 0; i < kMmer; i++) r |= (3u - ((f >> (2 * i)) & 3u)) << (2 * (kMmer - 1 - i));
    const uint32_t h = mmer_hash(f < r ? f : r);
    best = h < best ? h : best;
  }
  return owner_of_minimizer(best, lbo);
}


struct OwnerSpec {
  uint32_t mode;
  uint32_t lbo;
  uint32_t part;
  int k;
};
template <int W> __device__ __forceinline__ bool owner_is_me(const TableView &t, const OwnerSpec &os, const Kmer<W> &key)
{
  if (os.mode == 2) return W > 2 ? true : superk_owner(W == 1 ? 0ULL : key.w[0], key.w[W - 1], os.k, os.lbo) == os.part;
  if (os.mode == 1) return key_owner<W>(t, key) == t.part;
  return true;
}

struct Counters {
  unsigned long long novel;
  unsigned long long kmers;
  unsigned long long contigs;
  unsigned long long full;
  unsigned long long bin_over;
  unsigned long long good_reads, bad_reads;
  unsigned long long absent;
  unsigned long long binned;
};

__device__ __forceinline__ void block_add(unsigned long long *counter, unsigned long long v)
{
  __shared__ unsigned long long s_sum;
  if (threadIdx.x == 0) s_sum = 0;
  __syncthreads();
  if (v) atomicAdd(&s_sum, v);
  __syncthreads();
  if (threadIdx.x == 0 && s_sum) atomicAdd(counter, s_sum);
// ... 1084 lines not shown
```

### mccortex_amd/graph.py

```python
import ctypes as C
import os

import numpy as np

from . import _build

MCX_OK, MCX_ERR_ARG, MCX_ERR_NODEVICE, MCX_ERR_NOMEM, MCX_ERR_FULL, MCX_ERR_HIP, MCX_ERR_SINK = 0, -1, -2, -3, -4, -5, -6

_LIB = None

SYMBOLS = [
    "mcx_last_error", "mcx_version", "mcx_device_count", "mcx_device_memory", "mcx_graph_create", "mcx_graph_create_multi", "mcx_graph_ndevices",
    "mcx_graph_create_shard", "mcx_graph_shard_layout", "mcx_graph_shard_bins_dev", "mcx_graph_add_segments_dev",
    "mcx_graph_key_owner", "mcx_graph_insert_tuple_segments_dev", "mcx_graph_add_records", "mcx_graph_kmer_covg", "mcx_graph_covg_histogram", "mcx_sort_records",
    "mcx_records_sorted", "mcx_graph_intersect_finish", "mcx_superk_supported", "mcx_superk_record_bytes", "mcx_superk_owner", "mcx_graph_checksum", "mcx_records_checksum",
    "mcx_graph_superk_layout", "mcx_graph_superk_bins_dev", "mcx_graph_add_superk_dev", "mcx_graph_destroy",
    "mcx_graph_reset", "mcx_graph_configure", "mcx_graph_profile", "mcx_graph_capacity", "mcx_graph_add_reads", "mcx_graph_add_reads_pcr", "mcx_graph_pcr_reset", "mcx_graph_add_stream_dev",
    "mcx_graph_partition_stream_dev", "mcx_graph_insert_tuples_dev", "mcx_key_owner", "mcx_graph_sync",
    "mcx_graph_nkmers", "mcx_graph_device_stats", "mcx_graph_stream", "mcx_graph_export",
    "mcx_kmer_from_str", "mcx_kmer_canonical", "mcx_kmer_hash", "mcx_pack_bases", "mcx_pack_reads_host", "mcx_pack_stream_dev", "mcx_graph_add_packed_dev",
    "mcx_ubench_stream", "mcx_ubench_random_rmw", "mcx_graph_insert_stats", "mcx_multi_exchange_bytes", "mcx_graph_hashtest", "mcx_hashtest_func", "mcx_debug_probe",
    "mcx_graph_infer_edges", "mcx_graph_infer_edges_dev", "mcx_graph_unitig_stats", "mcx_graph_clean",
]


class McxError(RuntimeError):
    def __init__(self, code, msg):
        super().__init__("mcx error %d: %s" % (code, msg))
        self.code = code


class LoadStats(C.Structure):
    _fields_ = [(n, C.c_uint64) for n in (
        "num_se_reads", "num_good_reads", "num_bad_reads", "total_bases_read",
        "total_bases_loaded", "contigs_parsed", "num_kmers_loaded", "num_kmers_novel",
        "num_pe_reads", "num_dup_se_reads", "num_dup_pe_pairs")]

    def as_dict(self):
        return {n: int(getattr(self, n)) for n, _ in self._fields_}


class RecordStats(C.Structure):
    _fields_ = [("nkmers_read", C.c_uint64), ("nkmers_loaded", C.c_uint64), ("nkmers_novel", C.c_uint64),
                ("first_oversized", C.c_int64), ("first_zero_covg", C.c_int64), ("first_edges_no_covg", C.c_int64)]

    def __init__(self):
        super().__init__(0, 0, 0, -1, -1, -1)

    def as_dict(self):
        return {n: int(getattr(self, n)) for n, _ in self._fields_}


class CleanStats(C.Structure):
    _fields_ = [(n, C.c_uint64) for n in ("num_tips", "num_tip_kmers", "num_low_covg_unitigs", "num_low_covg_unitig_kmers",
                                          "num_tip_and_low_unitigs", "num_tip_and_low_unitig_kmers", "nkmers_before",
                                          "nkmers_removed")]

    def as_dict(self):
        return {n: int(getattr(self, n)) for n, _ in self._fields_}


CLEAN_NBINS = 1000
RECORDS_MUST_EXIST = 1
INFER_POP, INFER_PRESENCE_COVG = 1, 2
SINK_FN = C.CFUNCTYPE(C.c_int, C.c_void_p, C.c_void_p, C.c_size_t)


def lib():
    global _LIB
    if _LIB is not None:
        return _LIB
    try:
        import torch
    except ImportError:
        pass
    path = os.environ.get("MCX_LIB") or _build.LIB
    if not os.path.exists(path):
        raise RuntimeError("HIP extension missing: %s (run __graft_entry__.build())" % path)
    L = C.CDLL(path)
    vp, u64p = C.c_void_p, C.POINTER(C.c_uint64)
    L.mcx_last_error.restype = C.c_char_p
    L.mcx_version.restype = C.c_char_p
    L.mcx_device_count.restype = C.c_int
    L.mcx_graph_create.argtypes = [C.POINTER(vp), C.c_int, C.c_int, C.c_uint64, C.c_int]
    L.mcx_graph_create_shard.argtypes = [C.POINTER(vp), C.c_int, C.c_int, C.c_uint64, C.c_int, C.c_int, C.c_int]
    L.mcx_graph_create_multi.argtypes = [C.POINTER(vp), C.c_int, C.c_int, C.c_uint64, C.POINTER(C.c_int), C.c_int]
    L.mcx_graph_ndevices.argtypes = [vp]
    L.mcx_graph_shard_layout.argtypes = [vp, C.c_uint64, C.POINTER(C.c_uint32), u64p, u64p]
    L.mcx_graph_shard_bins_dev.argtypes = [vp, vp, C.c_uint64, vp, vp, C.c_uint64, vp, vp, vp, C.c_uint64]
    L.mcx_graph_add_segments_dev.argtypes = [vp, C.c_int, vp, vp, C.c_uint32, C.c_uint64, C.c_uint64]
    L.mcx_graph_insert_tuple_segments_dev.argtypes = [vp, C.c_int, vp, vp, vp, C.c_uint32, C.c_uint64]
    L.mcx_graph_add_records.argtypes = [vp, vp, C.c_uint64, C.c_int, vp, vp, C.c_int, C.c_uint32, C.POINTER(RecordStats)]
    L.mcx_graph_kmer_covg.argtypes = [vp, u64p, u64p]
    L.mcx_graph_insert_stats.argtypes = [vp, vp]
    L.mcx_graph_covg_histogram.argtypes = [vp, u64p, C.c_uint32]
    L.mcx_sort_records.argtypes = [vp, C.c_uint64, C.c_int, C.c_int, C.c_int]
    L.mcx_records_sorted.argtypes = [vp, C.c_uint64, C.c_int, C.c_int, C.c_int, C.POINTER(C.c_int64)]
    L.mcx_graph_intersect_finish.argtypes = [vp, u64p]
    L.mcx_graph_unitig_stats.argtypes = [vp, vp]
    L.mcx_graph_clean.argtypes = [vp, C.c_uint32, C.c_uint32, C.POINTER(CleanStats), vp]
    L.mcx_graph_infer_edges.argtypes = [vp, vp, C.c_uint64, C.c_int, C.c_uint32, u64p]
    L.mcx_graph_infer_edges_dev.argtypes = [vp, vp, C.c_uint64, C.c_int, C.c_uint32, u64p]
    L.mcx_superk_supported.argtypes = [C.c_int]
    L.mcx_superk_record_bytes.argtypes = [C.c_int]
    L.mcx_superk_owner.restype = C.c_uint32
    L.mcx_superk_owner.argtypes = [u64p, C.c_int, C.c_int]
    L.mcx_graph_superk_layout.argtypes = [vp, C.c_int, C.c_uint64, C.POINTER(C.c_uint32), u64p]
    L.mcx_graph_superk_bins_dev.argtypes = [vp, vp, C.c_uint64, C.c_int, vp, vp, C.c_uint64]
    L.mcx_graph_add_superk_dev.argtypes = [vp, C.c_int, vp, vp, C.c_uint32, C.c_uint64, C.c_uint64]
    L.mcx_graph_checksum.argtypes = [vp, u64p, u64p]
    L.mcx_records_checksum.restype = C.c_uint64
    L.mcx_records_checksum.argtypes = [vp, C.c_uint64, C.c_int, C.c_int]
    L.mcx_ubench_stream.argtypes = [C.c_int, C.c_uint64, C.POINTER(C.c_double), C.POINTER(C.c_double), C.POINTER(C.c_double)]
    L.mcx_ubench_random_rmw.argtypes = [C.c_int, C.c_uint64, C.c_uint64, C.POINTER(C.c_double), C.POINTER(C.c_double), C.POINTER(C.c_double)]
    L.mcx_graph_key_owner.restype = C.c_uint32
    L.mcx_graph_key_owner.argtypes = [vp, u64p]
    L.mcx_graph_destroy.argtypes = [vp]
    L.mcx_graph_destroy.restype = None
    L.mcx_graph_reset.argtypes = [vp]
    L.mcx_graph_capacity.argtypes = [vp, u64p, u64p]
    L.mcx_graph_configure.argtypes = [vp, C.c_char_p, C.c_uint64]
    L.mcx_graph_profile.argtypes = [vp, C.c_char_p, C.c_size_t]
    L.mcx_graph_add_reads.argtypes = [vp, C.c_int, vp, vp, vp, C.c_uint64, C.c_uint8, C.c_uint8,
                                      C.POINTER(LoadStats)]
    L.mcx_graph_add_reads_pcr.argtypes = [vp, C.c_int, vp, vp, vp, C.c_uint64, C.c_uint8, C.c_uint8, C.c_uint8,
                                          C.c_int, C.c_int, C.POINTER(LoadStats)]
    L.mcx_graph_pcr_reset.argtypes = [vp]
    L.mcx_graph_add_stream_dev.argtypes = [vp, C.c_int, vp, C.c_uint64]
    L.mcx_pack_stream_dev.argtypes = [vp, C.c_uint64, vp, vp, vp]
    L.mcx_graph_add_packed_dev.argtypes = [vp, C.c_int, vp, vp, C.c_uint64]
    L.mcx_graph_partition_stream_dev.argtypes = [vp, vp, C.c_uint64, C.c_int, C.c_uint64, vp, vp, vp]
    L.mcx_graph_insert_tuples_dev.argtypes = [vp, C.c_int, vp, vp, C.c_uint64]
    L.mcx_graph_hashtest.argtypes = [vp, C.c_uint64, C.c_uint64]
    L.mcx_hashtest_func.argtypes = [C.c_int, C.c_int, C.c_uint64, C.c_uint32, C.POINTER(C.c_uint64)]
    L.mcx_key_owner.restype = C.c_uint32
    L.mcx_key_owner.argtypes = [u64p, C.c_int, C.c_int]
    L.mcx_graph_sync.argtypes = [vp]
    L.mcx_graph_nkmers.argtypes = [vp, u64p]
    L.mcx_graph_device_stats.argtypes = [vp, C.POINTER(LoadStats)]
    L.mcx_graph_stream.restype = vp
    L.mcx_graph_stream.argtypes = [vp]
    L.mcx_graph_export.argtypes = [vp, C.c_int, SINK_FN, vp]
    L.mcx_kmer_from_str.restype = None
    L.mcx_kmer_from_str.argtypes = [C.c_char_p, C.c_int, u64p]
    L.mcx_kmer_canonical.restype = None
    L.mcx_kmer_canonical.argtypes = [u64p, C.c_int, u64p, C.POINTER(C.c_int)]
    L.mcx_kmer_hash.restype = C.c_uint32
    L.mcx_kmer_hash.argtypes = [u64p, C.c_int, C.c_uint32]
    _LIB = L
    return L


def _check(rc):
    if rc != MCX_OK:
        raise McxError(rc, lib().mcx_last_error().decode())


def device_count():
    return lib().mcx_device_count()


def _words(k):
    return (2 * k + 63) // 64


def kmer_from_str(s, k):
    out = (C.c_uint64 * 4)()
    lib().mcx_kmer_from_str(s.encode() if isinstance(s, str) else s, k, out)
    return [int(out[i]) for i in range(_words(k))]


def kmer_canonical(words, k):
    a = (C.c_uint64 * 4)(*words)
    out = (C.c_uint64 * 4)()
    o = C.c_int()
    lib().mcx_kmer_canonical(a, k, out, C.byref(o))
    return [int(out[i]) for i in range(_words(k))], int(o.value)
# ... 149 lines not shown
        return int(n.value)

    @staticmethod
    def _clean_hists(a):
        return {"kmer_covg": a[:CLEAN_NBINS], "unitig_covg": a[CLEAN_NBINS:2 * CLEAN_NBINS], "unitig_len": a[2 * CLEAN_NBINS:]}

    def unitig_stats(self):
        a = np.zeros(3 * CLEAN_NBINS, dtype=np.uint64)
        _check(self.L.mcx_graph_unitig_stats(self.h, _ptr(a)))
        return self._clean_hists(a)

    def clean(self, threshold, tips):
        a = np.zeros(3 * CLEAN_NBINS, dtype=np.uint64)
        st = CleanStats()
        _check(self.L.mcx_graph_clean(self.h, int(threshold), int(tips), C.byref(st), _ptr(a)))
        return st.as_dict(), self._clean_hists(a)

    def kmer_covg(self):
        nk = np.zeros(self.ncols, dtype=np.uint64)
        sc = np.zeros(self.ncols, dtype=np.uint64)
        _check(self.L.mcx_graph_kmer_covg(self.h, nk.ctypes.data_as(C.POINTER(C.c_uint64)), sc.ctypes.data_as(C.POINTER(C.c_uint64))))
        return nk, sc

    def covg_histogram(self, nbins):
        h = np.zeros(nbins, dtype=np.uint64)
        _check(self.L.mcx_graph_covg_histogram(self.h, h.ctypes.data_as(C.POINTER(C.c_uint64)), nbins))
        return h

    def add_packed_dev(self, colour, d_code, d_inv, npos):
        _check(self.L.mcx_graph_add_packed_dev(self.h, colour, _ptr(d_code), _ptr(d_inv), int(npos)))

    def add_stream_dev(self, colour, d_stream, nbytes):
        _check(self.L.mcx_graph_add_stream_dev(self.h, colour, _ptr(d_stream), nbytes))

    def partition_stream_dev(self, d_stream, nbytes, nparts, bin_capacity, d_keys, d_edges, d_counts):
        _check(self.L.mcx_graph_partition_stream_dev(self.h, _ptr(d_stream), nbytes, nparts, bin_capacity,
                                                     _ptr(d_keys), _ptr(d_edges), _ptr(d_counts)))

    def hashtest(self, first, n):
        _check(self.L.mcx_graph_hashtest(self.h, first, n))

    def insert_tuples_dev(self, colour, d_keys, d_edges, n):
        _check(self.L.mcx_graph_insert_tuples_dev(self.h, colour, _ptr(d_keys), _ptr(d_edges), n))

    def shard_layout(self, tuples_per_call):
        segs, cap, ov = C.c_uint32(), C.c_uint64(), C.c_uint64()
        _check(self.L.mcx_graph_shard_layout(self.h, int(tuples_per_call), C.byref(segs), C.byref(cap), C.byref(ov)))
        return int(segs.value), int(cap.value), int(ov.value)

    def shard_bins_dev(self, d_stream, nbytes, d_keys, d_counts, seg_cap, d_ov_keys, d_ov_edges, d_ov_counts, ov_cap):
        _check(self.L.mcx_graph_shard_bins_dev(self.h, _ptr(d_stream), nbytes, _ptr(d_keys), _ptr(d_counts), seg_cap,
                                               _ptr(d_ov_keys), _ptr(d_ov_edges), _ptr(d_ov_counts), ov_cap))

    def add_segments_dev(self, colour, d_keys, d_counts, nseg, seg_cap, ntuples):
        _check(self.L.mcx_graph_add_segments_dev(self.h, colour, _ptr(d_keys), _ptr(d_counts), nseg, seg_cap, int(ntuples)))

    def insert_tuple_segments_dev(self, colour, d_keys, d_edges, d_counts, nseg, seg_cap):
        _check(self.L.mcx_graph_insert_tuple_segments_dev(self.h, colour, _ptr(d_keys), _ptr(d_edges), _ptr(d_counts),
                                                          nseg, seg_cap))

    def key_owner(self, words):
        a = (C.c_uint64 * 2)(*words)
        return int(self.L.mcx_graph_key_owner(self.h, a))

    def sync(self):
        _check(self.L.mcx_graph_sync(self.h))

    @property
    def nkmers(self):
        n = C.c_uint64()
        _check(self.L.mcx_graph_nkmers(self.h, C.byref(n)))
        return int(n.value)

    def device_stats(self):
        st = LoadStats()
        _check(self.L.mcx_graph_device_stats(self.h, C.byref(st)))
        return st

    def insert_stats(self):
        st = (C.c_uint64 * 4)()
        _check(self.L.mcx_graph_insert_stats(self.h, st))
        return dict(zip(("fallback_inserts", "foreign_inserts", "spilled", "flushes"), (int(x) for x in st)))

    @property
    def stream(self):
        return self.L.mcx_graph_stream(self.h)

    def export(self, sorted_=True):
        parts = []

        def sink(_ctx, ptr, n):
            parts.append(C.string_at(ptr, n))
            return 0

        cb = SINK_FN(sink)
        _check(self.L.mcx_graph_export(self.h, 1 if sorted_ else 0, cb, None))
        return b"".join(parts)

    def records(self, sorted_=True):
        body = self.export(sorted_)
        rs = 8 * self.W + 5 * self.ncols
        rec = np.frombuffer(body, dtype=np.uint8).reshape(-1, rs)
        keys = rec[:, :8 * self.W].copy().view(np.uint64).reshape(-1, self.W)
        cov = rec[:, 8 * self.W:8 * self.W + 4 * self.ncols].copy().view(np.uint32).reshape(-1, self.ncols)
        edg = rec[:, 8 * self.W + 4 * self.ncols:].copy()
        return keys, cov, edg


def sort_records(recs, kmer_size, ncols, device=0):
    a = np.frombuffer(bytes(recs), dtype=np.uint8).copy()
    rs = 8 * _words(kmer_size) + 5 * ncols
    assert a.size % rs == 0
    _check(lib().mcx_sort_records(_ptr(a), a.size // rs, kmer_size, ncols, device))
    return a.tobytes()


def records_sorted(recs, kmer_size, ncols, device=0):
    a = np.frombuffer(bytes(recs), dtype=np.uint8)
    rs = 8 * _words(kmer_size) + 5 * ncols
    bad = C.c_int64(-1)
    _check(lib().mcx_records_sorted(_ptr(a), a.size // rs, kmer_size, ncols, device, C.byref(bad)))
    return int(bad.value)


def superk_supported(kmer_size):
    return bool(lib().mcx_superk_supported(kmer_size))


def multi_exchange_bytes(kmer_size, ndevices, capacity_kmers):
    out = C.c_uint64(0)
    L = lib()
    L.mcx_multi_exchange_bytes.argtypes = [C.c_int, C.c_int, C.c_uint64, C.POINTER(C.c_uint64)]
    rc = L.mcx_multi_exchange_bytes(kmer_size, ndevices, capacity_kmers, C.byref(out))
    if rc != 0:
        raise McxError(rc, L.mcx_last_error().decode())
    return int(out.value)


def superk_record_words(kmer_size):
    return int(lib().mcx_superk_record_bytes(kmer_size)) // 8


def superk_owner(words, kmer_size, nparts):
    a = (C.c_uint64 * 2)(*(list(words) + [0])[:2])
    return int(lib().mcx_superk_owner(a, kmer_size, nparts))


def pack_stream_dev(d_stream, nbytes, d_code, d_inv, hip_stream=None):
    _check(lib().mcx_pack_stream_dev(_ptr(d_stream), int(nbytes), _ptr(d_code), _ptr(d_inv), C.c_void_p(hip_stream) if hip_stream else None))


def ubench_stream(nbytes=8 << 30, device=0):
    c, r, w = C.c_double(0), C.c_double(0), C.c_double(0)
    _check(lib().mcx_ubench_stream(device, C.c_uint64(nbytes), C.byref(c), C.byref(r), C.byref(w)))
    return {"copy": c.value, "read": r.value, "write": w.value}


def ubench_random_rmw(table_bytes=16 << 30, nupdates=1 << 29, device=0):
    a, b, c = C.c_double(0), C.c_double(0), C.c_double(0)
    _check(lib().mcx_ubench_random_rmw(device, C.c_uint64(table_bytes), C.c_uint64(nupdates), C.byref(a), C.byref(b), C.byref(c)))
    return {"rmw": a.value, "load16": b.value, "load_rmw": c.value}


def records_checksum(recs, kmer_size, ncols):
    if isinstance(recs, np.ndarray) and recs.dtype == np.uint8 and recs.flags.c_contiguous:
        a = recs
# ... 6 lines not shown
```

Measured before the change: 103.8 billion.

## Add compact sub-table bin formats with rank-select sub addressing for one-word keys

For one-word keys with power-of-two sub-table counts, sub-bin selection now uses low quotient bits XOR a hash mask (rs_pick) instead of a multiply-high hash, which lets those bits be dropped from stored keys. On top of that, opt-in compact L2 bin formats store each tuple as a 32-bit low word plus a 16-bit high word, with edges packed as raw bits or a 5-bit code. This roughly halves staging-bin memory traffic between the split and LDS-insert kernels. The compact formats only run when MCX_L2_COMPACT is set, but the rank-select addressing is on by default whenever its conditions hold. That changes the table layout and adds decode work, including a skip code for the code format.

```diff
diff --git a/include/mcx_gpu.h b/include/mcx_gpu.h
--- a/include/mcx_gpu.h
+++ b/include/mcx_gpu.h
@@ -48,6 +48,7 @@
 int mcx_graph_reset(mcx_graph *g);
 
 int mcx_graph_configure(mcx_graph *g, const char *key, uint64_t value);
+int mcx_graph_l2_format(mcx_graph *g, int reads_only, uint32_t *sx);
 int mcx_graph_profile(mcx_graph *g, char *buf, size_t buflen);
 
 int mcx_graph_create_multi(mcx_graph **out, int kmer_size, int ncols, uint64_t capacity_kmers,
diff --git a/mccortex_amd/csrc/mcx_api.hip b/mccortex_amd/csrc/mcx_api.hip
--- a/mccortex_amd/csrc/mcx_api.hip
+++ b/mccortex_amd/csrc/mcx_api.hip
@@ -187,6 +187,8 @@
   uint64_t set_cap = 0;
   std::vector<int> set_colour;
   std::vector<uint64_t> set_pending;
+  std::vector<uint8_t> set_reads;
+  int l2_compact = 0;
   uint64_t pending = 0;
   uint64_t pending_l2 = 0;
   uint32_t l2_regions = 0;
@@ -235,6 +237,7 @@
 {
   std::fill(g->set_colour.begin(), g->set_colour.end(), -1);
   std::fill(g->set_pending.begin(), g->set_pending.end(), 0);
+  std::fill(g->set_reads.begin(), g->set_reads.end(), (uint8_t)1);
 }
 struct StreamLaunch;
 static int group_submit_stream(mcx_group *G, int idx, const StreamLaunch &L, int colour);
@@ -352,7 +355,15 @@
   g->t.spb = (uint32_t)spb;
   g->t.S = (uint32_t)(g->W + ncols);
   g->t.max_probe = (uint32_t)sub_slots;
+  if (g->W == 1 && !lbo && (spb & (spb - 1)) == 0) {
+    uint32_t lbs = 0;
+    while ((1ull << lbs) < spb) lbs++;
+    const int qb = 2 * kmer_size - (int)lb1 - (int)lbs;
+    const int sx = qb + 5 <= 48 ? 0 : (qb - 1 + 5 <= 48 && spb <= (uint64_t)kMaxBins / 2) ? 1 : -1;
+    if (sx >= 0 && qb - sx >= 16) { g->t.rs = 1; g->t.sbits = lbs + (uint32_t)sx; g->t.sx = (uint32_t)sx; }
+  }
   { const char *e = getenv("MCX_DEFER"); if (e) g->defer = atoi(e) != 0; }
+  { const char *e = getenv("MCX_L2_COMPACT"); if (e) g->l2_compact = atoi(e) != 0; }
   if (g->W > 2) g->defer = false;
   { const char *e = getenv("MCX_GRID_STREAM"); if (e) g->grid_stream = atoi(e); }
   { const char *e = getenv("MCX_REP1"); if (e && atoi(e) >= 1 && atoi(e) <= 4096) { g->rep1 = (uint32_t)atoi(e); g->rep1_forced = true; } }
@@ -459,7 +470,7 @@
   g->n_flushes = 0;
   if (g->h_full) { HIP_TRY(hipStreamSynchronize(g->stream)); *g->h_full = 0; }
   if (g->l1_cnt) HIP_TRY(hipMemsetAsync(g->l1_cnt, 0, (size_t)g->nsets * g->b1 * g->rep1 * 8, g->stream));
-  if (g->l2_cnt) HIP_TRY(hipMemsetAsync(g->l2_cnt, 0, (size_t)g->l2_regions * g->subs_per_bin * 8, g->stream));
+  if (g->l2_cnt) HIP_TRY(hipMemsetAsync(g->l2_cnt, 0, (size_t)g->l2_regions * g->subs_per_bin * 16, g->stream));
   if (g->d_readstrt) HIP_TRY(hipMemsetAsync(g->d_readstrt, 0xff, g->t.nslots * 8, g->stream));
   g->pending = g->pending_l2 = 0;
   g->idle_next = 0; g->idle_base = 0; g->idle_mark.clear();
@@ -615,7 +626,7 @@
   else launch_bin_stream_pk<W, ONECOL, FULL, SH, false>(g, a, nt, colour, bs, out);
 }
 
-template <int W, bool ONECOL, bool IN_FULL, bool SHARD>
+template <int W, bool ONECOL, bool IN_FULL, bool SHARD, int F = kL2Word>
 static void launch_bin_tuples_t(mcx_graph *g, TupleIn in, int colour, BinSpec bs, BinOut out)
 {
   constexpr bool kWide = W == 1 && !IN_FULL;
@@ -630,12 +641,12 @@
   static bool once_dev[64] = {false};
   bool &once = once_dev[g->device & 63];
   if (!once) {
-    allow_lds(k_tuples_bin<W, ONECOL, 512, IN_FULL, SHARD>, sizeof(BinLds<W, 512, false>));
-    allow_lds(k_tuples_bin<W, ONECOL, 1024, IN_FULL, SHARD>, sizeof(BinLds<W, 1024, false>));
-    allow_lds(k_tuples_bin<W, ONECOL, kMaxBins, IN_FULL, SHARD>, sizeof(BinLds<W, kMaxBins, false>));
-    if constexpr (kWide) allow_lds(k_tuples_bin<W, ONECOL, 512, IN_FULL, SHARD, 512>, sizeof(BinLds<W, 512, false, GeoW>));
-    if constexpr (kWide) allow_lds(k_tuples_bin<W, ONECOL, 1024, IN_FULL, SHARD, 512>, sizeof(BinLds<W, 1024, false, GeoW>));
-    if constexpr (kWide) allow_lds(k_tuples_bin<W, ONECOL, kMaxBins, IN_FULL, SHARD, 1024>, sizeof(BinLds<W, kMaxBins, false, Geo<1024, 1024 * 16>>));
+    allow_lds(k_tuples_bin<W, ONECOL, 512, IN_FULL, SHARD, kThreads, kRounds, 16, F>, sizeof(BinLds<W, 512, false>));
+    allow_lds(k_tuples_bin<W, ONECOL, 1024, IN_FULL, SHARD, kThreads, kRounds, 16, F>, sizeof(BinLds<W, 1024, false>));
+    allow_lds(k_tuples_bin<W, ONECOL, kMaxBins, IN_FULL, SHARD, kThreads, kRounds, 16, F>, sizeof(BinLds<W, kMaxBins, false>));
+    if constexpr (kWide) allow_lds(k_tuples_bin<W, ONECOL, 512, IN_FULL, SHARD, 512, kRounds, 16, F>, sizeof(BinLds<W, 512, false, GeoW>));
+    if constexpr (kWide) allow_lds(k_tuples_bin<W, ONECOL, 1024, IN_FULL, SHARD, 512, kRounds, 16, F>, sizeof(BinLds<W, 1024, false, GeoW>));
+    if constexpr (kWide) allow_lds(k_tuples_bin<W, ONECOL, kMaxBins, IN_FULL, SHARD, 1024, kRounds, 16, F>, sizeof(BinLds<W, kMaxBins, false, Geo<1024, 1024 * 16>>));
     once = true;
   }
   SpanGuard sp(g, "k_tuples_bin");
@@ -644,33 +655,40 @@
     if (use_huge) {
       using GeoH = Geo<1024, 1024 * 16>;
       const dim3 gridh((unsigned)std::min<uint64_t>(nchunks, g->grid_split ? gmax : gmax / 4));
-      hipLaunchKernelGGL((k_tuples_bin<W, ONECOL, kMaxBins, IN_FULL, SHARD, 1024>), gridh, dim3(1024), sizeof(BinLds<W, kMaxBins, false, GeoH>), g->stream, in, bs, out, is, g->d_ctr);
+      hipLaunchKernelGGL((k_tuples_bin<W, ONECOL, kMaxBins, IN_FULL, SHARD, 1024, kRounds, 16, F>), gridh, dim3(1024), sizeof(BinLds<W, kMaxBins, false, GeoH>), g->stream, in, bs, out, is, g->d_ctr);
       return;
     }
     if (use_wide) {
       const dim3 gridw((unsigned)std::min<uint64_t>(nchunks, g->grid_split ? gmax : gmax / 2));
       if (bs.nlocal <= 512)
-        hipLaunchKernelGGL((k_tuples_bin<W, ONECOL, 512, IN_FULL, SHARD, 512>), gridw, dim3(512), sizeof(BinLds<W, 512, false, GeoW>), g->stream, in, bs, out, is, g->d_ctr);
+        hipLaunchKernelGGL((k_tuples_bin<W, ONECOL, 512, IN_FULL, SHARD, 512, kRounds, 16, F>), gridw, dim3(512), sizeof(BinLds<W, 512, false, GeoW>), g->stream, in, bs, out, is, g->d_ctr);
       else
-        hipLaunchKernelGGL((k_tuples_bin<W, ONECOL, 1024, IN_FULL, SHARD, 512>), gridw, dim3(512), sizeof(BinLds<W, 1024, false, GeoW>), g->stream, in, bs, out, is, g->d_ctr);
+        hipLaunchKernelGGL((k_tuples_bin<W, ONECOL, 1024, IN_FULL, SHARD, 512, kRounds, 16, F>), gridw, dim3(512), sizeof(BinLds<W, 1024, false, GeoW>), g->stream, in, bs, out, is, g->d_ctr);
       return;
     }
   }
   const dim3 grid((unsigned)std::min<uint64_t>(nchunks, gmax));
   if (bs.nlocal <= 512)
-    hipLaunchKernelGGL((k_tuples_bin<W, ONECOL, 512, IN_FULL, SHARD>), grid, dim3(kThreads), sizeof(BinLds<W, 512, false>), g->stream, in, bs, out, is, g->d_ctr);
+    hipLaunchKernelGGL((k_tuples_bin<W, ONECOL, 512, IN_FULL, SHARD, kThreads, kRounds, 16, F>), grid, dim3(kThreads), sizeof(BinLds<W, 512, false>), g->stream, in, bs, out, is, g->d_ctr);
   else if (bs.nlocal <= 1024)
-    hipLaunchKernelGGL((k_tuples_bin<W, ONECOL, 1024, IN_FULL, SHARD>), grid, dim3(kThreads), sizeof(BinLds<W, 1024, false>), g->stream, in, bs, out, is, g->d_ctr);
+    hipLaunchKernelGGL((k_tuples_bin<W, ONECOL, 1024, IN_FULL, SHARD, kThreads, kRounds, 16, F>), grid, dim3(kThreads), sizeof(BinLds<W, 1024, false>), g->stream, in, bs, out, is, g->d_ctr);
   else
-    hipLaunchKernelGGL((k_tuples_bin<W, ONECOL, kMaxBins, IN_FULL, SHARD>), grid, dim3(kThreads), sizeof(BinLds<W, kMaxBins, false>), g->stream, in, bs, out, is, g->d_ctr);
+    hipLaunchKernelGGL((k_tuples_bin<W, ONECOL, kMaxBins, IN_FULL, SHARD, kThreads, kRounds, 16, F>), grid, dim3(kThreads), sizeof(BinLds<W, kMaxBins, false>), g->stream, in, bs, out, is, g->d_ctr);
 }
 template <int W, bool ONECOL> static void launch_bin_region_stream(mcx_graph *g, const StreamLaunch &L, int colour, BinSpec bs, BinOut out)
 {
   if (g->t.lbo) launch_bin_stream_t<W, ONECOL, false, 1>(g, L, colour, bs, out);
   else launch_bin_stream_t<W, ONECOL, false, 0>(g, L, colour, bs, out);
 }
-template <int W, bool ONECOL> static void launch_split_regions(mcx_graph *g, TupleIn in, int colour, BinSpec bs, BinOut out)
-{ launch_bin_tuples_t<W, ONECOL, false, false>(g, in, colour, bs, out); }
+template <int W, bool ONECOL> static void launch_split_regions(mcx_graph *g, TupleIn in, int colour, BinSpec bs, BinOut out, int fmt)
+{
+  if constexpr (W == 1) {
+    if (fmt == kL2WordRs) return launch_bin_tuples_t<W, ONECOL, false, false, kL2WordRs>(g, in, colour, bs, out);
+    if (fmt == kL2Byte) return launch_bin_tuples_t<W, ONECOL, false, false, kL2Byte>(g, in, colour, bs, out);
+    if (fmt == kL2Code) return launch_bin_tuples_t<W, ONECOL, false, false, kL2Code>(g, in, colour, bs, out);
+  }
+  launch_bin_tuples_t<W, ONECOL, false, false>(g, in, colour, bs, out);
+}
 template <int W, bool ONECOL> static void launch_bin_received(mcx_graph *g, TupleIn in, int colour, BinSpec bs, BinOut out)
 {
   if (g->t.lbo) launch_bin_tuples_t<W, ONECOL, true, true>(g, in, colour, bs, out);
@@ -683,16 +701,47 @@
   return g->l2_keys + off * g->cap2 * g->W;
 }
 
-template <int W, bool ONECOL> static void launch_lds_insert_t(mcx_graph *g, int colour, uint32_t sub0, uint32_t nsub)
+static uint64_t l2_cap_compact(const mcx_graph *g) { return (g->cap2 * 4 / 3 >> g->t.sx) & ~7ull; }
+static BinOut l2_out_at(const mcx_graph *g, uint64_t *p, uint32_t nreg, int fmt)
+{
+  if (fmt < kL2Byte) return BinOut{p, nullptr, nullptr, g->cap2, nullptr, nullptr, nullptr, 0, nullptr, 0};
+  const uint64_t cap = l2_cap_compact(g), nbins = ((uint64_t)nreg * g->subs_per_bin) << g->t.sx;
+  return BinOut{p, nullptr, nullptr, cap, nullptr, nullptr, nullptr, 0,
+                reinterpret_cast<uint16_t *>(reinterpret_cast<uint8_t *>(p) + nbins * cap * 4), g->t.sbits};
+}
+static BinOut l2_out(const mcx_graph *g, uint64_t off, uint32_t nreg, int fmt)
+{
+  BinOut o = l2_out_at(g, l2_ptr(g, off), nreg, fmt);
+  o.counts = g->l2_cnt + (fmt >= kL2Byte ? off << g->t.sx : off);
+  return o;
+}
+static int l2_format(const mcx_graph *g, bool reads_only)
+{
+  if (!g->t.rs) return kL2Word;
+  const int qpb = 2 * g->k - (int)g->t.lb1 - (int)g->t.sbits;
+  if (g->l2_compact && qpb + 8 <= 48) return kL2Byte;
+  if (g->l2_compact && reads_only && qpb + 5 <= 48) return kL2Code;
+  return kL2WordRs;
+}
+static uint32_t l2_bins_per_region(const mcx_graph *g, int fmt) { return fmt >= kL2Byte ? g->subs_per_bin << g->t.sx : g->subs_per_bin; }
+
+template <int W, bool ONECOL, int F> static void launch_lds_insert_f(mcx_graph *g, int colour, uint32_t sub0, uint32_t nsub, const BinOut &bins)
 {
   const size_t lds = Sub<W>::kSlots * (W + 1) * 8 + LdsQueue<W>::kTuples * 8 * W;
   static bool once_dev[64] = {false};
   bool &once = once_dev[g->device & 63];
-  if (!once) { allow_lds(k_lds_insert<W, ONECOL>, lds); once = true; }
-  BinOut bins{l2_ptr(g, g->l2_off), nullptr, g->l2_cnt + g->l2_off, g->cap2, nullptr, nullptr, nullptr, 0};
+  if (!once) { allow_lds(k_lds_insert<W, ONECOL, F>, lds); once = true; }
   SpanGuard sp(g, "k_lds_insert");
-  hipLaunchKernelGGL((k_lds_insert<W, ONECOL>), dim3((unsigned)std::min<uint64_t>(nsub, (uint64_t)(g->grid_insert ? g->grid_insert : g->grid * 4))),
+  hipLaunchKernelGGL((k_lds_insert<W, ONECOL, F>), dim3((unsigned)std::min<uint64_t>(nsub, (uint64_t)(g->grid_insert ? g->grid_insert : g->grid * 4))),
                      dim3(LdsCfg<W>::kThreads), lds, g->stream, g->t, (uint32_t)colour, bins, sub0, nsub, g->d_ctr);
+}
+template <int W, bool ONECOL> static void launch_lds_insert_t(mcx_graph *g, int colour, uint32_t sub0, uint32_t nsub, int fmt, BinOut bins)
+{
+  if constexpr (W == 1) {
+    if (fmt == kL2Byte) return launch_lds_insert_f<W, ONECOL, kL2Byte>(g, colour, sub0, nsub, bins);
+    if (fmt == kL2Code) return launch_lds_insert_f<W, ONECOL, kL2Code>(g, colour, sub0, nsub, bins);
+  }
+  launch_lds_insert_f<W, ONECOL, kL2Word>(g, colour, sub0, nsub, bins);
 }
 
 template <int W, bool ONECOL>
@@ -711,11 +760,12 @@
   g->l1_keys = g->l2_keys = g->l2_base = g->l2_hi = nullptr; g->l1_cnt = g->l2_cnt = nullptr;
   g->cap1 = g->cap2 = 0;
   g->l2_regions = 0;
-  g->set_colour.clear(); g->set_pending.clear();
+  g->set_colour.clear(); g->set_pending.clear(); g->set_reads.clear();
 }
 
 __global__ __launch_bounds__(512) void k_l2_probe(uint64_t *keys, uint64_t cap, uint32_t nregions, uint32_t spb, uint32_t iters,
-                                                  uint32_t jit_mask = 0 )
+                                                  uint32_t jit_mask = 0 ,
+                                                  uint16_t *khi = nullptr)
 {
   const uint32_t region = blockIdx.x % nregions, blk = blockIdx.x / nregions, nblk = gridDim.x / nregions;
   const uint32_t w = threadIdx.x >> 6, l = threadIdx.x & 63u;
@@ -725,7 +775,10 @@
       const uint32_t seg = region * spb + front;
       const uint64_t jit = ((seg * 0x9E3779B1u) >> 8) & jit_mask & ~15u;
       const uint64_t at = (uint64_t)seg * cap + jit + ((uint64_t)it * nblk + blk) * 16u + (l & 15u);
-      if (jit + ((uint64_t)it * nblk + blk) * 16u + 16u <= cap) keys[at] = at;
+      if (jit + ((uint64_t)it * nblk + blk) * 16u + 16u <= cap) {
+        if (khi) { reinterpret_cast<uint32_t *>(keys)[at] = (uint32_t)at; khi[at] = (uint16_t)at; }
+        else keys[at] = at;
+      }
     }
 }
 
@@ -736,6 +789,7 @@
   hipEvent_t e0 = nullptr, e1 = nullptr;
   if (tries > 1 && (hipEventCreate(&e0) != hipSuccess || hipEventCreate(&e1) != hipSuccess)) { (void)hipGetLastError(); tries = 1; }
   const uint32_t iters = (uint32_t)std::max<uint64_t>(8, g->cap2 * g->W / 1024);
+  const int fmt = l2_format(g, true);
   for (int i = 0; i < std::max(tries, 1); i++) {
     if (i > 0) {
       size_t fr = 0, tot = 0;
@@ -748,7 +802,12 @@
     if (tries > 1)
       for (int rep = 0; rep < 2; rep++) {
         (void)hipEventRecord(e0, g->stream);
-        hipLaunchKernelGGL(k_l2_probe, dim3(nreg * 64), dim3(512), 0, g->stream, p, g->cap2 * g->W, nreg, g->subs_per_bin, iters);
+        if (fmt >= kL2Byte) {
+          const BinOut o = l2_out_at(g, p, nreg, fmt);
+          hipLaunchKernelGGL(k_l2_probe, dim3(nreg * 64), dim3(512), 0, g->stream, p, o.cap, nreg, l2_bins_per_region(g, fmt), iters, 0u, o.khi);
+        } else {
+          hipLaunchKernelGGL(k_l2_probe, dim3(nreg * 64), dim3(512), 0, g->stream, p, g->cap2 * g->W, nreg, g->subs_per_bin, iters, 0u, (uint16_t *)nullptr);
+        }
         (void)hipEventRecord(e1, g->stream);
         if (hipEventSynchronize(e1) != hipSuccess || hipEventElapsedTime(&t, e0, e1) != hipSuccess) { (void)hipGetLastError(); t = 0.f; }
       }
@@ -795,12 +854,12 @@
   } else {
     g->l2_base = l2_place(g, nb * g->cap2 * 8 * g->W, std::min<uint32_t>(regions, 32), tries, nullptr);
   }
-  if (!g->l2_base || hipMalloc((void **)&g->l2_cnt, nb * 8) != hipSuccess) {
+  if (!g->l2_base || hipMalloc((void **)&g->l2_cnt, nb * 16) != hipSuccess) {
     (void)hipGetLastError();
     (void)hipFree(g->l2_base); (void)hipFree(g->l2_hi); g->l2_base = g->l2_hi = nullptr;
     return fail(MCX_ERR_NOMEM, "out of device memory for the sub-table bins (%llu regions)", (unsigned long long)regions);
   }
-  HIP_TRY(hipMemsetAsync(g->l2_cnt, 0, nb * 8, g->stream));
+  HIP_TRY(hipMemsetAsync(g->l2_cnt, 0, nb * 16, g->stream));
   g->l2_keys = g->l2_base;
   g->l2_regions = regions;
   return MCX_OK;
@@ -866,6 +925,7 @@
   }
   HIP_TRY(hipMemsetAsync(g->l1_cnt, 0, (size_t)g->nsets * g->b1 * g->rep1 * 8, g->stream));
   g->set_colour.assign(g->nsets, -1);
+  g->set_reads.assign(g->nsets, 1);
   g->set_pending.assign(g->nsets, 0);
   return MCX_OK;
 }
@@ -919,8 +979,11 @@
     const int colour = colours[ci];
     TupleIn in{};
     uint32_t nmine = 0;
+    bool reads_only = true;
     for (uint32_t s = 0; s < g->nsets && g->pending; s++)
-      if (g->set_colour[s] == colour && g->set_pending[s]) in.set_map[nmine++] = (uint8_t)s;
+      if (g->set_colour[s] == colour && g->set_pending[s]) { in.set_map[nmine++] = (uint8_t)s; reads_only = reads_only && g->set_reads[s]; }
+    const int fmt = g->pending_l2 && ci == 0 ? (g->t.rs ? kL2WordRs : kL2Word) : l2_format(g, reads_only);
+    const uint32_t bpr = l2_bins_per_region(g, fmt);
     for (uint32_t r0 = 0; r0 < g->b1; r0 += G, gi++) {
       const uint32_t ng = std::min(G, g->b1 - r0);
       const int hb = overlap ? (int)(gi & 1u) : 0;
@@ -935,9 +998,8 @@
         in.seg_group = ng;
         in.seg_stride = g->b1;
         in.set_rep = g->nsets > 1 ? g->rep1 : 0;
-        BinSpec bs{BIN_SUBLOCAL, 0, g->subs_per_bin, 1, ng * g->subs_per_bin, ng, 0, r0};
-        BinOut out{l2_ptr(g, g->l2_off), nullptr, g->l2_cnt + g->l2_off, g->cap2, nullptr, nullptr, nullptr, 0};
-        DISPATCH_WC(g, launch_split_regions, g, in, colour, bs, out);
+        BinSpec bs{BIN_SUBLOCAL, 0, bpr, 1, ng * bpr, ng, 0, r0};
+        DISPATCH_WC(g, launch_split_regions, g, in, colour, bs, l2_out(g, g->l2_off, G, fmt), fmt);
         HIP_TRY(hipGetLastError());
       }
       if (overlap) {
@@ -945,7 +1007,7 @@
         HIP_TRY(hipStreamWaitEvent(g->stream2, g->ev_split[hb], 0));
         g->stream = g->stream2;
       }
-      DISPATCH_WC(g, launch_lds_insert_t, g, colour, r0 * g->subs_per_bin, ng * g->subs_per_bin);
+      DISPATCH_WC(g, launch_lds_insert_t, g, colour, r0 * g->subs_per_bin, ng * g->subs_per_bin, fmt, l2_out(g, g->l2_off, G, fmt));
       g->stream = s1;
       HIP_TRY(hipGetLastError());
       if (overlap) HIP_TRY(hipEventRecord(g->ev_ins[hb], g->stream2));
@@ -1119,6 +1181,14 @@
 
 
 
+extern "C" int mcx_graph_l2_format(mcx_graph *g, int reads_only, uint32_t *sx)
+{
+  NO_GROUP(g, "mcx_graph_l2_format");
+  if (!g) return fail(MCX_ERR_ARG, "null graph");
+  if (sx) *sx = g->t.sx;
+  return l2_format(g, reads_only != 0);
+}
+
 extern "C" int mcx_graph_configure(mcx_graph *g, const char *key, uint64_t value)
 {
   if (g && key && g->as_group) {
@@ -1156,6 +1226,12 @@
     g->l2_base = g->l2_keys = nk;
     return MCX_OK;
   }
+  if (!strcmp(key, "l2_compact")) {
+    int rc = flush_deferred(g);
+    if (rc != MCX_OK) return rc;
+    g->l2_compact = value != 0;
+    return MCX_OK;
+  }
   if (!strcmp(key, "place_bins")) {
     if (value < 1 || value > 32) return fail(MCX_ERR_ARG, "place_bins: 1..32");
     g->place_tries = (int)value;
@@ -1356,6 +1432,7 @@
     int set = 0;
     int rc = defer_reserve(g, colour, cnt, &set);
     if (rc != MCX_OK) return rc;
+    g->set_reads[set] = 0;
     TupleIn in{(const uint64_t *)d_keys + lo * g->W, (const uint8_t *)d_edges + lo, nullptr, cnt, 1, 1, 1};
     BinSpec bs{BIN_GROUP, 0, g->b1, g->rep1, g->b1, 1, 0, 0};
     BinOut out = l1_out(g, set);
@@ -1472,6 +1549,7 @@
   int set = 0;
   rc = defer_reserve(g, colour, ub, &set);
   if (rc != MCX_OK) return rc;
+  g->set_reads[set] = 0;
   TupleIn in{(const uint64_t *)d_keys, (const uint8_t *)d_edges, (const unsigned long long *)d_counts, seg_cap, nseg, nseg, nseg};
   BinSpec bs{BIN_GROUP, 0, g->b1, g->rep1, g->b1, 1, 0, 0};
   BinOut out = l1_out(g, set);
@@ -1548,7 +1626,7 @@
   TupleIn in{(const uint64_t *)d_keys, nullptr, (const unsigned long long *)d_counts, seg_cap, nseg, nseg, nseg};
   BinSpec bs{BIN_SUBLOCAL, 0, g->subs_per_bin, 1, g->nsub, g->b1, 0, 0};
   BinOut out{g->l2_keys, nullptr, g->l2_cnt, g->cap2, nullptr, nullptr, nullptr, 0};
-  DISPATCH_WC(g, launch_split_regions, g, in, colour, bs, out);
+  DISPATCH_WC(g, launch_split_regions, g, in, colour, bs, out, g->t.rs ? kL2WordRs : kL2Word);
   HIP_TRY(hipGetLastError());
   g->pending_l2 += ntuples;
   return MCX_OK;
@@ -1935,11 +2013,12 @@
   const int colour = g->set_colour[0];
   g->l2_off = 0;
   TupleIn in{g->l1_keys + (uint64_t)r0 * g->cap1 * g->W, nullptr, g->l1_cnt + r0, g->cap1, ng * g->rep1, ng, g->b1};
-  BinSpec bs{BIN_SUBLOCAL, 0, g->subs_per_bin, 1, ng * g->subs_per_bin, ng, 0, r0};
-  BinOut out{g->l2_keys, nullptr, g->l2_cnt, g->cap2, nullptr, nullptr, nullptr, 0};
-  DISPATCH_WC(g, launch_split_regions, g, in, colour, bs, out);
+  const int fmt = l2_format(g, g->set_reads[0] != 0);
+  const uint32_t bpr = l2_bins_per_region(g, fmt);
+  BinSpec bs{BIN_SUBLOCAL, 0, bpr, 1, ng * bpr, ng, 0, r0};
+  DISPATCH_WC(g, launch_split_regions, g, in, colour, bs, l2_out(g, 0, G, fmt), fmt);
   HIP_TRY(hipGetLastError());
-  DISPATCH_WC(g, launch_lds_insert_t, g, colour, r0 * g->subs_per_bin, ng * g->subs_per_bin);
+  DISPATCH_WC(g, launch_lds_insert_t, g, colour, r0 * g->subs_per_bin, ng * g->subs_per_bin, fmt, l2_out(g, 0, G, fmt));
   HIP_TRY(hipGetLastError());
   HIP_TRY(hipMemset2DAsync(g->l1_cnt + r0, (size_t)g->b1 * 8, 0, (size_t)ng * 8, g->rep1, g->stream));
   if (g->idle_mark.size() != ngroups) g->idle_mark.assign(ngroups, g->idle_base);
diff --git a/mccortex_amd/csrc/mcx_defer.h b/mccortex_amd/csrc/mcx_defer.h
--- a/mccortex_amd/csrc/mcx_defer.h
+++ b/mccortex_amd/csrc/mcx_defer.h
@@ -32,6 +32,8 @@
   uint8_t *ov_edges;
   unsigned long long *ov_counts;
   uint64_t ov_cap;
+  uint16_t *khi;
+  uint32_t qsh;
 };
 
 #define MCX_LDS_AS __attribute__((address_space(3)))
@@ -64,6 +66,22 @@
   return q;
 }
 
+enum : int { kL2Word = 0, kL2WordRs = 1, kL2Byte = 2, kL2Code = 3 };
+constexpr uint64_t kL2Mask = (1ull << 48) - 1;
+constexpr uint32_t kL2Skip = 31u;
+template <int F> constexpr uint32_t l2_edge_bits() { return F == kL2Code ? 5u : 8u; }
+__device__ __forceinline__ bool edge_codable(uint32_t e)
+{
+  const uint32_t lo = e & 15u, hi = e >> 4;
+  return ((lo & (lo - 1u)) | (hi & (hi - 1u))) == 0u;
+}
+__device__ __forceinline__ uint32_t edge_code(uint32_t e) { return 5u * (uint32_t)__ffs(e & 15u) + (uint32_t)__ffs(e >> 4); }
+__device__ __forceinline__ uint32_t edge_decode(uint32_t c)
+{
+  const uint32_t a = (c * 13u) >> 6, b = c - 5u * a;
+  return ((1u << a) >> 1) | (((1u << b) >> 1) << 4);
+}
+
 constexpr int kRounds = 2;
 constexpr int kStage = kTile / kRounds;
 
@@ -183,7 +201,7 @@
   if (FULL) L.se[q] = (uint8_t)e;
 }
 
-template <int W, bool ONECOL, bool FULL, int SH, class LDS>
+template <int W, bool ONECOL, bool FULL, int SH, class LDS, int L2F = kL2Word>
 __device__ __forceinline__ void bin_writeout(LDS &L, int round, const BinSpec &bs, const BinOut &out, uint32_t ob0,
                                              uint32_t region_of_seg, const InsertSink<W, ONECOL> &isink,
                                              uint32_t &novel, uint32_t &full)
@@ -194,13 +212,24 @@
   const uint32_t lo = (uint32_t)round * kSt;
   const uint32_t hi = min(n, lo + kSt);
   auto emit = [&](uint32_t p, uint32_t b, unsigned long long gb, uint64_t t0, uint64_t t1) {
-    if (p < (uint32_t)(gb >> 48)) {
+    const bool room = p < (uint32_t)(gb >> 48);
+    if (L2F >= kL2Byte && room) {
+      const uint64_t at = (gb + p) & kDstMask;
+      const uint32_t e = (uint32_t)(t0 >> 56);
+      const bool codable = L2F == kL2Byte || edge_codable(e);
+      const uint64_t v = codable ? (((t0 & kQMask) >> out.qsh) << l2_edge_bits<L2F>()) | (L2F == kL2Byte ? e : edge_code(e)) : kL2Skip;
+      reinterpret_cast<uint32_t *>(out.keys)[at] = (uint32_t)v;
+      out.khi[at] = (uint16_t)(v >> 32);
+      if (codable) return;
+    } else if (L2F < kL2Byte && room) {
       const uint64_t at = (gb + p) & kDstMask;
       uint64_t *kd = out.keys + at * W;
       kd[0] = t0;
       if (W == 2) kd[1] = t1;
       if (FULL) out.edges[at] = L.se[p - lo];
-    } else if (FULL || bs.mode == BIN_OWNER) {
+      return;
+    }
+    if (FULL || bs.mode == BIN_OWNER) {
       full = 2;
     } else {
       Kmer<W> tq;
@@ -512,7 +541,7 @@
   return (uint64_t)q * in.seg_stride + seg % in.seg_group;
 }
 
-template <int W, bool ONECOL, int NB, bool IN_FULL, bool SHARD, int T = kThreads, int R = kRounds, int P = 16>
+template <int W, bool ONECOL, int NB, bool IN_FULL, bool SHARD, int T = kThreads, int R = kRounds, int P = 16, int L2F = kL2Word>
 __global__ __launch_bounds__(T, (W == 1 || T > kThreads ? 4 : 3)) void k_tuples_bin(TupleIn in, BinSpec bs, BinOut out,
                                                                          InsertSink<W, ONECOL> isink_arg, Counters *ctr)
 {
@@ -524,6 +553,8 @@
   if (threadIdx.x == 0) isink = isink_arg;
   __syncthreads();
   const uint32_t t_spb = isink_arg.t.spb, t_lb1 = isink_arg.t.lb1, t_lbq = isink_arg.t.lb1 + isink_arg.t.lbo, t_part = isink_arg.t.part;
+  const uint32_t t_sbits = isink_arg.t.sbits, t_sx = isink_arg.t.sx;
+  static_assert(L2F == kL2Word || (W == 1 && !IN_FULL), "recoverable sub-table bins: one-word packed tuples");
   const int tid = threadIdx.x;
   uint32_t n_novel = 0, full = 0;
   const uint64_t chunks_per_seg = (in.seg_cap + kTile - 1) / kTile;
@@ -562,7 +593,7 @@
     const uint32_t n = (uint32_t)min((uint64_t)kTile, cnt - start);
     const uint32_t lregion = bs.mode == BIN_SUBLOCAL ? seg % bs.seg_mod : 0;
     const uint32_t region = bs.region0 + lregion;
-    const uint32_t ob0 = (bs.mode == BIN_SUBLOCAL ? lregion * t_spb : 0) + (blockIdx.x % bs.rep) * bs.nout;
+    const uint32_t ob0 = (bs.mode == BIN_SUBLOCAL ? lregion * bs.nlocal : 0) + (blockIdx.x % bs.rep) * bs.nout;
     MCX_PH(6) MCX_PH_COUNT
     __syncthreads();
     for (uint32_t b = tid; b < bs.nlocal + 64; b += kThreads) { L.cnt[b] = 0; L.rnk[b] = 0; }
@@ -627,6 +658,10 @@
           foreign_insert<W, ONECOL>(isink, key, ev[q], n_novel, full);
           okm &= ~(1u << q);
         }
+      } else if (L2F != kL2Word) {
+        hb = 0;
+        const uint32_t v = rs_pick(tk[q].w[0] & kQMask, t_sbits);
+        loc[q] = L2F == kL2WordRs ? v >> t_sx : v;
       } else {
         hb = sub_hash<W>(tuple_q<W>(tk[q]));
         loc[q] = __umulhi(hb, t_spb);
@@ -649,7 +684,7 @@
 #pragma unroll
       for (int q = 0; q < PER; q++)
         bin_place<W, false, LDS>(L, round, loc[q] >> 16, loc[q] & 0xffffu, tk[q], 0);
-      bin_writeout<W, ONECOL, false, 0, LDS>(L, round, bs, out, ob0, region, isink, n_novel, full);
+      bin_writeout<W, ONECOL, false, 0, LDS, L2F>(L, round, bs, out, ob0, region, isink, n_novel, full);
       if (round == 0) { MCX_PH(4) } else { MCX_PH(5) }
     }
   }
@@ -934,10 +969,14 @@
   }
 }
 
-template <int W, bool ONECOL>
+template <int W, bool ONECOL, int L2F = kL2Word>
 __global__ __launch_bounds__(LdsCfg<W>::kThreads, LdsCfg<W>::kMinWaves) void k_lds_insert(TableView t, uint32_t col, BinOut bins,
                                                                        uint32_t sub0, uint32_t nsub, Counters *ctr)
 {
+  constexpr bool kCompact = L2F >= kL2Byte;
+  static_assert(!kCompact || W == 1, "compact sub-table bins: one-word keys");
+  constexpr uint32_t kEb = l2_edge_bits<L2F>();
+  const uint32_t bsh = kCompact ? t.sx : 0u;
   constexpr int kLdsThreads = LdsCfg<W>::kThreads;
   constexpr int kLdsBatch = LdsCfg<W>::kBatch;
   extern __shared__ __attribute__((aligned(16))) unsigned char dyn_lds[];
@@ -950,7 +989,7 @@
   if (tid == 0) s_nq = 0;
 
   auto next_bin = [&](uint32_t from) {
-    while (from < nsub && bins.counts[from] == 0) from += gridDim.x;
+    while (from < nsub && bins.counts[from << bsh] == 0 && bins.counts[(from << bsh) + bsh] == 0) from += gridDim.x;
     return from;
   };
   uint32_t bi = next_bin(blockIdx.x);
@@ -959,7 +998,19 @@
   constexpr bool kPrefetch = LdsCfg<W>::kPrefetch;
   if (kPrefetch && bi < nsub) slice_fetch<W, ONECOL, kLdsThreads>(t, sub0 + bi, col, tid, v, zeros_known);
   auto idx = [&](int q) -> uint32_t { return (uint32_t)q * kLdsThreads + tid; };
-  auto load_batch_of = [&](uint32_t bin, uint64_t nfill, uint64_t j0, Kmer<W> (&tk)[kLdsBatch]) {
+  auto load_batch_of = [&](uint32_t bin, uint64_t nfill, uint64_t n0, uint64_t j0, Kmer<W> (&tk)[kLdsBatch]) {
+    if constexpr (kCompact) {
+      const uint32_t *lo32 = reinterpret_cast<const uint32_t *>(bins.keys);
+#pragma unroll
+      for (int q = 0; q < kLdsBatch; q++) {
+        uint64_t i = j0 + idx(q);
+        i = i < nfill ? i : 0;
+        const uint32_t h = i >= n0 ? 1u : 0u;
+        const uint64_t at = (((uint64_t)bin << bsh) + h) * bins.cap + (i - (h ? n0 : 0));
+        tk[q].w[0] = (uint64_t)lo32[at] | ((uint64_t)bins.khi[at] << 32) | ((uint64_t)h << 48);
+      }
+      return;
+    }
     const uint64_t *kin = bins.keys + (uint64_t)bin * bins.cap * W;
 #pragma unroll
     for (int q = 0; q < kLdsBatch; q++) {
@@ -975,21 +1026,36 @@
     const uint32_t sub = sub0 + bi;
     const uint32_t region = sub / t.spb;
     MCX_PH(6) MCX_PH_COUNT
-    uint64_t n = bins.counts[bi];
+    uint64_t n = bins.counts[bi << bsh];
     if (n > bins.cap) n = bins.cap;
+    const uint64_t n0 = n;
+    if (kCompact && bsh) {
+      const uint64_t n1 = bins.counts[(bi << bsh) + 1];
+      n += n1 > bins.cap ? bins.cap : n1;
+    }
     const uint32_t nb = next_bin(bi + gridDim.x);
     __syncthreads();
     MCX_PH(0)
-    if (tid == 0) bins.counts[bi] = 0;
+    if (tid == 0) { bins.counts[bi << bsh] = 0; bins.counts[(bi << bsh) + bsh] = 0; }
     if (!kPrefetch) slice_fetch<W, ONECOL, kLdsThreads>(t, sub, col, tid, v, zeros_known);
     slice_to_lds<W, ONECOL, kLdsThreads>(lds, tid, v);
     __syncthreads();
     MCX_PH(1)
 
-    auto load_batch = [&](uint64_t j0, Kmer<W> (&tk)[kLdsBatch]) { load_batch_of(bi, n, j0, tk); };
+    auto load_batch = [&](uint64_t j0, Kmer<W> (&tk)[kLdsBatch]) { load_batch_of(bi, n, n0, j0, tk); };
+    const uint32_t vbin0 = (sub & (t.spb - 1u)) << bsh;
     auto unpack = [&](const Kmer<W> &tp, Kmer<W> &key, uint32_t &bucket, uint32_t &e) {
-      e = (uint32_t)(tp.w[0] >> 56);
-      const Kmer<W> qq = tuple_q<W>(tp);
+      Kmer<W> qq;
+      if constexpr (kCompact) {
+        const uint64_t v = tp.w[0];
+        const uint32_t ec = (uint32_t)v & ((1u << kEb) - 1u);
+        e = L2F == kL2Code ? edge_decode(ec) : ec;
+        const uint64_t qp = (v & kL2Mask) >> kEb;
+        qq.w[0] = (qp << t.sbits) | ((vbin0 | (uint32_t)(v >> 48)) ^ rs_mask(qp, t.sbits));
+      } else {
+        e = (uint32_t)(tp.w[0] >> 56);
+        qq = tuple_q<W>(tp);
+      }
       const uint32_t m = region_mix<W>(qq);
       key = key_unquot<W>(qq, lbq_of(t), ((t.part << t.lb1) | region) ^ mix_g(m, lbq_of(t)));
       bucket = mix_bucket(m, lbq_of(t), Sub<W>::kBuckets);
@@ -1001,7 +1067,7 @@
     auto apply_batch = [&](uint64_t j0, const Kmer<W> (&tk)[kLdsBatch]) {
 #pragma unroll
       for (int q = 0; q < kLdsBatch; q++)
-        if (j0 + idx(q) < n) {
+        if (j0 + idx(q) < n && !(L2F == kL2Code && ((uint32_t)tk[q].w[0] & 31u) == kL2Skip)) {
           Kmer<W> key;
           uint32_t bucket, e;
           unpack(tk[q], key, bucket, e);
diff --git a/mccortex_amd/csrc/mcx_kernels.h b/mccortex_amd/csrc/mcx_kernels.h
--- a/mccortex_amd/csrc/mcx_kernels.h
+++ b/mccortex_amd/csrc/mcx_kernels.h
@@ -28,6 +28,7 @@
   uint64_t *val;
   uint64_t VC;
   uint32_t *touch;
+  uint32_t rs, sbits, sx;
 };
 constexpr int kTouchHdr = 32;
 __device__ __forceinline__ void table_mark_written(const TableView &t)
@@ -129,15 +130,24 @@
 }
 __device__ __host__ __forceinline__ uint32_t lbq_of(const TableView &t) { return t.lb1 + t.lbo; }
 
+__device__ __host__ __forceinline__ uint32_t rs_mask(uint64_t qp, uint32_t sbits)
+{
+  return mix_g(sub_hash<1>(Kmer<1>{{qp}}), sbits);
+}
+__device__ __host__ __forceinline__ uint32_t rs_pick(uint64_t q, uint32_t sbits)
+{
+  return ((uint32_t)q & ((1u << sbits) - 1u)) ^ rs_mask(q >> sbits, sbits);
+}
+
 struct TableAddr { uint32_t G, region, sub, bucket; };
 template <int W> __device__ __forceinline__ TableAddr addr_of(const TableView &t, const Kmer<W> &q, uint32_t r)
 {
-  const uint32_t b = sub_hash<W>(q);
   const uint32_t lbq = lbq_of(t), m = region_mix<W>(q);
   TableAddr a;
   a.G = r ^ mix_g(m, lbq);
   a.region = a.G & ((1u << t.lb1) - 1u);
-  a.sub = a.region * t.spb + __umulhi(b, t.spb);
+  if (W == 1 && t.rs) a.sub = a.region * t.spb + (rs_pick(q.w[0], t.sbits) >> t.sx);
+  else a.sub = a.region * t.spb + __umulhi(sub_hash<W>(q), t.spb);
   a.bucket = mix_bucket(m, lbq, Sub<W>::kBuckets);
   return a;
 }
diff --git a/mccortex_amd/graph.py b/mccortex_amd/graph.py
--- a/mccortex_amd/graph.py
+++ b/mccortex_amd/graph.py
@@ -21,6 +21,7 @@
     "mcx_kmer_from_str", "mcx_kmer_canonical", "mcx_kmer_hash", "mcx_pack_bases", "mcx_pack_reads_host", "mcx_pack_stream_dev", "mcx_graph_add_packed_dev",
     "mcx_ubench_stream", "mcx_ubench_random_rmw", "mcx_graph_insert_stats", "mcx_multi_exchange_bytes", "mcx_graph_hashtest", "mcx_hashtest_func", "mcx_debug_probe",
     "mcx_graph_infer_edges", "mcx_graph_infer_edges_dev", "mcx_graph_unitig_stats", "mcx_graph_clean",
+    "mcx_graph_l2_format",
 ]
 
 
@@ -93,6 +94,7 @@
     L.mcx_graph_add_records.argtypes = [vp, vp, C.c_uint64, C.c_int, vp, vp, C.c_int, C.c_uint32, C.POINTER(RecordStats)]
     L.mcx_graph_kmer_covg.argtypes = [vp, u64p, u64p]
     L.mcx_graph_insert_stats.argtypes = [vp, vp]
+    L.mcx_graph_l2_format.argtypes = [vp, C.c_int, C.POINTER(C.c_uint32)]
     L.mcx_graph_covg_histogram.argtypes = [vp, u64p, C.c_uint32]
     L.mcx_sort_records.argtypes = [vp, C.c_uint64, C.c_int, C.c_int, C.c_int]
     L.mcx_records_sorted.argtypes = [vp, C.c_uint64, C.c_int, C.c_int, C.c_int, C.POINTER(C.c_int64)]
@@ -408,6 +410,13 @@
         _check(self.L.mcx_graph_insert_stats(self.h, st))
         return dict(zip(("fallback_inserts", "foreign_inserts", "spilled", "flushes"), (int(x) for x in st)))
 
+    def l2_format(self, reads_only=True):
+        sx = C.c_uint32()
+        rc = self.L.mcx_graph_l2_format(self.h, 1 if reads_only else 0, C.byref(sx))
+        if rc < 0:
+            _check(rc)
+        return int(rc), int(sx.value)
+
     @property
     def stream(self):
         return self.L.mcx_graph_stream(self.h)
```

After: 103.1 billion, median of 2. No clear change (-0.6%).
